# hadleyhzy34/porl

Measured on AMD Instinct MI355X. Metric: gradient-steps/sec (POR update, batch=1024), higher is better.
Workload: dtype f32; 1 GPU; POR S=60 A=2 H=1024 L=2 B=1024/GPU (global 1024), 1000000 -row replay (1000000/GPU) resident in HBM, device sampler + gather + full update per step; parallelism=dp1, global_batch=1024

## Files before the change

### include/porl_hip.h

```cpp
#ifndef PORL_HIP_H
#define PORL_HIP_H

#include <stdint.h>

#ifdef __cplusplus
extern "C" {
#endif

#define PORL_ABI_VERSION 11
#define PORL_MAX_HIDDEN 8

#define PORL_OK 0
#define PORL_ERR_INVALID (-1)
#define PORL_ERR_UNSUPPORTED (-2)
#define PORL_ERR_UNBOUND (-3)

int porl_abi_version(void);
const char* porl_last_error(void);

typedef struct porl_iql_cfg {
  int32_t obs_dim;
  int32_t pol_out_dim;
  int32_t hidden_dim;
  int32_t n_hidden;
  int32_t layer_norm;
  int32_t pol_tanh;
  int32_t weight_mode;
  int32_t max_batch;
} porl_iql_cfg;

typedef struct porl_iql porl_iql;

int porl_iql_create(const porl_iql_cfg* cfg, porl_iql** out);
void porl_iql_destroy(porl_iql* h);

int64_t porl_iql_group_floats(const porl_iql* h, int group);
int32_t porl_iql_group_tensors(const porl_iql* h, int group);
int porl_iql_tensor_info(const porl_iql* h, int group, int index, int64_t* offset, int32_t* rows,
                         int32_t* cols);

int64_t porl_iql_workspace_floats(const porl_iql* h);

typedef struct porl_iql_buffers {
  float* params_vf;
  float* params_tgt;
  float* params_pol;
  float* grads_vf;
  float* grads_pol;
  float* adam_m_vf;
  float* adam_v_vf;
  float* adam_m_pol;
  float* adam_v_pol;
  float* workspace;
  float* stats;
} porl_iql_buffers;

int porl_iql_bind(porl_iql* h, const porl_iql_buffers* bufs);

int porl_iql_load_batch(porl_iql* h, int32_t batch,
                        const float* obs, int64_t obs_rs,
                        const float* next_obs, int64_t next_rs,
                        const float* rew, int64_t rew_rs,
                        const float* term, int64_t term_rs,
                        const float* pol_target, int64_t pt_rs,
                        void* stream);

int porl_iql_load_batch_sampled(porl_iql* h, int32_t batch, const float* rows, int64_t row_stride,
                                int64_t n_rows, int32_t act_dim, int32_t target_is_action,
                                uint64_t seed, uint64_t step, int64_t* idx_out, void* stream);

#define PORL_IQL_SLOTS 3
#define PORL_IQL_MODE_TWO_SLOTS 1
#define PORL_IQL_MODE_FOLD_COMBINE 2
#define PORL_IQL_MODE_SHORT_BLOCKS 4
int porl_iql_set_mode(porl_iql* h, int32_t mode);

int porl_iql_set_stats(porl_iql* h, float* stats);

typedef struct porl_iql_hyper {
  float tau;
  float discount;
  float alpha;
  float inv_batch;
  int32_t value_step;
  int32_t policy_step;
  int32_t reserved;
  double ema_beta;
  double value_lr;
  double policy_lr;
  double adam_beta1, adam_beta2, adam_eps;
} porl_iql_hyper;

int porl_iql_value_backward(porl_iql* h, const porl_iql_hyper* hp, void* stream);
int porl_iql_value_apply(porl_iql* h, const porl_iql_hyper* hp, void* stream);
int porl_iql_policy_prefetch(porl_iql* h, void* stream);
int porl_iql_policy_forward(porl_iql* h, const porl_iql_hyper* hp, void* stream);
int porl_iql_policy_backward(porl_iql* h, const porl_iql_hyper* hp, void* stream);
int porl_iql_policy_apply(porl_iql* h, const porl_iql_hyper* hp, void* stream);
int porl_iql_step(porl_iql* h, const porl_iql_hyper* hp, void* stream);
int porl_iql_policy_only_forward(porl_iql* h, const porl_iql_hyper* hp, void* stream);
int porl_iql_policy_only_step(porl_iql* h, const porl_iql_hyper* hp, void* stream);

int porl_iql_forward_value(porl_iql* h, int which, const float* x, int64_t x_rs, int32_t batch,
                           float* v1_out, float* v2_out, void* stream);
int porl_iql_forward_policy(porl_iql* h, const float* x, int64_t x_rs, int32_t batch, float* mean_out,
                            int64_t mean_rs, void* stream);

typedef struct porl_qnet_cfg {
  int32_t state_dim;
  int32_t n_actions;
  int32_t n_hidden;
  int32_t hidden[PORL_MAX_HIDDEN];
  int32_t max_batch;
} porl_qnet_cfg;

typedef struct porl_qnet porl_qnet;

typedef struct porl_qnet_buffers {
  float* params;
  float* params_tgt;
  float* grads;
  float* adam_m;
  float* adam_v;
  float* workspace;
  float* stats;
} porl_qnet_buffers;

typedef struct porl_qnet_hyper {
  float gamma;
  float alpha;
  float inv_batch;
  int32_t step;
  double lr;
  double adam_beta1, adam_beta2, adam_eps;
} porl_qnet_hyper;

int porl_qnet_create(const porl_qnet_cfg* cfg, porl_qnet** out);
void porl_qnet_destroy(porl_qnet* h);
int64_t porl_qnet_param_floats(const porl_qnet* h);
int32_t porl_qnet_tensors(const porl_qnet* h);
int porl_qnet_tensor_info(const porl_qnet* h, int index, int64_t* offset, int32_t* rows, int32_t* cols,
                          int32_t* row_stride);
int64_t porl_qnet_workspace_floats(const porl_qnet* h);
int porl_qnet_bind(porl_qnet* h, const porl_qnet_buffers* bufs);
int porl_qnet_load_batch(porl_qnet* h, int32_t batch, const float* states, int64_t s_rs,
                         const int64_t* actions, int64_t a_rs, const float* rewards, int64_t r_rs,
                         const float* next_states, int64_t n_rs, const float* dones, int64_t d_rs,
                         void* stream);
int porl_qnet_cql_backward(porl_qnet* h, const porl_qnet_hyper* hp, void* stream);
int porl_qnet_forward_loaded(porl_qnet* h, int which_params, int which_input, int keep, float* out, int64_t out_rs,
                             void* stream);
int porl_qnet_backward(porl_qnet* h, const float* dout, int64_t dout_rs, void* stream);

int porl_qr_loss(const float* z_cur, const float* z_next_online, const float* z_next_target, int64_t ld,
                 const int64_t* actions, const float* rewards, const float* dones, int32_t batch, int32_t n_actions,
                 int32_t n_quantiles, float gamma, float kappa, float* dz_out, float* row_loss, void* stream);
int porl_iqn_quantile_huber(const float* current, const float* target, const float* taus, int32_t batch, int32_t n_current,
                            int32_t n_target, float kappa, float* dcurrent_out, float* row_loss, void* stream);
int porl_iqn_cos_embed(const float* taus, int64_t n, int32_t embedding_dim, float* out, void* stream);
int porl_iqn_hadamard(const float* feat, int64_t ldf, const float* emb, int32_t batch, int32_t n_tau, int32_t width,
                      float* out, void* stream);
int porl_iqn_hadamard_backward(const float* dout, const float* feat, int64_t ldf, const float* emb, int32_t batch,
                               int32_t n_tau, int32_t width, float* dfeat, float* demb, void* stream);
int porl_iqn_select(const float* z, const int64_t* actions, int32_t batch, int32_t n_tau, int32_t n_actions, float* out,
                    void* stream);
int porl_iqn_scatter(const float* dsel, const int64_t* actions, int32_t batch, int32_t n_tau, int32_t n_actions, float* dz,
                     void* stream);
int porl_iqn_target(const float* z_online_next, const float* z_target_next, const float* rewards, const float* dones,
                    float gamma, int32_t batch, int32_t n_tau, int32_t n_actions, float* td, int64_t* next_actions,
                    void* stream);
int porl_grad_clip(float* grads, int64_t n, float max_norm, float* norm_coef, double* workspace, void* stream);
int porl_c51_loss(const float* logits_cur, const float* logits_next_target, int64_t ld, const int64_t* actions,
                  const float* rewards, const float* dones, const float* support, int32_t batch, int32_t n_actions,
                  int32_t n_atoms, float gamma, float v_min, float v_max, float* dlogits_out, float* row_loss, void* stream);
int porl_reduce_mean(const float* x, int32_t n, float* out, void* stream);

int porl_qnet_apply(porl_qnet* h, const porl_qnet_hyper* hp, void* stream);
int porl_qnet_learn(porl_qnet* h, const porl_qnet_hyper* hp, void* stream);
int32_t porl_qnet_one_launch(const porl_qnet* h);
int porl_qnet_learn_indexed(porl_qnet* h, const float* states, int64_t s_rs, const int64_t* actions,
                            const float* rewards, const float* next_states, int64_t n_rs, const float* dones,
                            const int64_t* idx, int32_t batch, const porl_qnet_hyper* hp, void* stream);
typedef struct porl_qnet_variant {
  int32_t double_dqn;
  const float* is_weights;
  const float* uniform_weight;
  float* td_abs;
  const float* next_mask;
  int32_t td_off;
} porl_qnet_variant;
int32_t porl_qnet_can_sample(const porl_qnet* h);
int porl_qnet_learn_sampled(porl_qnet* h, const float* states, int64_t s_rs, const int64_t* actions, const float* rewards,
                            const float* next_states, int64_t n_rs, const float* dones, int64_t n_rows, uint64_t seed,
                            uint64_t draw, int32_t batch, const porl_qnet_hyper* hp, void* stream);
int porl_qnet_learn_variant(porl_qnet* h, const float* states, int64_t s_rs, const int64_t* actions,
                            const float* rewards, const float* next_states, int64_t n_rs, const float* dones,
                            const int64_t* idx, int32_t batch, const porl_qnet_hyper* hp,
                            const porl_qnet_variant* variant, void* stream);
int porl_qnet_learn_sampled_variant(porl_qnet* h, const float* states, int64_t s_rs, const int64_t* actions,
                                    const float* rewards, const float* next_states, int64_t n_rs, const float* dones,
                                    int64_t n_rows, uint64_t seed, uint64_t draw, int32_t batch, const porl_qnet_hyper* hp,
                                    const porl_qnet_variant* variant, void* stream);
int porl_qnet_bcq_mask(porl_qnet* beh, const float* next_states, int64_t n_rs, const int64_t* idx, int32_t batch,
                       float threshold, float* mask_out, void* stream);
int porl_qnet_bcq_learn(porl_qnet* h, porl_qnet* beh, const float* states, int64_t s_rs, const int64_t* actions,
                        const float* rewards, const float* next_states, int64_t n_rs, const float* dones,
                        const int64_t* idx, int32_t batch, const porl_qnet_hyper* hp, float threshold, void* stream);
int porl_qnet_bcq_learn_sampled(porl_qnet* h, porl_qnet* beh, const float* states, int64_t s_rs, const int64_t* actions,
                                const float* rewards, const float* next_states, int64_t n_rs, const float* dones,
                                int64_t n_rows, uint64_t seed, uint64_t draw, int32_t batch, const porl_qnet_hyper* hp,
                                float threshold, void* stream);
#define PORL_DIST_QR 0
#define PORL_DIST_C51 1
typedef struct porl_dist_head {
  int32_t kind;
  int32_t n_actions;
  int32_t n_sub;
  float kappa;
  float v_min, v_max;
  const float* support;
} porl_dist_head;
int porl_qnet_dist_learn(porl_qnet* h, const float* states, int64_t s_rs, const int64_t* actions, const float* rewards,
                         const float* next_states, int64_t n_rs, const float* dones, const int64_t* idx, int32_t batch,
                         const porl_qnet_hyper* hp, const porl_dist_head* head, void* stream);
int porl_qnet_sync_target(porl_qnet* h, void* stream);
int porl_qnet_forward(porl_qnet* h, int which, const float* states, int64_t s_rs, int32_t batch,
                      float* q_out, int64_t q_rs, void* stream);
// ... 216 lines not shown
```

### porl_amd/agent/_iql.py

```python
from __future__ import annotations

import math
import warnings

import torch
import torch.nn as nn

from ..engine import IqlEngine
from ..parallel import GradExchange



_PIPE_SYNC = __import__("os").environ.get("PORL_PIPE_SYNC", "signal2")
_PIPE_ONECALL = __import__("os").environ.get("PORL_PIPE_ONECALL", "auto")
_DP_POLICY_GROUP = __import__("os").environ.get("PORL_DP_POLICY_GROUP", "1") != "0"
_ONECALL_MAX_WORK = 32 << 20

class ArenaAdam:

    def __init__(self, agent, group, named_params, lr):
        self._agent, self._group = agent, group
        self._names = [n for n, _ in named_params]
        self._params = [p for _, p in named_params]
        self.step_count = 0
# ... 12 lines not shown
        table = eng.tensor_table(self._group)
        return IqlEngine.views(flat_m, table), IqlEngine.views(flat_v, table)

    def zero_grad(self, set_to_none=True):
        pass

    def step(self):
        raise RuntimeError("ArenaAdam steps inside the fused update (por_residual_update / update)")

    sharded = False

    def _gather_moments(self):
        if self.sharded:
            eng, ex = self._agent._engine, self._agent._exchange
            _, _, m, v, _ = eng.group(self._group)
            ex.all_gather_(m)
            ex.all_gather_(v)

    def _unshard(self):
        if self.sharded:
            self._gather_moments()
            self.sharded = False

    def consolidate_state(self):
        self._agent.flush()
        self._unshard()

    def state_dict(self):
        self._agent.flush()
        self._gather_moments()
        ms, vs = self._moments()
        state = {}
        if self.step_count > 0:
            for i, (m, v) in enumerate(zip(ms, vs)):
                state[i] = dict(step=torch.tensor(float(self.step_count)), exp_avg=m.clone(), exp_avg_sq=v.clone())
        groups = [{k: v for k, v in self.param_groups[0].items() if k != "params"}]
        groups[0]["params"] = list(range(len(self._params)))
        return dict(state=state, param_groups=groups)

    def load_state_dict(self, sd):
        self._agent.flush()
        ms, vs = self._moments()
        steps = set()
        with torch.no_grad():
            for i, st in sd["state"].items():
                ms[int(i)].copy_(st["exp_avg"])
                vs[int(i)].copy_(st["exp_avg_sq"])
                steps.add(int(float(st["step"])))
        if len(steps) > 1:
            raise ValueError("per-parameter Adam step counts differ; the flat sweep needs one counter")
        self.step_count = steps.pop() if steps else 0
        self.sharded = False
        g = sd["param_groups"][0]
        for k in ("lr", "betas", "eps", "initial_lr"):
            if k in g:
                self.param_groups[0][k] = g[k]


class CosineSchedule:

    def __init__(self, optimizer: ArenaAdam, T_max):
        self.optimizer, self.T_max, self.last_epoch = optimizer, T_max, 0
        self.base_lrs = [optimizer.param_groups[0]["initial_lr"]]

    def _lr(self, t):
        return self.base_lrs[0] * (1.0 + math.cos(math.pi * t / self.T_max)) / 2.0

    def step(self):
        self.last_epoch += 1
        self.optimizer.param_groups[0]["lr"] = self._lr(self.last_epoch)

    def get_last_lr(self):
        return [self.optimizer.param_groups[0]["lr"]]

    def state_dict(self):
        return dict(T_max=self.T_max, last_epoch=self.last_epoch, base_lrs=list(self.base_lrs))

    def load_state_dict(self, sd):
        self.T_max, self.last_epoch = sd["T_max"], sd["last_epoch"]
        self.base_lrs = list(sd["base_lrs"])
        self.optimizer.param_groups[0]["lr"] = self._lr(self.last_epoch)


class IqlAgentBase(nn.Module):

    _warned_nll = False
    pipeline = True
    grad_exchange = "reduce_scatter"
    dp_policy_group = _DP_POLICY_GROUP

    def _setup_engine(self, vf: nn.Module, v_target: nn.Module, policy: nn.Module, *, obs_dim, pol_out_dim,
                      hidden_dim, n_hidden, layer_norm, pol_tanh, weight_mode, device, max_batch):
        self._engine = IqlEngine(obs_dim, pol_out_dim, hidden_dim, n_hidden, layer_norm, pol_tanh, weight_mode,
                                 max_batch, device)
        self._mods = (vf, v_target, policy)
        self._adopt(copy_from_modules=True)
        self._exchange = GradExchange()
        self._gslice = {}
        self.async_losses = False

    def _adopt(self, copy_from_modules=False):
        eng = self._engine
        vf, v_target, policy = self._mods
        pairs = ((vf, eng.params_vf, IqlEngine.GROUP_VF, "vf"),
                 (v_target, eng.params_tgt, IqlEngine.GROUP_VF, "target"),
                 (policy, eng.params_pol, IqlEngine.GROUP_POL, "policy"))
        with torch.no_grad():
            for mod, flat, group, role in pairs:
                views = IqlEngine.views(flat, eng.tensor_table(group))
                params = list(mod.parameters())
                if len(params) != len(views):
                    raise RuntimeError(f"{role}: {len(params)} parameters vs {len(views)} engine tensors")
                for p, v in zip(params, views):
                    if tuple(p.shape) != tuple(v.shape):
                        raise RuntimeError(f"{role}: parameter shape {tuple(p.shape)} vs engine {tuple(v.shape)}")
                    if copy_from_modules:
                        v.copy_(p)
                    p.data = v
                mod._engine, mod._engine_role, mod._private = eng, role, False
        for p in v_target.parameters():
            p.requires_grad_(False)

    def _apply(self, fn, recurse=True):
        self.flush()
        probe = fn(torch.empty(0, dtype=torch.float32, device=self._engine.device))
        if probe.dtype != torch.float32:
            raise RuntimeError("porl_amd agents are fp32 only")
        self._engine.to(probe.device)
        self.device = probe.device
        self._adopt()
        backbone = getattr(self, "backbone", None)
        if backbone is not None:
            backbone._apply(fn)
        return self

    def _hyper(self, batch, v_opt: ArenaAdam, p_opt: ArenaAdam):
        world = self._exchange.world_size
        return self._engine.hyper(
            tau=self.tau, discount=self.discount, alpha=self.alpha, ema_beta=self.beta,
            inv_batch=1.0 / (batch * world), value_lr=v_opt.lr, policy_lr=p_opt.lr,
            value_step=v_opt.step_count, policy_step=p_opt.step_count,
            adam_beta1=v_opt.param_groups[0]["betas"][0], adam_beta2=v_opt.param_groups[0]["betas"][1],
            adam_eps=v_opt.param_groups[0]["eps"])

    def _full_update(self, obs, next_obs, rew, term, pol_target, v_opt, p_opt, sched, replay=None, batch=None):
        eng, ex = self._engine, self._exchange
        world = ex.world_size
        dp = ex.active
        pipelined = self.async_losses and self.pipeline
        if not pipelined:
            eng.join()
        eng._ensure_bound()
        eng.set_mode(((IqlEngine.MODE_TWO_SLOTS | IqlEngine.MODE_SHORT_BLOCKS) if pipelined else 0) |
                     (IqlEngine.MODE_FOLD_COMBINE if not dp else 0))
        use_sig = pipelined and _PIPE_SYNC in ("signal", "signal2") and eng.signals() is not None
        onecall = _PIPE_ONECALL is True or _PIPE_ONECALL == "1" or (
            _PIPE_ONECALL == "auto" and (batch or 0) * eng.cfg.hidden_dim ** 2 <= _ONECALL_MAX_WORK)
        if use_sig and not dp and replay is not None and onecall:
            eng._seq += 1
            seq = eng._seq
            v_opt.step_count += 1
            p_opt.step_count += 1
            hp = self._hyper(batch, v_opt, p_opt)
            vr = eng._values_read
            try:
                eng.update_pipelined(hp, replay, batch, seq,
                                     wait_policy_seq=max(0, seq - eng.SLOTS) if _PIPE_SYNC == "signal" else 0,
                                     wait_fwd_seq=vr[1] if isinstance(vr, tuple) else 0,
                                     write_policy=_PIPE_SYNC == "signal")
            except Exception:
                eng._seq -= 1
                v_opt.step_count -= 1
                p_opt.step_count -= 1
                raise
            replay.draws += 1
            eng._values_read, eng._policy_done = ("sig", seq), True
            sched.step()
            return self._losses()
        if use_sig:
            main = torch.cuda.current_stream(eng.device)
            eng._seq += 1
            seq = eng._seq
            if _PIPE_SYNC == "signal":
                eng.wait_signal(eng.SIG_POLICY, seq - eng.SLOTS, main)
        elif pipelined:
            eng.wait_slot_free()
        if replay is not None:
            B = eng.load_batch_sampled(replay.rows, batch, replay.seed, replay.draws, replay.act_dim,
                                       self._engine.cfg.weight_mode == 1)
            replay.draws += 1
        else:
            B = eng.load_batch(obs, next_obs, rew, term, pol_target)
        v_opt.step_count += 1
        p_opt.step_count += 1
        hp = self._hyper(B, v_opt, p_opt)
        if not dp and not pipelined:
            eng.step(hp)
            sched.step()
            return self._losses()
        eng.value_backward(hp)
        if dp and self._sharded():
            self._sharded_apply(IqlEngine.GROUP_VF, hp, v_opt)
        else:
            if dp:
                v_opt._unshard()
                ex.allreduce_sum_(eng.grads_vf)
            eng.wait_values_read()
            eng.value_apply(hp)
        if pipelined:
            main, side = torch.cuda.current_stream(eng.device), eng.side_stream()
            k = (v_opt.step_count % eng.SLOTS) * 3
            ev_v, ev_f, ev_p = eng.event(k), eng.event(k + 1), eng.event(k + 2)
            if use_sig:
                eng.signal(eng.SIG_VALUE, seq, main)
            else:
                ev_v.record(main)
            with torch.cuda.stream(side):
                if use_sig:
                    eng.wait_signal(eng.SIG_VALUE, seq, side)
                else:
                    side.wait_event(ev_v)
                eng.policy_forward(hp)
                if use_sig:
                    eng.signal(eng.SIG_FWD, seq, side)
                else:
                    ev_f.record(side)
                eng.policy_backward(hp)
                if dp and self._sharded():
                    self._sharded_apply(IqlEngine.GROUP_POL, hp, p_opt, self._exchange_for(IqlEngine.GROUP_POL, True))
                else:
                    if dp:
                        p_opt._unshard()
                        self._exchange_for(IqlEngine.GROUP_POL, True).allreduce_sum_(eng.grads_pol)
                    eng.policy_apply(hp)
                if _PIPE_SYNC == "signal" and use_sig:
                    eng.signal(eng.SIG_POLICY, seq, side)
                if not use_sig:
                    ev_p.record(side)
            eng._values_read, eng._policy_done = (("sig", seq) if use_sig else ev_f), (True if use_sig else ev_p)
            eng._slot_users = eng._slot_users[1:] + [None if use_sig else ev_p]
        else:
            eng.policy_backward(hp)
            if self._sharded():
                self._sharded_apply(IqlEngine.GROUP_POL, hp, p_opt)
            else:
                p_opt._unshard()
                ex.allreduce_sum_(eng.grads_pol)
                eng.policy_apply(hp)
            if not self.async_losses:
                ex.allreduce_stats_(eng.stats)
        sched.step()
        return self._losses()

    def _sharded(self):
        eng, ex = self._engine, self._exchange
        return self.grad_exchange == "reduce_scatter" and ex.can_shard(eng.grads_vf) and ex.can_shard(eng.grads_pol)

    def _exchange_for(self, group, pipelined):
        ex = self._exchange
        if group != IqlEngine.GROUP_POL or not pipelined or not ex.active or not self.dp_policy_group:
            return ex
        if getattr(self, "_exchange_pol", None) is None:
            import torch.distributed as dist
            self._exchange_pol = GradExchange(dist.new_group(), force=ex.force)
            probe = torch.zeros(1, dtype=torch.float32, device=self._engine.device)
            dist.all_reduce(probe, group=self._exchange_pol.group)
            torch.cuda.synchronize(self._engine.device)
        return self._exchange_pol

    def _sharded_apply(self, group, hp, opt, ex=None):
        from .. import engine as E
        eng = self._engine
        ex = ex or self._exchange
        p, g, m, v, tgt = eng.group(group)
        gs = self._gslice.get(group)
        if gs is None or gs.numel() != p.numel() // ex.world_size:
            gs = self._gslice[group] = torch.empty(p.numel() // ex.world_size, dtype=torch.float32, device=p.device)
        ex.reduce_scatter_sum(g, gs)
        if group == IqlEngine.GROUP_VF:
            eng.wait_values_read()
        b1, b2 = opt.param_groups[0]["betas"]
        E.adam_ema(ex.slice_of(p), gs, ex.slice_of(m), ex.slice_of(v), None, opt.lr, opt.step_count, b1, b2,
                   opt.param_groups[0]["eps"], 0.0)
        ex.all_gather_(p)
        if tgt is not None:
            E.ema(tgt, p, hp.ema_beta)
        opt.sharded = True

    def flush(self):
        self._engine.join()

    def state_dict(self, *args, **kwargs):
        self.flush()
        return super().state_dict(*args, **kwargs)

    def load_state_dict(self, *args, **kwargs):
        self.flush()
        return super().load_state_dict(*args, **kwargs)

    def _load(self, obs, next_obs, rew, term, pol_target, replay, batch):
        eng = self._engine
        if replay is None:
            return eng.load_batch(obs, next_obs, rew, term, pol_target)
        B = eng.load_batch_sampled(replay.rows, batch, replay.seed, replay.draws, replay.act_dim,
                                   eng.cfg.weight_mode == 1)
        replay.draws += 1
        return B
# ... 74 lines not shown
```

### porl_amd/csrc/gemm_f32.hpp

```cpp
#pragma once
#include <hip/hip_runtime.h>
#include <stdint.h>

#ifndef PORL_ABL
#define PORL_ABL 0
#endif

namespace porl {

enum : int { ACT_NONE = 0, ACT_RELU = 1, ACT_TANH = 2 };

enum : int {
  APRO_NONE = 0,
  APRO_AFFINE_RELU = 1,
};

struct GemmProb {
  const float* A;
  const float* B;
  float* C;
  const float* bias;
  const float* mask;
  const float* headw;
  float* headout;
  float* colsum;
  const float* a_colscale;
  const float* a_colshift;
  const float* resid;
  const float* rscale;
  float* cstat;
  int rs_rows, rs_row0;
  int a_grp, a_grp_jump, a_seg_tiles, a_seg_jump;
  int M, N, K;
  int lda, ldb, ldc, ldmask;
  int act;
  int apro;
  int splitk;
  int store_c;
  int a_vec, b_vec;
  int a_kc, b_kc;
  int c_vec;
  int tiles_m, tiles_n, block_start, kchunk;
};

constexpr int MAX_GROUP = 8;
struct GemmGroup {
  int nprob;
  int total_blocks;
  int single_buffer;
  GemmProb p[MAX_GROUP];
  int lds_pad, lds_pad_min_blocks;
};

typedef float f32x16 __attribute__((ext_vector_type(16)));

__host__ __device__ constexpr int lds_stride(int R) { return R + 4; }

struct StageSlot {
  unsigned off;
  int kpos;
  int cpos;
  int lds;
};

typedef int i32x4 __attribute__((ext_vector_type(4)));
typedef float f32x4 __attribute__((ext_vector_type(4)));
constexpr unsigned BUF_OOB = 0x80000000u;

__device__ f32x4 llvm_raw_buffer_load_v4f32(i32x4 rsrc, int voffset, int soffset, int aux) __asm("llvm.amdgcn.raw.buffer.load.v4f32");
__device__ float llvm_raw_buffer_load_f32(i32x4 rsrc, int voffset, int soffset, int aux) __asm("llvm.amdgcn.raw.buffer.load.f32");

typedef i32x4 BufRsrc;
__device__ __forceinline__ BufRsrc make_rsrc(const float* p, size_t bytes) {
  const unsigned long long a = reinterpret_cast<unsigned long long>(p);
  BufRsrc r;
  r.x = (int)(unsigned)(a & 0xFFFFFFFFull);
  r.y = (int)(unsigned)((a >> 32) & 0xFFFFull);
  r.z = (int)(bytes >= 0x7FFFFFFFull ? 0x7FFFFFFFu : (unsigned)bytes);
  r.w = 0x00020000;
  return r;
}
__device__ __forceinline__ float4 buf_ld128(BufRsrc r, unsigned voff, unsigned soff) {
  const f32x4 v = llvm_raw_buffer_load_v4f32(r, (int)voff, (int)soff, 0);
  return make_float4(v.x, v.y, v.z, v.w);
}
__device__ __forceinline__ float buf_ld32(BufRsrc r, unsigned voff, unsigned soff) {
  return llvm_raw_buffer_load_f32(r, (int)voff, (int)soff, 0);
}

template <bool V> struct BoolTag { static constexpr bool value = V; };
template <int V> struct IntTag { static constexpr int value = V; };

#ifdef PORL_STAMP
__device__ unsigned long long g_stamps[16 * 4096];
#endif

template <int BM, int BN, int BK, int WM, int WN, bool VEC, bool APRO, bool ONEBUF = false>
__global__ __launch_bounds__(64 * WM * WN) void gemm_f32_kernel(const GemmGroup g) {
  constexpr int THREADS = 64 * WM * WN;
  constexpr int WTM = BM / WM / 32;
  constexpr int WTN = BN / WN / 32;
  constexpr int SA = lds_stride(BM);
  constexpr int SB = lds_stride(BN);
  constexpr int SK = BK + 4;
  constexpr int A_TILE = (BK * SA > BM * SK) ? BK * SA : BM * SK;
  constexpr int B_TILE = (BK * SB > BN * SK) ? BK * SB : BN * SK;
  static_assert(BK % 8 == 0, "a k-group is 8 wide");
  constexpr int NLA = BM * BK / 4 / THREADS;
  constexpr int NLB = BN * BK / 4 / THREADS;
  static_assert(NLA >= 1 && NLB >= 1, "tile too small for the thread count");
  static_assert(BM * BK / 4 % THREADS == 0 && BN * BK / 4 % THREADS == 0, "staging must divide evenly");
  static_assert(BK % 4 == 0 && WTM >= 1 && WTN >= 1 && BM % (32 * WM) == 0 && BN % (32 * WN) == 0, "tile shape");

  constexpr int APRO_MAX_K = ONEBUF ? 512 : 1024;
  constexpr int NBUF = ONEBUF ? 1 : 2;
  __shared__ __attribute__((aligned(16))) float lds[NBUF * (A_TILE + B_TILE) + (APRO ? 2 * APRO_MAX_K : 0)];

  const int t = threadIdx.x;
  const int lane = t & 63;
  const int wave = t >> 6;
  const int wm = wave / WN, wn = wave % WN;
  const int li = lane & 31, kh = lane >> 5;
#ifdef PORL_STAMP
  unsigned long long rt_entry = 0, rt_loop0 = 0, rt_loop1 = 0, cy0 = 0, cy1 = 0, cy_barrier = 0, cy_store = 0, cy_load = 0, cy_group[4] = {0, 0, 0, 0};
  if (t == 0) rt_entry = __builtin_amdgcn_s_memrealtime();
#endif

  int lin;
  {
    const int nb = gridDim.x, bid = blockIdx.x;
    const int q = nb >> 3, r = nb & 7, xcd = bid & 7;
    lin = (xcd < r ? xcd * (q + 1) : r * (q + 1) + (xcd - r) * q) + (bid >> 3);
  }
  int pi = 0;
#pragma unroll
  for (int i = 1; i < MAX_GROUP; ++i)
    if (i < g.nprob && lin >= g.p[i].block_start) pi = i;
  const GemmProb& P = g.p[pi];
  const int local = lin - P.block_start;
  const int tiles = P.tiles_m * P.tiles_n;
  const int split = local / tiles;
  const int tl = local - split * tiles;
  const int tm = tl / P.tiles_n, tn = tl - tm * P.tiles_n;
  const int m0 = tm * BM, n0 = tn * BN;
  const int M = P.M, N = P.N;
  const int ks = split * P.kchunk;
  const int ke = min(P.K, ks + P.kchunk);
  const int nkt = (ke - ks + BK - 1) / BK;
  const float* __restrict__ Ag = P.A;
  const float* __restrict__ Bg = P.B;
  const bool a_kc = P.a_kc != 0, b_kc = P.b_kc != 0;
  const bool do_colsum = (!a_kc) && (P.colsum != nullptr) && (tn == 0);
  const bool full = VEC && (m0 + BM <= M) && (n0 + BN <= N) && ((ke - ks) % BK == 0);
  auto ktile = [&](int i) { return i; };

  StageSlot sa[NLA], sb[NLB];
  const int a_dk = a_kc ? 1 : 0, a_dc = 1 - a_dk;
  const int b_dk = b_kc ? 1 : 0, b_dc = 1 - b_dk;
  const size_t a_step = a_kc ? (size_t)BK : (size_t)BK * P.lda;
  const size_t b_step = b_kc ? (size_t)BK : (size_t)BK * P.ldb;
  const size_t a_rows_ext = P.a_grp > 0 ? (size_t)M + (size_t)(M / P.a_grp + 1) * (size_t)(P.a_grp_jump / P.lda + 1) +
                                              (size_t)(P.a_seg_jump / P.lda + 1)
                                        : (size_t)(a_kc ? M : P.K);
  const BufRsrc a_rsrc = make_rsrc(Ag, a_rows_ext * P.lda * sizeof(float));
  const BufRsrc b_rsrc = make_rsrc(Bg, (size_t)(b_kc ? N : P.K) * P.ldb * sizeof(float));
  const unsigned a_org = (unsigned)((a_kc ? (size_t)ks : (size_t)ks * P.lda) * sizeof(float));
  const unsigned b_org = (unsigned)((b_kc ? (size_t)ks : (size_t)ks * P.ldb) * sizeof(float));
  const int a_seg_tiles = P.a_grp > 0 ? P.a_seg_tiles : 0x7fffffff;
  const unsigned a_seg_jump = (unsigned)((size_t)P.a_seg_jump * sizeof(float));
  auto a_soff = [&](int kt) {
    return a_org + (unsigned)(kt * a_step * sizeof(float)) + (kt >= a_seg_tiles ? a_seg_jump : 0u);
  };
  auto b_soff = [&](int kt) { return b_org + (unsigned)(kt * b_step * sizeof(float)); };
#pragma unroll
  for (int i = 0; i < NLA; ++i) {
    const int f = t + THREADS * i;
    if (a_kc) {
      const int kq = f % (BK / 4), row = f / (BK / 4);
      sa[i].kpos = ks + kq * 4; sa[i].cpos = m0 + row; sa[i].lds = row * SK + kq * 4;
      const size_t grp = P.a_grp > 0 ? (size_t)((m0 + row) / P.a_grp) * P.a_grp_jump : 0;
      sa[i].off = (unsigned)(((size_t)(m0 + row) * P.lda + grp + kq * 4) * sizeof(float));
    } else {
      const int c4 = f % (BM / 4), kr = f / (BM / 4);
      sa[i].kpos = ks + kr; sa[i].cpos = m0 + c4 * 4; sa[i].lds = kr * SA + c4 * 4;
      sa[i].off = (unsigned)(((size_t)kr * P.lda + (m0 + c4 * 4)) * sizeof(float));
    }
  }
#pragma unroll
  for (int i = 0; i < NLB; ++i) {
    const int f = t + THREADS * i;
    if (b_kc) {
      const int kq = f % (BK / 4), row = f / (BK / 4);
      sb[i].kpos = ks + kq * 4; sb[i].cpos = n0 + row; sb[i].lds = row * SK + kq * 4;
      sb[i].off = (unsigned)(((size_t)(n0 + row) * P.ldb + kq * 4) * sizeof(float));
    } else {
      const int c4 = f % (BN / 4), kr = f / (BN / 4);
      sb[i].kpos = ks + kr; sb[i].cpos = n0 + c4 * 4; sb[i].lds = kr * SB + c4 * 4;
      sb[i].off = (unsigned)(((size_t)kr * P.ldb + (n0 + c4 * 4)) * sizeof(float));
    }
  }

  float* const apro_cs = lds + NBUF * (A_TILE + B_TILE);
  if constexpr (APRO) {
    for (int k = t; k < P.K; k += THREADS) { apro_cs[k] = P.a_colscale[k]; apro_cs[APRO_MAX_K + k] = P.a_colshift[k]; }
  }

  float4 ra[NLA], rb[NLB];
  float4 csum = make_float4(0.f, 0.f, 0.f, 0.f);

  f32x16 acc[WTM][WTN];
#pragma unroll
  for (int i = 0; i < WTM; ++i)
#pragma unroll
    for (int j = 0; j < WTN; ++j)
#pragma unroll
      for (int r = 0; r < 16; ++r) acc[i][j][r] = 0.f;

  const int a_off = wm * (BM / WM) + li;
  const int b_off = wn * (BN / WN) + li;

  auto main_loop = [&](auto guard_tag, auto akc_tag, auto bkc_tag, auto csum_tag) {
    constexpr bool GUARD = decltype(guard_tag)::value;
    constexpr bool AKC = decltype(akc_tag)::value;
    constexpr bool CSUM = decltype(csum_tag)::value;

    auto slot_ok = [&](const StageSlot& s, int kadv, int dk, int dc, int cmax, bool (&ok)[4]) {
      const int k = s.kpos + kadv;
      if constexpr (VEC) {
        ok[0] = ok[1] = ok[2] = ok[3] = (k < ke) && (s.cpos < cmax);
      } else {
#pragma unroll
        for (int j = 0; j < 4; ++j) ok[j] = (k + j * dk < ke) && (s.cpos + j * dc < cmax);
      }
    };
    auto load_raw = [&](const StageSlot& s, BufRsrc r, unsigned soff, const bool (&ok)[4]) -> float4 {
      float4 v;
      if constexpr (VEC) {
        v = buf_ld128(r, ok[0] ? s.off : BUF_OOB, soff);
      } else {
        v.x = buf_ld32(r, ok[0] ? s.off : BUF_OOB, soff);
        v.y = buf_ld32(r, ok[1] ? s.off + 4u : BUF_OOB, soff);
        v.z = buf_ld32(r, ok[2] ? s.off + 8u : BUF_OOB, soff);
        v.w = buf_ld32(r, ok[3] ? s.off + 12u : BUF_OOB, soff);
      }
      return v;
    };

    auto load_tile = [&](int kt) {
      const int kadv = kt * BK;
#pragma unroll
// ... 258 lines not shown
    } else {
      main_loop(guard_tag, BoolTag<false>{}, BoolTag<false>{}, BoolTag<false>{});
    }
  };
  if constexpr (VEC) {
    if (full) run(BoolTag<false>{});
    else run(BoolTag<true>{});
  } else {
    run(BoolTag<true>{});
  }
#ifdef PORL_STAMP
  if (t == 0) { rt_loop1 = __builtin_amdgcn_s_memrealtime(); cy1 = __builtin_amdgcn_s_memtime(); }
#endif

  if (do_colsum) {
    __syncthreads();
    float4* red = reinterpret_cast<float4*>(lds);
    constexpr int C4 = BM / 4;
    auto reduce_cols = [&](const float4& mine, float* out) {
      red[t] = mine;
      __syncthreads();
      if (t < C4) {
        float4 s = red[t];
        for (int u = t + C4; u < THREADS; u += C4) {
          const float4 o = red[u];
          s.x += o.x; s.y += o.y; s.z += o.z; s.w += o.w;
        }
        const int c = m0 + t * 4;
        if (c < M) out[c] = s.x;
        if (c + 1 < M) out[c + 1] = s.y;
        if (c + 2 < M) out[c + 2] = s.z;
        if (c + 3 < M) out[c + 3] = s.w;
      }
      __syncthreads();
    };
    reduce_cols(csum, P.colsum + (size_t)split * M);
  }

  const bool raw = P.splitk > 1;
  float* __restrict__ Cg = P.C + (raw ? (size_t)split * M * P.ldc : 0);
  const bool has_head = (!raw) && P.headw != nullptr;
  const float* __restrict__ maskp = raw ? nullptr : P.mask;
  const int act = raw ? ACT_NONE : P.act;
  const bool store_c = P.store_c != 0;
  constexpr int WROWS = BM / WM, WCOLS = BN / WN, CS = WCOLS + 4;
  static_assert(WM * WN * WROWS * CS <= NBUF * (A_TILE + B_TILE), "C sub-tiles must fit in the staging LDS");
  const bool fast_c = store_c && P.c_vec && (m0 + BM <= M) && (n0 + BN <= N);
  float* ctile = lds + wave * (WROWS * CS);
#pragma unroll
  for (int i = 0; i < WTM; ++i) {
    const int rbase = m0 + wm * (BM / WM) + i * 32 + 4 * kh;
#pragma unroll
    for (int j = 0; j < WTN; ++j) {
      const int col = n0 + wn * (BN / WN) + j * 32 + li;
      const bool col_ok = col < N;
      float bv = 0.f, hw = 0.f;
      if (!raw && col_ok) {
        if (P.bias) bv = P.bias[col];
        if (has_head) hw = P.headw[col];
      }
      float vals[16];
#pragma unroll
      for (int r = 0; r < 16; ++r) {
        float v = acc[i][j][r] + bv;
        if (act == ACT_RELU) v = fmaxf(v, 0.f);
        else if (act == ACT_TANH) v = tanhf(v);
        vals[r] = v;
      }
      if (maskp && !fast_c) {
#pragma unroll
        for (int r = 0; r < 16; ++r) {
          const int row = rbase + (r & 3) + 8 * (r >> 2);
          const bool ok = row < M && col_ok;
          const float mv = *(ok ? maskp + (size_t)row * P.ldmask + col : maskp);
          vals[r] = (ok && mv > 0.f) ? vals[r] : 0.f;
        }
      }
      if (!raw && P.resid && !fast_c) {
#pragma unroll
        for (int r = 0; r < 16; ++r) {
          const int row = rbase + (r & 3) + 8 * (r >> 2);
          if (row < M && col_ok) {
            const float rs = P.rscale ? P.rscale[(row + P.rs_row0) / P.rs_rows] : 1.f;
            vals[r] = __fadd_rn(P.resid[(size_t)row * P.ldc + col], __fmul_rn(vals[r], rs));
          }
        }
      }
      if (!raw && P.cstat) {
        float cs = 0.f, cq = 0.f;
#pragma unroll
        for (int r = 0; r < 16; ++r) {
          const int row = rbase + (r & 3) + 8 * (r >> 2);
          const float v = row < M ? vals[r] : 0.f;
          cs += v;
          cq = fmaf(v, v, cq);
        }
        cs += __shfl_xor(cs, 32);
        cq += __shfl_xor(cq, 32);
        const int rblk = (m0 + wm * (BM / WM)) / 32 + i;
        if (kh == 0 && col_ok && rblk * 32 < M) {
          float* o = P.cstat + (size_t)rblk * 2 * N + col;
          o[0] = cs;
          o[N] = cq;
        }
      }
      if (has_head) {
        const int part = (n0 + wn * (BN / WN) + j * 32) >> 5;
#pragma unroll
        for (int r = 0; r < 16; ++r) {
          float sh = vals[r] * hw;
          sh += __shfl_xor(sh, 16);
          sh += __shfl_xor(sh, 8);
          sh += __shfl_xor(sh, 4);
          sh += __shfl_xor(sh, 2);
          sh += __shfl_xor(sh, 1);
          const int row = rbase + (r & 3) + 8 * (r >> 2);
          if (li == 0 && row < M && part * 32 < N) P.headout[(size_t)part * M + row] = sh;
        }
      }
      if (store_c) {
        if (fast_c) {
#pragma unroll
          for (int r = 0; r < 16; ++r)
            ctile[(i * 32 + (r & 3) + 8 * (r >> 2) + 4 * kh) * CS + j * 32 + li] = vals[r];
        } else {
#pragma unroll
          for (int r = 0; r < 16; ++r) {
            const int row = rbase + (r & 3) + 8 * (r >> 2);
            if (row < M && col_ok) Cg[(size_t)row * P.ldc + col] = vals[r];
          }
        }
      }
    }
  }
  if (fast_c) {
    constexpr int C4 = WCOLS / 4;
    const int wr0 = m0 + wm * WROWS, wc0 = n0 + wn * WCOLS;
#pragma unroll 4
    for (int f = lane; f < WROWS * C4; f += 64) {
      const int r = f / C4, c = (f % C4) * 4;
      float4 v = *reinterpret_cast<const float4*>(ctile + r * CS + c);
      if (maskp) {
        const float4 mk = *reinterpret_cast<const float4*>(maskp + (size_t)(wr0 + r) * P.ldmask + wc0 + c);
        v.x = mk.x > 0.f ? v.x : 0.f; v.y = mk.y > 0.f ? v.y : 0.f;
        v.z = mk.z > 0.f ? v.z : 0.f; v.w = mk.w > 0.f ? v.w : 0.f;
      }
      if (!raw && P.resid) {
        const float rs = P.rscale ? P.rscale[(wr0 + r + P.rs_row0) / P.rs_rows] : 1.f;
        const float4 x4 = *reinterpret_cast<const float4*>(P.resid + (size_t)(wr0 + r) * P.ldc + wc0 + c);
        v.x = __fadd_rn(x4.x, __fmul_rn(v.x, rs)); v.y = __fadd_rn(x4.y, __fmul_rn(v.y, rs));
        v.z = __fadd_rn(x4.z, __fmul_rn(v.z, rs)); v.w = __fadd_rn(x4.w, __fmul_rn(v.w, rs));
      }
      *reinterpret_cast<float4*>(Cg + (size_t)(wr0 + r) * P.ldc + wc0 + c) = v;
    }
  }
#ifdef PORL_STAMP
  __syncthreads();
  if (t == 0 && blockIdx.x < 4096) {
    const unsigned hwid = __builtin_amdgcn_s_getreg((4 ) | (0 << 6) | (31 << 11));
    const unsigned xcc = __builtin_amdgcn_s_getreg((20 ) | (0 << 6) | (31 << 11));
    unsigned long long* o = g_stamps + 16 * blockIdx.x;
    o[0] = rt_entry; o[1] = rt_loop0; o[2] = rt_loop1; o[3] = __builtin_amdgcn_s_memrealtime();
    o[4] = cy1 - cy0; o[5] = ((xcc & 0xF) << 12) | ((hwid >> 8) & 0xFFF);
    o[6] = cy_group[0]; o[7] = cy_group[1]; o[8] = cy_group[2]; o[9] = cy_group[3];
  }
#endif
}

__global__ void slab_reduce_kernel(float* __restrict__ out, const float* __restrict__ slab, int nslab,
                                   long n, long stride, const float* __restrict__ bias, int ncols, int act) {
  for (long i = (long)blockIdx.x * blockDim.x + threadIdx.x; i < n; i += (long)gridDim.x * blockDim.x) {
    float s = slab[i];
    for (int k = 1; k < nslab; ++k) s += slab[(long)k * stride + i];
    if (bias) s += bias[i % ncols];
    if (act == ACT_RELU) s = fmaxf(s, 0.f);
    else if (act == ACT_TANH) s = tanhf(s);
    out[i] = s;
  }
}

enum GemmMode : int { GEMM_NT = 0, GEMM_NN = 1, GEMM_TN = 2 };
enum GemmTile : int { TILE_128x128 = 0, TILE_128x64 = 1, TILE_64x128 = 2, TILE_64x64 = 3,
                      TILE_128x96 = 4,
                      TILE_COUNT = 5 };

constexpr int GEMM_BK = 32;

struct TileCfg { int bm, bn, wm, wn; };
inline TileCfg tile_cfg(int tile) {
  switch (tile) {
    case TILE_128x128: return {128, 128, 2, 2};
    case TILE_128x64: return {128, 64, 2, 2};
    case TILE_64x128: return {64, 128, 2, 2};
    case TILE_128x96: return {128, 96, 4, 1};
    default: return {64, 64, 2, 2};
  }
}

inline void tile_dims(int tile, int& bm, int& bn) {
  const TileCfg c = tile_cfg(tile);
  bm = c.bm; bn = c.bn;
}

inline int head_parts(int N, int tile) {
  (void)tile;
  return (N + 31) / 32;
}
constexpr int HEAD_PARTS_PER_64_COLS = 2;

inline bool aligned16(const void* p) { return (reinterpret_cast<uintptr_t>(p) & 15u) == 0; }

inline int plan_group(GemmGroup& g, int tile) {
  int bm, bn;
  tile_dims(tile, bm, bn);
  int start = 0;
  for (int i = 0; i < g.nprob; ++i) {
    GemmProb& p = g.p[i];
    p.tiles_m = (p.M + bm - 1) / bm;
    p.tiles_n = (p.N + bn - 1) / bn;
    if (p.splitk < 1) p.splitk = 1;
    int kc = (p.K + p.splitk - 1) / p.splitk;
    kc = ((kc + GEMM_BK - 1) / GEMM_BK) * GEMM_BK;
    p.kchunk = kc;
    p.c_vec = aligned16(p.C) && (p.ldc % 4 == 0) && (p.splitk == 1 || ((size_t)p.M * p.ldc) % 4 == 0) &&
              (p.mask == nullptr || (aligned16(p.mask) && p.ldmask % 4 == 0));
    p.block_start = start;
    start += p.tiles_m * p.tiles_n * p.splitk;
  }
  g.total_blocks = start;
  return start;
}

template <int BM, int BN, int WM, int WN>
inline hipError_t launch_tile(const GemmGroup& g, hipStream_t s) {
  dim3 grid(g.total_blocks), block(64 * WM * WN);
  const int pad = g.total_blocks >= g.lds_pad_min_blocks ? g.lds_pad : 0;
  bool vec = true, apro = g.p[0].apro != APRO_NONE;
  for (int i = 0; i < g.nprob; ++i) {
    vec = vec && g.p[i].a_vec && g.p[i].b_vec;
    if ((g.p[i].apro != APRO_NONE) != apro) return hipErrorInvalidValue;
    if (g.p[i].splitk <= 1 && (g.p[i].mask || g.p[i].resid) && (g.p[i].cstat || g.p[i].headw)) return hipErrorInvalidValue;
  }
  if (apro) {
    if constexpr ((BM == 64 && BN == 64) || (BM == 128 && BN == 64) || (BM == 128 && BN == 96)) {
      for (int i = 0; i < g.nprob; ++i) {
        const GemmProb& p = g.p[i];
        if (!p.a_kc || !p.b_kc || p.K % GEMM_BK || p.splitk > 1 || !p.a_colscale || !p.a_colshift || !vec ||
            (reinterpret_cast<uintptr_t>(p.a_colscale) & 15u) || (reinterpret_cast<uintptr_t>(p.a_colshift) & 15u))
          return hipErrorInvalidValue;
        if (p.K > (g.single_buffer && BM == 64 && BN == 64 ? 512 : 1024)) return hipErrorInvalidValue;
      }
      if constexpr (BM == 64 && BN == 64) {
        if (g.single_buffer) {
          hipLaunchKernelGGL((gemm_f32_kernel<BM, BN, GEMM_BK, WM, WN, true, true, true>), grid, block, pad, s, g);
          return hipGetLastError();
        }
      }
      hipLaunchKernelGGL((gemm_f32_kernel<BM, BN, GEMM_BK, WM, WN, true, true>), grid, block, pad, s, g);
      return hipGetLastError();
    } else {
      return hipErrorInvalidValue;
    }
  }
  if constexpr (BM == 64 && BN == 64) {
    if (vec && g.single_buffer) {
      hipLaunchKernelGGL((gemm_f32_kernel<BM, BN, GEMM_BK, WM, WN, true, false, true>), grid, block, pad, s, g);
      return hipGetLastError();
    }
  }
  if (vec) hipLaunchKernelGGL((gemm_f32_kernel<BM, BN, GEMM_BK, WM, WN, true, false>), grid, block, pad, s, g);
  else hipLaunchKernelGGL((gemm_f32_kernel<BM, BN, GEMM_BK, WM, WN, false, false>), grid, block, pad, s, g);
  return hipGetLastError();
}

inline hipError_t launch_gemm_group(int tile, GemmGroup& g, hipStream_t s) {
  if (g.nprob < 1 || g.nprob > MAX_GROUP) return hipErrorInvalidValue;
  if (plan_group(g, tile) == 0) return hipSuccess;
  switch (tile) {
    case TILE_128x128: return launch_tile<128, 128, 2, 2>(g, s);
    case TILE_128x64: return launch_tile<128, 64, 2, 2>(g, s);
    case TILE_64x128: return launch_tile<64, 128, 2, 2>(g, s);
    case TILE_64x64: return launch_tile<64, 64, 2, 2>(g, s);
    case TILE_128x96: return launch_tile<128, 96, 4, 1>(g, s);
  }
  return hipErrorInvalidValue;
}

inline GemmProb make_prob(int mode, const float* A, int lda, const float* B, int ldb, float* C, int ldc, int M,
                          int N, int K) {
  GemmProb p{};
  p.a_kc = (mode == GEMM_NT || mode == GEMM_NN);
  p.b_kc = (mode == GEMM_NT);
  p.A = A; p.B = B; p.C = C;
  p.M = M; p.N = N; p.K = K;
  p.lda = lda; p.ldb = ldb; p.ldc = ldc;
  p.act = ACT_NONE; p.apro = APRO_NONE; p.splitk = 1; p.store_c = 1; p.rs_rows = 1;
  p.a_vec = aligned16(A) && (lda % 4 == 0) && ((p.a_kc ? K : M) % 4 == 0);
  p.b_vec = aligned16(B) && (ldb % 4 == 0) && ((p.b_kc ? K : N) % 4 == 0);
  return p;
}

}
```

### porl_amd/csrc/kernels.hpp

```cpp
#pragma once
#include <hip/hip_runtime.h>
#include <stdint.h>

namespace porl {

constexpr float LOG_STD_MIN = -5.0f;
constexpr float LOG_STD_MAX = 2.0f;
constexpr float EXP_ADV_MAX = 100.0f;

__device__ __forceinline__ float wave_sum(float v) {
#pragma unroll
  for (int o = 32; o > 0; o >>= 1) v += __shfl_xor(v, o);
  return v;
}
__device__ __forceinline__ float wave_min(float v) {
#pragma unroll
  for (int o = 32; o > 0; o >>= 1) v = fminf(v, __shfl_xor(v, o));
  return v;
}

struct PackJob {
  const float* src; float* dst;
  long src_row_stride;
  long src_col_stride;
// ... 155 lines not shown
    m += mb[0];
    if (a.tanh_mean) m = tanhf(m);
    const float z = cv ? (xv - m) * isg[0] : 0.f;
    const float zz = wave_sum(z * z);
    const float nlp = half_log2pi_D + 0.5f * zz + lsig;
    loss_acc += wb * nlp;
    min_acc = fminf(min_acc, nlp);
    if (cv) {
      float dm = -wb * z * isg[0];
      if (a.tanh_mean) dm *= (1.f - m * m);
      a.dmean[(size_t)b * a.ldd + lane] = dm;
      dls[0] += wb * (1.f - z * z);
    }
  }
  for (int b = row0 + wave; !fast && b < row1; b += 4) {
    float v0 = 0.f, v1 = 0.f;
    for (int p = lane; p < a.parts; p += 64) {
      v0 += a.hp_v[0][(size_t)p * a.B + b];
      v1 += a.hp_v[1][(size_t)p * a.B + b];
    }
    v0 = wave_sum(v0); v1 = wave_sum(v1);
    const float adv = a.weight ? 0.f : a.target_v[b] - fminf(v0 + bv0, v1 + bv1);
    const float wgt = a.weight ? a.weight[b] : fminf(expf(a.weight_mode ? a.alpha * adv : adv / a.alpha), EXP_ADV_MAX);
    const float wb = wgt * a.inv_batch;
    float zz = 0.f;
    float z[NLL_MAX_COLS_PER_LANE], mu[NLL_MAX_COLS_PER_LANE];
#pragma unroll
    for (int c = 0; c < NLL_MAX_COLS_PER_LANE; ++c) {
      const int j = lane + 64 * c;
      z[c] = 0.f; mu[c] = 0.f;
      if (c < ncl && j < a.D) {
        float m = a.mean_slab[(size_t)b * a.ldm + j];
#pragma unroll 8
        for (int s = 1; s < a.nslab; ++s) m += a.mean_slab[(size_t)s * a.slab_stride + (size_t)b * a.ldm + j];
        m += mb[c];
        if (a.tanh_mean) m = tanhf(m);
        mu[c] = m;
        z[c] = (a.x[(size_t)b * a.ldx + j] - m) * isg[c];
        zz += z[c] * z[c];
      }
    }
    zz = wave_sum(zz);
    const float nlp = half_log2pi_D + 0.5f * zz + lsig;
    loss_acc += wb * nlp;
    min_acc = fminf(min_acc, nlp);
#pragma unroll
    for (int c = 0; c < NLL_MAX_COLS_PER_LANE; ++c) {
      const int j = lane + 64 * c;
      if (c < ncl && j < a.D) {
        float dm = -wb * z[c] * isg[c];
        if (a.tanh_mean) dm *= (1.f - mu[c] * mu[c]);
        a.dmean[(size_t)b * a.ldd + j] = dm;
        dls[c] += wb * (1.f - z[c] * z[c]);
      }
    }
  }
  for (int b = row0 + wave; b < row1; b += 4)
    for (int j = a.D + lane; j < a.ldd; j += 64) a.dmean[(size_t)b * a.ldd + j] = 0.f;

#pragma unroll
  for (int c = 0; c < NLL_MAX_COLS_PER_LANE; ++c) sh_dls[wave][c * 64 + lane] = dls[c];
  if (lane == 0) { sh_loss[wave] = loss_acc; sh_min[wave] = min_acc; }
  __syncthreads();
  if (wave == 0) {
#pragma unroll
    for (int c = 0; c < NLL_MAX_COLS_PER_LANE; ++c) {
      const int j = lane + 64 * c;
      if (c < ncl && j < a.D) {
        const float ls = a.log_std[j];
        const float inside = (ls >= LOG_STD_MIN && ls <= LOG_STD_MAX) ? 1.f : 0.f;
        a.part_dls[(size_t)blockIdx.x * a.D + j] = inside *
            (sh_dls[0][c * 64 + lane] + sh_dls[1][c * 64 + lane] + sh_dls[2][c * 64 + lane] + sh_dls[3][c * 64 + lane]);
      }
    }
    if (lane == 0) {
      a.part_loss[blockIdx.x] = sh_loss[0] + sh_loss[1] + sh_loss[2] + sh_loss[3];
      a.part_min[blockIdx.x] = fminf(fminf(sh_min[0], sh_min[1]), fminf(sh_min[2], sh_min[3]));
    }
  }
}


struct ReduceJob {
  float* out; const float* slab; const float* bias;
  long n; long stride; int nslab; int ncols; int act;
  int op;
  float scale;
  long adam_off;
  int width;
};
constexpr int MAX_REDUCE_JOBS = 12;
struct ReduceArgs { int njobs; ReduceJob job[MAX_REDUCE_JOBS]; };

constexpr int REDUCE_LDS_FLOATS = 64 * 5;
__device__ __forceinline__ float reduce_chunk(const ReduceJob& j, long i0, float* sh) {
  const int W = j.width, L = 256 / W;
  const int tx = threadIdx.x % W, ty = threadIdx.x / W;
  const long i = i0 + tx;
  const float id = j.op ? INFINITY : 0.f;
  float s0 = id, s1 = id, s2 = id, s3 = id;
  if (i < j.n) {
    const float* p = j.slab + i;
    int k = ty;
    for (; k + 3 * L < j.nslab; k += 4 * L) {
      const float x0 = p[(long)k * j.stride], x1 = p[(long)(k + L) * j.stride];
      const float x2 = p[(long)(k + 2 * L) * j.stride], x3 = p[(long)(k + 3 * L) * j.stride];
      if (j.op) { s0 = fminf(s0, x0); s1 = fminf(s1, x1); s2 = fminf(s2, x2); s3 = fminf(s3, x3); }
      else { s0 += x0; s1 += x1; s2 += x2; s3 += x3; }
    }
    for (; k < j.nslab; k += L) {
      const float x = p[(long)k * j.stride];
      s0 = j.op ? fminf(s0, x) : s0 + x;
    }
  }
  const float s = j.op ? fminf(fminf(s0, s1), fminf(s2, s3)) : (s0 + s1) + (s2 + s3);
  sh[ty * (W + 1) + tx] = s;
  __syncthreads();
  if (W == 4) {
    const int w = threadIdx.x >> 6, ln = threadIdx.x & 63;
    float v = sh[ln * (W + 1) + w];
    v = j.op ? wave_min(v) : wave_sum(v);
    __syncthreads();
    if (ln == 0) sh[w] = v;
    __syncthreads();
  }
  float t = 0.f;
  if (ty == 0 && i < j.n) {
    t = sh[tx];
    if (W != 4)
      for (int q = 1; q < L; ++q) t = j.op ? fminf(t, sh[q * (W + 1) + tx]) : t + sh[q * (W + 1) + tx];
    t *= j.scale;
    if (j.bias) t += j.bias[i % j.ncols];
    if (j.act == 1) t = fmaxf(t, 0.f);
    else if (j.act == 2) t = tanhf(t);
  }
  __syncthreads();
  return t;
}

__global__ __launch_bounds__(256) void multi_reduce_kernel(const ReduceArgs a) {
  __shared__ float sh[REDUCE_LDS_FLOATS];
  const ReduceJob& j = a.job[blockIdx.y];
  const int W = j.width, tx = threadIdx.x % W, ty = threadIdx.x / W;
  for (long i0 = (long)blockIdx.x * W; i0 < j.n; i0 += (long)gridDim.x * W) {
    const float t = reduce_chunk(j, i0, sh);
    if (ty == 0 && i0 + tx < j.n) j.out[i0 + tx] = t;
  }
}

struct AdamScalars { float omb1, beta2, omb2, eps, step_size, bc2_sqrt, ema_beta, omeb; };
constexpr int ADAM_SWEEP_SLABS = 16;
constexpr int MAX_ADAM_REGIONS = 8;
struct AdamRegion { long lo, hi; const float* slab; long stride; int nslab; };
struct AdamArgs {
  float* p; float* g; float* m; float* v; float* tgt;
  long n4;
  long span4;
  int reduce_blocks;
  AdamScalars s;
  int nregions; AdamRegion region[MAX_ADAM_REGIONS];
  int nskip; long skip_lo[MAX_REDUCE_JOBS], skip_hi[MAX_REDUCE_JOBS];
  int job_block0[MAX_REDUCE_JOBS + 1];
  ReduceArgs r;
};

__device__ __forceinline__ float ema1(float t, float p, float omeb, float ema_beta) { return t * omeb + ema_beta * p; }

__device__ __forceinline__ void adam1(float& p, float g, float& m, float& v, const AdamScalars& s) {
  m = m + s.omb1 * (g - m);
  v = v * s.beta2 + s.omb2 * g * g;
  p = p - s.step_size * (m / (sqrtf(v) / s.bc2_sqrt + s.eps));
}

__global__ __launch_bounds__(256) void adam_ema_kernel(const AdamArgs a) {
  __shared__ float sh[REDUCE_LDS_FLOATS];
  const AdamScalars s = a.s;
  if ((int)blockIdx.x < a.reduce_blocks) {
    const int rb = blockIdx.x;
    int ji = 0;
#pragma unroll
    for (int q = 1; q < MAX_REDUCE_JOBS; ++q)
      if (q < a.r.njobs && rb >= a.job_block0[q]) ji = q;
    const ReduceJob& j = a.r.job[ji];
    const long i0 = (long)(rb - a.job_block0[ji]) * j.width;
    const float t = reduce_chunk(j, i0, sh);
    const int tx = threadIdx.x % j.width, ty = threadIdx.x / j.width;
    if (ty == 0 && i0 + tx < j.n) {
      j.out[i0 + tx] = t;
      if (j.adam_off >= 0) {
        const long e = j.adam_off + i0 + tx;
        float pp = a.p[e], mm = a.m[e], vv = a.v[e];
        adam1(pp, t, mm, vv, s);
        a.p[e] = pp; a.m[e] = mm; a.v[e] = vv;
        if (a.tgt) a.tgt[e] = ema1(a.tgt[e], pp, s.omeb, s.ema_beta);
      }
    }
    return;
  }
  float4* p4 = reinterpret_cast<float4*>(a.p);
  float4* g4 = reinterpret_cast<float4*>(a.g);
  float4* m4 = reinterpret_cast<float4*>(a.m);
  float4* v4 = reinterpret_cast<float4*>(a.v);
  float4* t4 = reinterpret_cast<float4*>(a.tgt);
  const long lo4 = (long)(blockIdx.x - a.reduce_blocks) * a.span4, hi4 = min(a.n4, lo4 + a.span4);
  bool special = false;
  for (int q = 0; q < a.nregions; ++q) special = special || (lo4 * 4 < a.region[q].hi && hi4 * 4 > a.region[q].lo);
  for (int q = 0; q < a.nskip; ++q) special = special || (lo4 * 4 < a.skip_hi[q] && hi4 * 4 > a.skip_lo[q]);
  for (long i = lo4 + threadIdx.x; i < hi4; i += 256) {
    float4 gg;
    bool have_g = false;
    if (special) {
      const long e = i * 4;
      bool skip = false;
      for (int q = 0; q < a.nskip; ++q) skip = skip || (e >= a.skip_lo[q] && e < a.skip_hi[q]);
      if (skip) continue;
      for (int q = 0; q < a.nregions; ++q) {
        const AdamRegion& R = a.region[q];
        if (e >= R.lo && e < R.hi) {
          float4 part[8];
#pragma unroll
          for (int u = 0; u < 8; ++u) part[u] = make_float4(0.f, 0.f, 0.f, 0.f);
          const float* base = R.slab + (e - R.lo);
#pragma unroll
          for (int k = 0; k < ADAM_SWEEP_SLABS; ++k)
            if (k < R.nslab) {
              const float4 x = *reinterpret_cast<const float4*>(base + (long)k * R.stride);
              part[k & 7].x += x.x; part[k & 7].y += x.y; part[k & 7].z += x.z; part[k & 7].w += x.w;
            }
          gg = part[0];
#pragma unroll
          for (int u = 1; u < 8; ++u) { gg.x += part[u].x; gg.y += part[u].y; gg.z += part[u].z; gg.w += part[u].w; }
          g4[i] = gg;
          have_g = true;
        }
      }
    }
    if (!have_g) gg = g4[i];
    float4 pp = p4[i];
    float4 mm = m4[i], vv = v4[i];
    adam1(pp.x, gg.x, mm.x, vv.x, s); adam1(pp.y, gg.y, mm.y, vv.y, s);
    adam1(pp.z, gg.z, mm.z, vv.z, s); adam1(pp.w, gg.w, mm.w, vv.w, s);
    p4[i] = pp; m4[i] = mm; v4[i] = vv;
    if (a.tgt) {
      float4 tt = t4[i];
      tt.x = ema1(tt.x, pp.x, s.omeb, s.ema_beta); tt.y = ema1(tt.y, pp.y, s.omeb, s.ema_beta);
      tt.z = ema1(tt.z, pp.z, s.omeb, s.ema_beta); tt.w = ema1(tt.w, pp.w, s.omeb, s.ema_beta);
      t4[i] = tt;
    }
  }
}

__global__ __launch_bounds__(256) void ema_kernel(float* __restrict__ tgt, const float* __restrict__ src, long n4,
                                                   float omeb, float ema_beta) {
  float4* t4 = reinterpret_cast<float4*>(tgt);
  const float4* p4 = reinterpret_cast<const float4*>(src);
  const long i = (long)blockIdx.x * 256 + threadIdx.x;
  if (i >= n4) return;
  float4 tt = t4[i];
  const float4 pp = p4[i];
  tt.x = ema1(tt.x, pp.x, omeb, ema_beta); tt.y = ema1(tt.y, pp.y, omeb, ema_beta);
  tt.z = ema1(tt.z, pp.z, omeb, ema_beta); tt.w = ema1(tt.w, pp.w, omeb, ema_beta);
  t4[i] = tt;
}

constexpr int SMALL_FWD_MAX_B = 8;
struct SmallFwdArgs {
  const float* W[2]; const float* bias[2];
  const float* X[2]; long ldx[2];
  float* Y[2]; long ldy[2];
  int N, K, B, act;
};

__global__ __launch_bounds__(256) void small_fwd_kernel(const SmallFwdArgs a) {
  extern __shared__ float xs[];
  const int net = blockIdx.y;
  const float* __restrict__ X = a.X[net];
  for (int i = threadIdx.x; i < a.B * a.K; i += 256) {
    const int b = i / a.K, k = i - b * a.K;
    xs[i] = X[(long)b * a.ldx[net] + k];
  }
  __syncthreads();
  const int wave = threadIdx.x >> 6, lane = threadIdx.x & 63;
  const float* __restrict__ W = a.W[net];
  const bool vec = (a.K & 3) == 0 && ((reinterpret_cast<uintptr_t>(W) & 15) == 0);
  for (int n = blockIdx.x * 4 + wave; n < a.N; n += gridDim.x * 4) {
    const float* __restrict__ w = W + (size_t)n * a.K;
    float acc[SMALL_FWD_MAX_B];
#pragma unroll
    for (int b = 0; b < SMALL_FWD_MAX_B; ++b) acc[b] = 0.f;
    if (vec) {
      for (int k = lane * 4; k < a.K; k += 256) {
        const float4 wv = *reinterpret_cast<const float4*>(w + k);
#pragma unroll
        for (int b = 0; b < SMALL_FWD_MAX_B; ++b)
          if (b < a.B) {
            const float4 xv = *reinterpret_cast<const float4*>(xs + b * a.K + k);
            acc[b] = fmaf(wv.x, xv.x, fmaf(wv.y, xv.y, fmaf(wv.z, xv.z, fmaf(wv.w, xv.w, acc[b]))));
          }
      }
    } else {
      for (int k = lane; k < a.K; k += 64) {
        const float wv = w[k];
#pragma unroll
        for (int b = 0; b < SMALL_FWD_MAX_B; ++b)
          if (b < a.B) acc[b] = fmaf(wv, xs[b * a.K + k], acc[b]);
      }
    }
    const float bv = a.bias[net] ? a.bias[net][n] : 0.f;
#pragma unroll
    for (int b = 0; b < SMALL_FWD_MAX_B; ++b)
      if (b < a.B) {
        float v = wave_sum(acc[b]) + bv;
        if (a.act == 1) v = fmaxf(v, 0.f);
        else if (a.act == 2) v = tanhf(v);
        if (lane == 0) a.Y[net][(long)b * a.ldy[net] + n] = v;
      }
  }
}

__global__ void head_finish_kernel(const float* __restrict__ hp0, const float* __restrict__ hp1,
                                   const float* __restrict__ b0, const float* __restrict__ b1, int parts, int B,
                                   float* __restrict__ out0, float* __restrict__ out1) {
  const int b = blockIdx.x * blockDim.x + threadIdx.x;
  if (b >= B) return;
  float v0 = 0.f, v1 = 0.f;
  for (int p = 0; p < parts; ++p) { v0 += hp0[(size_t)p * B + b]; v1 += hp1[(size_t)p * B + b]; }
  out0[b] = v0 + b0[0];
  out1[b] = v1 + b1[0];
}

__global__ void mean_finish_kernel(const float* __restrict__ slab, int nslab, long stride, int B, int D, int ldm,
                                   const float* __restrict__ bias, int tanh_mean, float* __restrict__ out,
                                   long out_rs) {
  const long n = (long)B * D;
  for (long i = (long)blockIdx.x * blockDim.x + threadIdx.x; i < n; i += (long)gridDim.x * blockDim.x) {
    const long b = i / D;
    const int j = (int)(i - b * D);
    float m = slab[b * ldm + j];
    for (int s = 1; s < nslab; ++s) m += slab[(long)s * stride + b * ldm + j];
    m += bias[j];
    if (tanh_mean) m = tanhf(m);
    out[b * out_rs + j] = m;
  }
}

__global__ __launch_bounds__(256) void gather_rows_kernel(const float* __restrict__ rows, long row_stride,
                                                           const int64_t* __restrict__ idx, int n, int width,
                                                           float* __restrict__ out, long out_stride) {
  const int wave = (blockIdx.x * blockDim.x + threadIdx.x) >> 6, lane = threadIdx.x & 63;
  const int nwaves = (gridDim.x * blockDim.x) >> 6;
  const bool vec = (width & 3) == 0 && (row_stride & 3) == 0 && (out_stride & 3) == 0 &&
                   ((reinterpret_cast<uintptr_t>(rows) | reinterpret_cast<uintptr_t>(out)) & 15) == 0;
  for (int i = wave; i < n; i += nwaves) {
    const float* src = rows + idx[i] * row_stride;
    float* dst = out + (long)i * out_stride;
    if (vec) {
      for (int c = lane * 4; c < width; c += 256)
        *reinterpret_cast<float4*>(dst + c) = *reinterpret_cast<const float4*>(src + c);
    } else {
      for (int c = lane; c < width; c += 64) dst[c] = src[c];
    }
  }
}

__device__ __forceinline__ uint32_t mix32(uint32_t x) {
  x ^= x >> 16; x *= 0x7feb352du; x ^= x >> 15; x *= 0x846ca68bu; x ^= x >> 16;
  return x;
}

__device__ __forceinline__ int64_t feistel_index(int64_t n, int64_t i, uint64_t seed, uint64_t step, int hb) {
  const uint32_t mask = (1u << hb) - 1u;
  uint32_t keys[4];
#pragma unroll
  for (int r = 0; r < 4; ++r)
    keys[r] = mix32((uint32_t)(seed >> (r & 1 ? 32 : 0)) ^ mix32((uint32_t)step * 4u + r) ^ (uint32_t)(step >> 30));
  uint64_t x = (uint64_t)i;
  do {
    uint32_t L = (uint32_t)(x >> hb) & mask, R = (uint32_t)x & mask;
#pragma unroll
    for (int r = 0; r < 4; ++r) {
      const uint32_t f = mix32(R ^ keys[r]) & mask;
      const uint32_t t = L ^ f;
      L = R; R = t;
    }
    x = ((uint64_t)L << hb) | R;
  } while ((int64_t)x >= n);
  return (int64_t)x;
}

struct SampledBatchArgs {
  const float* rows; long row_stride; int64_t n_rows;
  int batch, S, A, D, Sp, Dp, hb, target_is_action;
  uint64_t seed, step;
  float* xs; float* xn; float* xt; float* rew; float* term;
  int64_t* idx_out;
};

__global__ __launch_bounds__(256) void sampled_batch_kernel(const SampledBatchArgs a) {
  const int i = blockIdx.x * 4 + (threadIdx.x >> 6), lane = threadIdx.x & 63;
  if (i >= a.batch) return;
  const int64_t r = feistel_index(a.n_rows, i, a.seed, a.step, a.hb);
  const float* __restrict__ src = a.rows + r * a.row_stride;
  const int S = a.S;
  for (int c = lane; c < a.Sp; c += 64) {
    a.xs[(size_t)i * a.Sp + c] = c < S ? src[c] : 0.f;
    a.xn[(size_t)i * a.Sp + c] = c < S ? src[S + 1 + c] : 0.f;
  }
  const int toff = a.target_is_action ? 2 * S + 2 : S + 1;
  for (int c = lane; c < a.Dp; c += 64) a.xt[(size_t)i * a.Dp + c] = c < a.D ? src[toff + c] : 0.f;
  if (lane == 0) {
    a.rew[i] = src[S];
    a.term[i] = src[2 * S + 1];
    if (a.idx_out) a.idx_out[i] = r;
  }
// ... 415 lines not shown
```

### porl_amd/csrc/porl_api.hip

```cpp
#include <hip/hip_runtime.h>

#include <algorithm>
#include <cmath>
#include <cstdio>
#include <cstring>
#include <string>
#include <vector>

#include "../../include/porl_hip.h"
#include "gemm_f32.hpp"
#include "gemm_bf16.hpp"
#include "kernels.hpp"
#include "l0_fwd.hpp"
#include "skinny.hpp"
#include "iqn.hpp"
#include "qnet_fused.hpp"
#include "per_tree.hpp"
#include "dist_losses.hpp"
#include "online.hpp"
#include "per_online.hpp"
#include "bcq_mask.hpp"

using namespace porl;

namespace {

thread_local std::string g_err;

#define PORL_FAIL(code, ...)                         \
  do {                                               \
    char _b[512];                                    \
    snprintf(_b, sizeof _b, __VA_ARGS__);            \
    g_err = _b;                                      \
    return (code);                                   \
  } while (0)

#define PORL_HIP(expr)                                                        \
  do {                                                                        \
    hipError_t _e = (expr);                                                   \
    if (_e != hipSuccess) {                                                   \
      g_err = std::string(#expr) + ": " + hipGetErrorString(_e);              \
      return (int)_e;                                                         \
    }                                                                         \
  } while (0)

#define PORL_TRY(expr)          \
  do {                          \
    int _r = (expr);            \
    if (_r != 0) return _r;     \
  } while (0)

struct DevGuard {
  int prev = -1;
  bool switched = false;
  explicit DevGuard(int dev) {
    if (dev >= 0 && hipGetDevice(&prev) == hipSuccess && prev != dev) switched = hipSetDevice(dev) == hipSuccess;
  }
  ~DevGuard() { if (switched) (void)hipSetDevice(prev); }
  DevGuard(const DevGuard&) = delete;
  DevGuard& operator=(const DevGuard&) = delete;
};
int device_of(const void* p) {
  hipPointerAttribute_t a;
  if (!p || hipPointerGetAttributes(&a, p) != hipSuccess) { (void)hipGetLastError(); return -1; }
  return a.type == hipMemoryTypeDevice ? a.device : -1;
}

struct ProfRec { int label; hipEvent_t e0, e1; double flops, bytes; };
struct ProfState {
  bool on = false;
  std::vector<std::string> labels;
  std::vector<ProfRec> recs;
  std::vector<hipEvent_t> pool;
  size_t pool_used = 0;
  hipEvent_t get() {
    if (pool_used == pool.size()) { hipEvent_t e; (void)hipEventCreate(&e); pool.push_back(e); }
    return pool[pool_used++];
  }
  int label_id(const std::string& s) {
    for (size_t i = 0; i < labels.size(); ++i) if (labels[i] == s) return (int)i;
    labels.push_back(s);
    return (int)labels.size() - 1;
  }
} g_prof;

const char* g_phase = "";

struct ProfScope {
  bool active; ProfRec r; hipStream_t s;
  ProfScope(const std::string& label, hipStream_t st, double flops, double bytes) : active(g_prof.on), s(st) {
    if (!active) return;
    r.label = g_prof.label_id(std::string(g_phase) + label); r.flops = flops; r.bytes = bytes;
    r.e0 = g_prof.get(); r.e1 = g_prof.get();
    (void)hipEventRecord(r.e0, s);
  }
  ~ProfScope() {
    if (!active) return;
    (void)hipEventRecord(r.e1, s);
    g_prof.recs.push_back(r);
  }
};

const float* g_dbg_a_scale = nullptr; const float* g_dbg_a_shift = nullptr; const float* g_dbg_resid = nullptr;
float* g_dbg_cstat = nullptr;
unsigned long long* g_qnet_stamps = nullptr;

constexpr int NUM_CU = 256;
constexpr int SK_MAX = 16;
constexpr int NLL_ROWS_PER_BLOCK = 4;
constexpr int LN_ROWS_PER_BLOCK = 8;
constexpr int HEAD_ROWS_PER_BLOCK = HEAD_ROWS;

struct Tune {
  int tile_map[4] = {TILE_64x128, TILE_64x64, TILE_64x128, TILE_64x64};
  int tile_map_short[4] = {TILE_64x64, TILE_64x64, TILE_64x128, TILE_64x64};
  int vbwd_tile_short = -1;
  int l0_kernel = 1;
  int l0_tile = -1;
  int skinny = 7;
  int skinny_pipelined = -1, skinny_pipelined_max_h = 768;
  int dw0_slabs = 16;
  int iql_fold = 1;
  int gemm_lds_pad = 0, gemm_lds_pad_min_blocks = 0;
  int iql_pad_value = 18432, iql_pad_policy = 0, iql_pad_min_blocks = 4 * NUM_CU, iql_pad_min_k = 0;
  int enc_tile_n96 = 0;
  int enc_gemm_sb = 1;
  int enc_patch_rows = 0;
  int enc_s2d = 0;
  int enc_bf16_operands_only = 0;
  int enc_pconv_mfma = 0;
  int enc_bn_sweep = 0;
  int enc_dense_patch = 0;
  int qnet_fused = 1;
  int qnet_rows16 = 1;
  int qnet_wgrad_share = 11;
  int qnet_two_groups = 1;
} g_tune;

enum TuneClamp { TC_ANY, TC_BOOL, TC_NONNEG, TC_1_16, TC_MASK };
struct TuneKey { const char* key; int Tune::*field; TuneClamp clamp; };
#define TK(key, clamp) {#key, &Tune::key, clamp}
const TuneKey k_tune_keys[] = {
    TK(gemm_lds_pad, TC_NONNEG), TK(gemm_lds_pad_min_blocks, TC_NONNEG), TK(iql_pad_value, TC_NONNEG), TK(iql_pad_policy, TC_NONNEG),
    TK(iql_pad_min_blocks, TC_NONNEG), TK(iql_pad_min_k, TC_NONNEG), TK(qnet_fused, TC_BOOL), TK(qnet_two_groups, TC_BOOL),
    TK(qnet_wgrad_share, TC_1_16), TK(qnet_rows16, TC_BOOL), TK(enc_dense_patch, TC_BOOL), TK(enc_s2d, TC_BOOL), TK(enc_patch_rows, TC_NONNEG),
    TK(enc_gemm_sb, TC_ANY), TK(enc_tile_n96, TC_BOOL), TK(enc_bn_sweep, TC_BOOL), TK(enc_pconv_mfma, TC_BOOL), TK(enc_bf16_operands_only, TC_BOOL),
    TK(iql_fold, TC_BOOL), TK(skinny, TC_MASK), TK(skinny_pipelined, TC_MASK), TK(skinny_pipelined_max_h, TC_ANY), TK(dw0_slabs, TC_1_16),
    TK(l0_tile, TC_ANY), TK(l0_kernel, TC_BOOL), TK(vbwd_tile_short, TC_ANY),
};

int tune_apply(Tune& t, const char* key, int value) {
  if (!key) PORL_FAIL(PORL_ERR_INVALID, "null key");
  for (const TuneKey& k : k_tune_keys) {
    if (strcmp(key, k.key)) continue;
    const TuneClamp c = k.clamp;
    t.*k.field = c == TC_BOOL ? value != 0 : c == TC_NONNEG ? std::max(0, value) : c == TC_1_16 ? std::max(1, std::min(value, 16))
               : c == TC_MASK && value == 1 ? 7 : value;
    return PORL_OK;
  }
  const bool sh = !strncmp(key, "tile_map_short", 14);
  const char* i = key + (sh ? 14 : 8);
  if (!strncmp(key, "tile_map", 8) && *i >= '0' && *i <= '3' && !i[1] && value >= 0 && value < TILE_COUNT) {
    (sh ? t.tile_map_short : t.tile_map)[*i - '0'] = value;
    return PORL_OK;
  }
  PORL_FAIL(PORL_ERR_INVALID, "unknown tuning key '%s'", key);
}

inline int64_t ru4(int64_t x) { return (x + 3) & ~int64_t(3); }
inline int cdiv(int a, int b) { return (a + b - 1) / b; }

struct TensorInfo { int64_t off; int rows, cols; };

struct MlpLayout {
  int n_lin = 0;
  int dims[PORL_MAX_HIDDEN + 2] = {0};
  int64_t w[PORL_MAX_HIDDEN + 1] = {0}, b[PORL_MAX_HIDDEN + 1] = {0};
  int64_t lnw[PORL_MAX_HIDDEN] = {0}, lnb[PORL_MAX_HIDDEN] = {0};
  bool ln = false;
};

int64_t add_tensor(std::vector<TensorInfo>& v, int64_t& cur, int rows, int cols) {
  const int64_t off = cur;
  v.push_back({off, rows, cols});
  cur += ru4((int64_t)(rows ? rows : 1) * cols);
  return off;
}

void layout_mlp(MlpLayout& m, std::vector<TensorInfo>& v, int64_t& cur, int in, int hid, int L, int out, bool ln) {
  m.n_lin = L + 1;
  m.ln = ln;
  m.dims[0] = in;
  for (int l = 0; l < L; ++l) m.dims[l + 1] = hid;
  m.dims[L + 1] = out;
  for (int l = 0; l <= L; ++l) {
    m.w[l] = add_tensor(v, cur, m.dims[l + 1], m.dims[l]);
    m.b[l] = add_tensor(v, cur, 0, m.dims[l + 1]);
    if (ln && l < L) {
      m.lnw[l] = add_tensor(v, cur, 0, hid);
      m.lnb[l] = add_tensor(v, cur, 0, hid);
    }
  }
}

struct Workspace {
  int64_t xs_slot[PORL_IQL_SLOTS], xt_slot[PORL_IQL_SLOTS], target_v_slot[PORL_IQL_SLOTS];
  int64_t xn, rew, term;
  int64_t act_v[2][PORL_MAX_HIDDEN], act_t[2][2], act_p[PORL_MAX_HIDDEN];
  int64_t dz_v[2][2], dz_p[2];
  int64_t hp_t[2], hp_v[2];
  int64_t act_q[2][2], hp_q[2];
  int64_t dv[2], dmu;
  int64_t slab_mean, slab_a, slab_b, slab_pa;
  int64_t part_loss, part_min, part_dls;
  int64_t xhat_v[2][PORL_MAX_HIDDEN], rstd_v[2][PORL_MAX_HIDDEN];
  int64_t ln_dg[2], ln_db[2], ln_dh[2];
  int64_t head_part[2], head_loss, head_db[2];
  int64_t pol_w;
  int64_t total;
};

}

struct porl_iql {
  porl_iql_cfg cfg;
  MlpLayout v[2], pol;
  int64_t logstd_off = 0, n_vf = 0, n_pol = 0;
  std::vector<TensorInfo> t_vf, t_pol;
  porl_iql_buffers buf{};
  bool bound = false;
  int device = -1;
  int mode = 0;
  int slot = 0;
  ReduceArgs fin_v{}, fin_p{};
  bool fin_v_pending = false, fin_p_pending = false;
  int batch = 0;
  bool have_pol_target = false;
  bool pol_prefetched = false;
  bool pol_fwd_done = false;
  int pol_nslab = 1;
  int Sp = 0, Dp = 0, Hp = 0, parts_max = 0;
  Workspace ws{};
  Tune tune = g_tune;
};

namespace {

int pick_tile(const GemmGroup& g, const Tune& t, bool short_blocks = false) {
  int minM = 1 << 30, minN = 1 << 30, maxK = 0;
  for (int i = 0; i < g.nprob; ++i) {
    minM = std::min(minM, g.p[i].M); minN = std::min(minN, g.p[i].N); maxK = std::max(maxK, g.p[i].K);
  }
  if (maxK <= 128) return TILE_64x64;
  auto blocks = [&](int tile) {
    int bm, bn, n = 0;
    tile_dims(tile, bm, bn);
    for (int i = 0; i < g.nprob; ++i) n += cdiv(g.p[i].M, bm) * cdiv(g.p[i].N, bn) * std::max(1, g.p[i].splitk);
    return n;
  };
  int cand[3], nc = 0;
  if (minN <= 64 && minM <= 64) { cand[nc++] = TILE_64x64; }
  else if (minN <= 64) { cand[nc++] = TILE_128x64; cand[nc++] = TILE_64x64; }
  else if (minM <= 64) { cand[nc++] = TILE_64x128; cand[nc++] = TILE_64x64; }
  else { cand[nc++] = TILE_128x128; cand[nc++] = TILE_128x64; cand[nc++] = TILE_64x64; }
  const int* map = short_blocks ? t.tile_map_short : t.tile_map;
  for (int i = 0; i < nc; ++i)
    if (blocks(cand[i]) >= NUM_CU) return map[cand[i]];
  return map[cand[nc - 1]];
}

int pick_splitk(int M, int N, int K, int nprob, int bm, int bn) {
  const int tiles = nprob * cdiv(M, bm) * cdiv(N, bn);
  int sk = cdiv(NUM_CU, tiles);
  sk = std::min(sk, std::max(1, K / 64));
  return std::max(1, std::min(sk, SK_MAX));
}

int launch_group(GemmGroup& g, int tile, const Tune& t, hipStream_t s, int iql_pad = -1) {
  const bool iql = iql_pad >= 0 && !t.gemm_lds_pad && g.nprob > 0 && g.p[0].K >= t.iql_pad_min_k;
  g.lds_pad = iql ? iql_pad : t.gemm_lds_pad;
  g.lds_pad_min_blocks = iql ? t.iql_pad_min_blocks : t.gemm_lds_pad_min_blocks;
  double flops = 0.0, bytes = 0.0;
  std::string label;
  if (g_prof.on) {
    bool vec = true, apro = false;
    for (int i = 0; i < g.nprob; ++i) {
      const GemmProb& p = g.p[i];
      flops += 2.0 * p.M * p.N * p.K;
      bytes += 4.0 * ((double)p.M * p.K + (double)p.N * p.K + (p.store_c ? (double)p.M * p.N : 0.0));
      vec = vec && p.a_vec && p.b_vec;
      apro = apro || p.apro != APRO_NONE;
    }
    int bm, bn;
    tile_dims(tile, bm, bn);
    const TileCfg tc = tile_cfg(tile);
    label = "gemm_f32_kernel<" + std::to_string(bm) + "," + std::to_string(bn) + "," + std::to_string(GEMM_BK) + "," +
            std::to_string(tc.wm) + "," + std::to_string(tc.wn) + "," + (vec ? "true" : "false") + "," +
            (apro ? "true" : "false") + (g.single_buffer && vec && tile == TILE_64x64 ? ",true>" : ">");
  }
  ProfScope ps(label, s, flops, bytes);
  hipError_t e = launch_gemm_group(tile, g, s);
  if (e != hipSuccess) {
    g_err = std::string("gemm launch: ") + hipGetErrorString(e);
    return (int)e;
  }
  return 0;
}

int launch_group_bf16(GemmGroup& g, int tile, hipStream_t s) {
  double flops = 0.0, bytes = 0.0;
  std::string label;
  if (g_prof.on) {
    for (int i = 0; i < g.nprob; ++i) {
      const GemmProb& p = g.p[i];
      flops += 2.0 * p.M * p.N * p.K;
      bytes += 4.0 * ((double)p.M * p.K + (double)p.N * p.K + (double)p.M * p.N * (p.resid ? 2.0 : 1.0));
    }
    int bm, bn;
    tile_dims(tile, bm, bn);
    label = "gemm_bf16_kernel<" + std::to_string(bm) + "," + std::to_string(bn) + "," +
            (g.p[0].apro != APRO_NONE ? "true" : "false") + ">";
  }
  ProfScope ps(label, s, flops, bytes);
  hipError_t e = launch_gemm_bf16_group(tile, g, s);
  if (e != hipSuccess) {
    g_err = std::string("bf16 gemm launch: ") + hipGetErrorString(e);
    return (int)e;
  }
  return 0;
}

int launch_reduce(ReduceArgs& r, hipStream_t s) {
  if (r.njobs == 0) return 0;
  long maxn = 0;
  for (int i = 0; i < r.njobs; ++i) maxn = std::max(maxn, r.job[i].n);
  dim3 grid((unsigned)std::min<long>((maxn + 31) / 32, 2048), r.njobs);
  ProfScope ps("multi_reduce_kernel", s, 0.0, 0.0);
  hipLaunchKernelGGL(multi_reduce_kernel, grid, dim3(256), 0, s, r);
  PORL_HIP(hipGetLastError());
  return 0;
}

void add_reduce(ReduceArgs& r, float* out, const float* slab, long n, long stride, int nslab, int op = 0,
                float scale = 1.f) {
  ReduceJob& j = r.job[r.njobs++];
  j.out = out; j.slab = slab; j.bias = nullptr; j.n = n; j.stride = stride; j.nslab = nslab; j.ncols = 1; j.act = 0;
  j.op = op; j.scale = scale; j.adam_off = -1;
  j.width = nslab > 64 ? 4 : 32;
}

int check_ready(const porl_iql* h, bool need_batch) {
  if (!h) PORL_FAIL(PORL_ERR_INVALID, "null engine");
  if (!h->bound) PORL_FAIL(PORL_ERR_UNBOUND, "porl_iql_bind() has not been called");
  if (need_batch && h->batch <= 0) PORL_FAIL(PORL_ERR_INVALID, "no minibatch loaded (porl_iql_load_batch)");
  return 0;
}

bool short_blocks(const porl_iql* h) { return (h->mode & PORL_IQL_MODE_SHORT_BLOCKS) != 0; }
int skinny_mask(const porl_iql* h) {
  const Tune& t = h->tune;
  if (!short_blocks(h)) return t.skinny;
  return t.skinny_pipelined >= 0 ? t.skinny_pipelined : h->cfg.hidden_dim <= t.skinny_pipelined_max_h ? t.skinny : 0;
}
int iql_tile(const porl_iql* h, const GemmGroup& g) { return pick_tile(g, h->tune, short_blocks(h)); }

int iql_launch(const porl_iql* h, GemmGroup& g, int tile, bool policy, hipStream_t s) {
  const Tune& t = h->tune;
  return launch_group(g, tile, t, s, !short_blocks(h) ? -1 : policy ? t.iql_pad_policy : t.iql_pad_value);
}

constexpr int MAX_FWD_NETS = 5;
struct FwdNet {
  const float* in; int ldin;
  const float* W; const float* b;
  float* out;
  const float* headw; float* headout;
  const float* ln_g = nullptr; const float* ln_b = nullptr;
  float* xhat = nullptr; float* rstd = nullptr;
};

int fwd_hidden_layer(porl_iql* h, const FwdNet* nets, int nnets, int B, int K, bool last, int* parts_out, bool policy,
                     hipStream_t s) {
  const int H = h->cfg.hidden_dim;
  if (h->tune.l0_kernel && K <= L0_KP && nnets <= L0_MAX_NETS) {
    L0Args a{};
    a.nnets = nnets; a.B = B; a.H = H; a.K = K; a.ldw = K; a.ldo = h->Hp;
    bool plain = true;
    for (int n = 0; n < nnets; ++n) {
      plain = plain && !nets[n].ln_g && nets[n].out && !(last && nets[n].headw);
      a.net[n] = L0Net{nets[n].in, nets[n].W, nets[n].b, nets[n].out, nets[n].ldin};
    }
    if (plain && l0_fwd_supported(a)) {
      if (parts_out) *parts_out = head_parts(H, 0);
      ProfScope ps("l0_fwd_kernel", s, 2.0 * nnets * B * (double)H * K, 4.0 * nnets * ((double)B * K + (double)H * K + (double)B * H));
      PORL_HIP(launch_l0_fwd(a, s));
      return 0;
    }
  }
  GemmGroup g{};
  g.nprob = nnets;
  bool any_ln = false;
  for (int n = 0; n < nnets; ++n) {
    const bool ln = nets[n].ln_g != nullptr;
    any_ln = any_ln || ln;
    GemmProb p = make_prob(GEMM_NT, nets[n].in, nets[n].ldin, nets[n].W, K, nets[n].out, h->Hp, B, H, K);
    p.bias = nets[n].b;
    p.act = ln ? ACT_NONE : ACT_RELU;
    p.store_c = nets[n].out != nullptr;
    if (ln && !nets[n].out) PORL_FAIL(PORL_ERR_INVALID, "LayerNorm needs a pre-activation buffer");
    if (!ln && last && nets[n].headw) { p.headw = nets[n].headw; p.headout = nets[n].headout; }
    g.p[n] = p;
  }
  const int tile = (K <= 128 && h->tune.l0_tile >= 0) ? h->tune.l0_tile : iql_tile(h, g);
  if (parts_out) *parts_out = any_ln ? 1 : head_parts(H, tile);
  PORL_TRY(iql_launch(h, g, tile, policy, s));
  if (any_ln) {
    LnFwdArgs a{};
    for (int n = 0; n < nnets; ++n) {
      if (!nets[n].ln_g) continue;
      const int k = a.nnets++;
      a.Z[k] = nets[n].out; a.xhat[k] = nets[n].xhat; a.rstd[k] = nets[n].rstd;
      a.gamma[k] = nets[n].ln_g; a.beta[k] = nets[n].ln_b;
      a.headw[k] = last ? nets[n].headw : nullptr; a.headb[k] = nullptr; a.headout[k] = nets[n].headout;
    }
    a.B = B; a.H = H; a.ld = h->Hp; a.rows_per_block = LN_ROWS_PER_BLOCK;
    hipLaunchKernelGGL(ln_relu_fwd_kernel, dim3(cdiv(B, LN_ROWS_PER_BLOCK), a.nnets), dim3(256), 0, s, a);
    PORL_HIP(hipGetLastError());
  }
  return 0;
}

}

extern "C" {

int porl_abi_version(void) { return PORL_ABI_VERSION; }
const char* porl_last_error(void) { return g_err.c_str(); }

int porl_iql_create(const porl_iql_cfg* c, porl_iql** out) {
  if (!c || !out) PORL_FAIL(PORL_ERR_INVALID, "null argument");
  if (c->obs_dim < 1 || c->pol_out_dim < 1 || c->hidden_dim < 1 || c->max_batch < 1)
    PORL_FAIL(PORL_ERR_INVALID, "dimensions must be positive");
  if (c->n_hidden < 1 || c->n_hidden > PORL_MAX_HIDDEN) PORL_FAIL(PORL_ERR_INVALID, "n_hidden must be in [1,%d]", PORL_MAX_HIDDEN);
  if (c->pol_out_dim > 64 * NLL_MAX_COLS_PER_LANE) PORL_FAIL(PORL_ERR_UNSUPPORTED, "pol_out_dim > %d", 64 * NLL_MAX_COLS_PER_LANE);
  if (c->layer_norm && c->hidden_dim > 256 * LN_MAX_COLS)
    PORL_FAIL(PORL_ERR_UNSUPPORTED, "layer_norm with hidden_dim > %d", 256 * LN_MAX_COLS);
  porl_iql* h = new porl_iql();
  h->cfg = *c;
  const int S = c->obs_dim, D = c->pol_out_dim, H = c->hidden_dim, L = c->n_hidden, B = c->max_batch;
  int64_t cur = 0;
  layout_mlp(h->v[0], h->t_vf, cur, S, H, L, 1, c->layer_norm != 0);
  layout_mlp(h->v[1], h->t_vf, cur, S, H, L, 1, c->layer_norm != 0);
  h->n_vf = cur;
  cur = 0;
  h->logstd_off = add_tensor(h->t_pol, cur, 0, D);
  layout_mlp(h->pol, h->t_pol, cur, S, H, L, D, false);
  h->n_pol = cur;

  h->Sp = (int)ru4(S); h->Dp = (int)ru4(D); h->Hp = (int)ru4(H);
  h->parts_max = 0;
  for (int tile = 0; tile < TILE_COUNT; ++tile) h->parts_max = std::max(h->parts_max, head_parts(H, tile));
  Workspace& w = h->ws;
  int64_t o = 0;
  auto take = [&](int64_t n) { int64_t r = o; o += ru4(n); return r; };
  const int64_t BH = (int64_t)B * h->Hp;
  for (int k = 0; k < PORL_IQL_SLOTS; ++k) {
    w.xs_slot[k] = take((int64_t)B * h->Sp); w.xt_slot[k] = take((int64_t)B * h->Dp); w.target_v_slot[k] = take(B);
  }
  w.xn = take((int64_t)B * h->Sp);
  w.rew = take(B); w.term = take(B);
  for (int i = 0; i < 2; ++i) {
    for (int l = 0; l < L; ++l) w.act_v[i][l] = take(BH);
    w.act_t[i][0] = take(BH); w.act_t[i][1] = take(BH);
    w.act_q[i][0] = take(BH); w.act_q[i][1] = take(BH);
    w.hp_q[i] = take((int64_t)h->parts_max * B);
    w.dz_v[i][0] = take(BH); w.dz_v[i][1] = take(BH);
    w.hp_t[i] = take((int64_t)h->parts_max * B); w.hp_v[i] = take((int64_t)h->parts_max * B);
    w.dv[i] = take(B);
  }
  for (int l = 0; l < L; ++l) w.act_p[l] = take(BH);
  w.dz_p[0] = take(BH); w.dz_p[1] = take(BH);
  w.dmu = take((int64_t)B * h->Dp);
  w.slab_mean = take((int64_t)SK_MAX * B * h->Dp);
  w.slab_a = take((int64_t)SK_MAX * 2 * ((int64_t)H * S + 2 * H + 8));
  w.slab_b = take((int64_t)SK_MAX * ((int64_t)D * H + D + 8));
  w.slab_pa = take((int64_t)SK_MAX * ((int64_t)H * S + 2 * H + 8));
  const int nblk = cdiv(B, NLL_ROWS_PER_BLOCK);
  w.part_loss = take(nblk); w.part_min = take(nblk); w.part_dls = take((int64_t)nblk * D);
  for (int i = 0; i < 2; ++i) { w.head_part[i] = take((int64_t)cdiv(B, HEAD_ROWS_PER_BLOCK) * H); w.head_db[i] = take(cdiv(B, HEAD_ROWS_PER_BLOCK)); }
  w.head_loss = take(cdiv(B, HEAD_ROWS_PER_BLOCK));
  if (c->layer_norm) {
    const int nln = cdiv(B, LN_ROWS_PER_BLOCK);
    for (int i = 0; i < 2; ++i) {
      for (int l = 0; l < L; ++l) { w.xhat_v[i][l] = take(BH); w.rstd_v[i][l] = take(B); }
      w.ln_dg[i] = take((int64_t)nln * H); w.ln_db[i] = take((int64_t)nln * H); w.ln_dh[i] = take((int64_t)nln * H);
    }
  }
  w.pol_w = take(B);
  w.total = o;
  *out = h;
  return PORL_OK;
}

void porl_iql_destroy(porl_iql* h) { delete h; }

int64_t porl_iql_group_floats(const porl_iql* h, int group) { return !h ? 0 : (group == 0 ? h->n_vf : h->n_pol); }
int32_t porl_iql_group_tensors(const porl_iql* h, int group) {
  return !h ? 0 : (int32_t)(group == 0 ? h->t_vf.size() : h->t_pol.size());
}
int porl_iql_tensor_info(const porl_iql* h, int group, int index, int64_t* offset, int32_t* rows, int32_t* cols) {
  if (!h || group < 0 || group > 1) PORL_FAIL(PORL_ERR_INVALID, "bad group");
  const auto& v = group == 0 ? h->t_vf : h->t_pol;
  if (index < 0 || index >= (int)v.size()) PORL_FAIL(PORL_ERR_INVALID, "tensor index out of range");
  if (offset) *offset = v[index].off;
  if (rows) *rows = v[index].rows;
  if (cols) *cols = v[index].cols;
  return PORL_OK;
}
int64_t porl_iql_workspace_floats(const porl_iql* h) { return h ? h->ws.total : 0; }

int porl_iql_bind(porl_iql* h, const porl_iql_buffers* b) {
  if (!h || !b) PORL_FAIL(PORL_ERR_INVALID, "null argument");
  const void* ptrs[] = {b->params_vf, b->params_tgt, b->params_pol, b->grads_vf, b->grads_pol, b->adam_m_vf,
                        b->adam_v_vf, b->adam_m_pol, b->adam_v_pol, b->workspace, b->stats};
  for (const void* p : ptrs) {
    if (!p) PORL_FAIL(PORL_ERR_INVALID, "null buffer");
    if (!aligned16(p)) PORL_FAIL(PORL_ERR_INVALID, "buffers must be 16-byte aligned");
  }
  h->buf = *b;
  h->bound = true;
  h->device = device_of(b->workspace);
  h->batch = 0;
  return PORL_OK;
}

int porl_iql_load_batch(porl_iql* h, int32_t batch, const float* obs, int64_t obs_rs, const float* next_obs,
                        int64_t next_rs, const float* rew, int64_t rew_rs, const float* term, int64_t term_rs,
                        const float* pol_target, int64_t pt_rs, void* stream) {
  PORL_TRY(check_ready(h, false)); DevGuard _dg(h->device);
  if (batch < 1 || batch > h->cfg.max_batch) PORL_FAIL(PORL_ERR_INVALID, "batch %d outside [1,%d]", batch, h->cfg.max_batch);
  if (!obs || !next_obs || !rew || !term) PORL_FAIL(PORL_ERR_INVALID, "null batch tensor");
  float* W = h->buf.workspace;
  if (h->mode & PORL_IQL_MODE_TWO_SLOTS) h->slot = (h->slot + 1) % PORL_IQL_SLOTS;
  PackArgs a{};
  a.rows = batch;
  auto job = [&](const float* src, int64_t rs, float* dst, int cols, int ld) {
    PackJob& j = a.job[a.njobs++];
    j.src = src; j.dst = dst; j.src_row_stride = rs; j.src_col_stride = 1; j.cols = cols; j.ld = ld;
  };
  job(obs, obs_rs, W + h->ws.xs_slot[h->slot], h->cfg.obs_dim, h->Sp);
  job(next_obs, next_rs, W + h->ws.xn, h->cfg.obs_dim, h->Sp);
  job(rew, rew_rs, W + h->ws.rew, 1, 1);
  job(term, term_rs, W + h->ws.term, 1, 1);
  if (pol_target) job(pol_target, pt_rs, W + h->ws.xt_slot[h->slot], h->cfg.pol_out_dim, h->Dp);
  h->have_pol_target = pol_target != nullptr;
  h->pol_prefetched = false;
  h->pol_fwd_done = false;
  const long n = (long)batch * std::max(h->Sp, h->Dp);
  dim3 grid((unsigned)std::min<long>((n + 255) / 256, 1024), a.njobs);
  hipLaunchKernelGGL(pack_kernel, grid, dim3(256), 0, (hipStream_t)stream, a);
  PORL_HIP(hipGetLastError());
  h->batch = batch;
  return PORL_OK;
}

static int value_backward_ln(porl_iql* h, const porl_iql_hyper* hp, hipStream_t s, ReduceArgs* defer) {
  (void)hp;
  const int B = h->batch, S = h->cfg.obs_dim, H = h->cfg.hidden_dim, L = h->cfg.n_hidden, Hp = h->Hp;
  float* W = h->buf.workspace;
  const Workspace& ws = h->ws;
  const float* Pv = h->buf.params_vf;
  float* Gv = h->buf.grads_vf;
  const int nln = cdiv(B, LN_ROWS_PER_BLOCK);
  for (int l = L - 1; l >= 0; --l) {
    const bool top = l == L - 1;
    const int Kin = l == 0 ? S : H;
    {
      LnBwdArgs a{};
      a.nnets = 2;
      for (int i = 0; i < 2; ++i) {
        a.dH[i] = top ? nullptr : W + ws.dz_v[i][0];
        a.dv[i] = W + ws.dv[i]; a.headw[i] = Pv + h->v[i].w[L];
        a.Hact[i] = W + ws.act_v[i][l]; a.xhat[i] = W + ws.xhat_v[i][l]; a.rstd[i] = W + ws.rstd_v[i][l];
        a.gamma[i] = Pv + h->v[i].lnw[l];
        a.dZ[i] = W + ws.dz_v[i][1];
        a.part_dgamma[i] = W + ws.ln_dg[i]; a.part_dbeta[i] = W + ws.ln_db[i]; a.part_dhead[i] = W + ws.ln_dh[i];
      }
      a.B = B; a.H = H; a.ld = Hp; a.rows_per_block = LN_ROWS_PER_BLOCK;
      hipLaunchKernelGGL(ln_relu_bwd_kernel, dim3(nln, 2), dim3(256), 0, s, a);
      PORL_HIP(hipGetLastError());
      ReduceArgs r{};
      for (int i = 0; i < 2; ++i) {
        add_reduce(r, Gv + h->v[i].lnw[l], W + ws.ln_dg[i], H, H, nln);
        add_reduce(r, Gv + h->v[i].lnb[l], W + ws.ln_db[i], H, H, nln);
        if (top) add_reduce(r, Gv + h->v[i].w[L], W + ws.ln_dh[i], H, H, nln);
      }
      PORL_TRY(launch_reduce(r, s));
    }
    ReduceArgs red{};
    GemmGroup g{};
    for (int i = 0; i < 2; ++i) {
      const float* dz = W + ws.dz_v[i][1];
      const float* in = l == 0 ? W + ws.xs_slot[h->slot] : W + ws.act_v[i][l - 1];
      const int ldin = l == 0 ? h->Sp : Hp;
      GemmProb p = make_prob(GEMM_TN, dz, Hp, in, ldin, Gv + h->v[i].w[l], Kin, H, Kin, B);
      p.colsum = Gv + h->v[i].b[l];
      g.p[g.nprob++] = p;
      if (l > 0)
        g.p[g.nprob++] = make_prob(GEMM_NN, dz, Hp, Pv + h->v[i].w[l], Kin, W + ws.dz_v[i][0], Hp, B, Kin, H);
    }
    const int tile = iql_tile(h, g);
    if (l == 0) {
      int bm, bn;
      tile_dims(tile, bm, bn);
      const int sk = pick_splitk(H, Kin, B, 2, bm, bn);
      if (sk > 1) {
        const int64_t per = (int64_t)H * Kin, perc = H;
        for (int i = 0; i < 2; ++i) {
          float* slabW = W + ws.slab_a + (int64_t)i * SK_MAX * (per + 2 * perc + 8);
          float* slabC = slabW + (int64_t)SK_MAX * per;
          g.p[i].splitk = sk; g.p[i].C = slabW; g.p[i].colsum = slabC;
          add_reduce(red, Gv + h->v[i].w[0], slabW, per, per, sk);
          add_reduce(red, Gv + h->v[i].b[0], slabC, perc, perc, sk);
        }
      }
    }
    PORL_TRY(iql_launch(h, g, tile, false, s));
    if (l == 0 && defer) *defer = red;
    else PORL_TRY(launch_reduce(red, s));
  }
  return PORL_OK;
}

static int feistel_half_bits(int64_t n_rows) {
  int bits = 1;
  while ((int64_t(1) << bits) < n_rows) ++bits;
  return std::max(1, (bits + 1) / 2);
}

int porl_iql_load_batch_sampled(porl_iql* h, int32_t batch, const float* rows, int64_t row_stride, int64_t n_rows,
                                int32_t act_dim, int32_t target_is_action, uint64_t seed, uint64_t step,
                                int64_t* idx_out, void* stream) {
  PORL_TRY(check_ready(h, false)); DevGuard _dg(h->device);
  if (batch < 1 || batch > h->cfg.max_batch) PORL_FAIL(PORL_ERR_INVALID, "batch %d outside [1,%d]", batch, h->cfg.max_batch);
  if (!rows || n_rows < batch || n_rows > (int64_t(1) << 40)) PORL_FAIL(PORL_ERR_INVALID, "need batch <= n_rows");
  const int S = h->cfg.obs_dim, D = h->cfg.pol_out_dim;
  if (row_stride < 2 * (int64_t)S + 2 + act_dim) PORL_FAIL(PORL_ERR_INVALID, "row stride shorter than 2*S+2+A");
  if (target_is_action ? D != act_dim : D != S) PORL_FAIL(PORL_ERR_INVALID, "policy target width mismatch");
  float* W = h->buf.workspace;
  if (h->mode & PORL_IQL_MODE_TWO_SLOTS) h->slot = (h->slot + 1) % PORL_IQL_SLOTS;
  SampledBatchArgs a{};
  a.rows = rows; a.row_stride = (long)row_stride; a.n_rows = n_rows;
  a.batch = batch; a.S = S; a.A = act_dim; a.D = D; a.Sp = h->Sp; a.Dp = h->Dp;
  a.hb = feistel_half_bits(n_rows); a.target_is_action = target_is_action;
  a.seed = seed; a.step = step;
  a.xs = W + h->ws.xs_slot[h->slot]; a.xn = W + h->ws.xn; a.xt = W + h->ws.xt_slot[h->slot]; a.rew = W + h->ws.rew; a.term = W + h->ws.term;
  a.idx_out = idx_out;
  {
    g_phase = "V1.";
    ProfScope ps("sampled_batch_kernel", (hipStream_t)stream, 0.0, 8.0 * batch * (2 * S + 2 + act_dim));
    hipLaunchKernelGGL(sampled_batch_kernel, dim3(cdiv(batch, 4)), dim3(256), 0, (hipStream_t)stream, a);
    g_phase = "";
  }
  PORL_HIP(hipGetLastError());
  h->batch = batch;
  h->have_pol_target = true;
  h->pol_prefetched = false;
  h->pol_fwd_done = false;
  return PORL_OK;
}

int porl_iql_set_mode(porl_iql* h, int32_t mode) {
  if (!h) PORL_FAIL(PORL_ERR_INVALID, "null engine");
  if (mode & ~(PORL_IQL_MODE_TWO_SLOTS | PORL_IQL_MODE_FOLD_COMBINE | PORL_IQL_MODE_SHORT_BLOCKS)) PORL_FAIL(PORL_ERR_INVALID, "unknown mode bits");
  if (h->fin_v_pending || h->fin_p_pending) PORL_FAIL(PORL_ERR_INVALID, "a backward pass is waiting for its apply call");
  h->mode = mode;
  return PORL_OK;
}

int porl_iql_set_stats(porl_iql* h, float* stats) {
  PORL_TRY(check_ready(h, false)); DevGuard _dg(h->device);
  if (!stats) PORL_FAIL(PORL_ERR_INVALID, "null stats");
  h->buf.stats = stats;
  return PORL_OK;
}


struct Dw0Net { const float* dz; float* gw; float* gb; float* slabW; float* slabC; };
static bool dw0_skinny(const porl_iql* h, const Dw0Net* nets, int nnets, const float* X, int ldx, int B, int H, int S, int ldz,
                       ReduceArgs& red, const char* phase, hipStream_t s, int* rc) {
  *rc = 0;
  if (!(skinny_mask(h) & 1) || S > SKN_T || nnets > SKN_MAX_NETS || H % 4 || !skn_ok4(X, ldx) || ldz % 4) return false;
  for (int i = 0; i < nnets; ++i) if (!skn_ok4(nets[i].dz, ldz)) return false;
  WgradSkinnyArgs a{};
  a.nnets = nnets; a.B = B; a.H = H; a.S = S; a.ldz = ldz; a.ldx = ldx; a.ldo = S;
  a.tiles_n = cdiv(H, SKN_T);
  skn_split(cdiv(B, SKN_T), h->tune.dw0_slabs, a.nslab, a.rtiles);
  a.slabW_stride = (long)H * S; a.slabC_stride = H;
  for (int i = 0; i < nnets; ++i) {
    a.net[i] = WgradSkinnyNet{nets[i].dz, X, nets[i].slabW, nets[i].slabC};
    add_reduce(red, nets[i].gw, nets[i].slabW, (long)H * S, (long)H * S, a.nslab);
    add_reduce(red, nets[i].gb, nets[i].slabC, H, H, a.nslab);
  }
  g_phase = phase;
  {
    ProfScope ps("wgrad_skinny_kernel", s, 2.0 * nnets * B * (double)H * S,
                 4.0 * nnets * ((double)B * H + (double)B * S + (double)a.nslab * H * (S + 1)));
    hipLaunchKernelGGL(wgrad_skinny_kernel, dim3(nnets * a.nslab * a.tiles_n), dim3(256), 0, s, a);
  }
  g_phase = "";
  const hipError_t e = hipGetLastError();
  if (e != hipSuccess) { g_err = std::string("wgrad_skinny_kernel: ") + hipGetErrorString(e); *rc = (int)e; }
  return true;
}

static int value_backward_impl(porl_iql* h, const porl_iql_hyper* hp, hipStream_t s, ReduceArgs* defer) {
  const int B = h->batch, S = h->cfg.obs_dim, H = h->cfg.hidden_dim, L = h->cfg.n_hidden, Hp = h->Hp;
  float* W = h->buf.workspace;
  const Workspace& ws = h->ws;
  const float* Pv = h->buf.params_vf;
  const float* Pt = h->buf.params_tgt;
  float* Gv = h->buf.grads_vf;
  int parts = 0;
  const bool LN = h->cfg.layer_norm != 0;

  for (int l = 0; l < L; ++l) {
    FwdNet nets[4];
    const int K = l == 0 ? S : H;
    for (int n = 0; n < 4; ++n) {
      const bool tgt = n < 2;
      const int i = n & 1;
      const float* P = tgt ? Pt : Pv;
      FwdNet& f = nets[n];
      if (l == 0) { f.in = W + (tgt ? ws.xn : ws.xs_slot[h->slot]); f.ldin = h->Sp; }
      else { f.in = W + (tgt ? ws.act_t[i][(l - 1) & 1] : ws.act_v[i][l - 1]); f.ldin = Hp; }
      f.W = P + h->v[i].w[l]; f.b = P + h->v[i].b[l];
      const bool last = l == L - 1;
      f.out = tgt ? ((last && !LN) ? nullptr : W + ws.act_t[i][l & 1]) : W + ws.act_v[i][l];
      f.headw = P + h->v[i].w[L];
      f.headout = W + (tgt ? ws.hp_t[i] : ws.hp_v[i]);
      if (LN) {
        f.ln_g = P + h->v[i].lnw[l]; f.ln_b = P + h->v[i].lnb[l];
        if (!tgt) { f.xhat = W + ws.xhat_v[i][l]; f.rstd = W + ws.rstd_v[i][l]; }
      }
    }
    g_phase = l == 0 ? "V2.L0fwd:" : "V3.fwd:";
    PORL_TRY(fwd_hidden_layer(h, nets, 4, B, K, l == L - 1, &parts, false, s));
  }
  g_phase = "V4.head:";

  if (LN) {
    ValueLossArgs a{};
    for (int i = 0; i < 2; ++i) {
      a.hp_t[i] = W + ws.hp_t[i]; a.hp_v[i] = W + ws.hp_v[i];
      a.b_t[i] = Pt + h->v[i].b[L]; a.b_v[i] = Pv + h->v[i].b[L];
      a.dv[i] = W + ws.dv[i];
      a.db_out[i] = Gv + h->v[i].b[L];
    }
    a.rew = W + ws.rew; a.term = W + ws.term; a.target_v = W + ws.target_v_slot[h->slot]; a.stats = h->buf.stats;
    a.B = B; a.parts = parts; a.tau = hp->tau; a.discount = hp->discount; a.inv_batch = hp->inv_batch;
    hipLaunchKernelGGL(value_loss_kernel, dim3(1), dim3(1024), 0, s, a);
    PORL_HIP(hipGetLastError());
  }

  ReduceArgs red{};
  if (LN) return value_backward_ln(h, hp, s, defer);
  {
    const int nhb = cdiv(B, HEAD_ROWS_PER_BLOCK);
    HeadBwdArgs a{};
    for (int i = 0; i < 2; ++i) {
      a.Hact[i] = W + ws.act_v[i][L - 1]; a.w[i] = Pv + h->v[i].w[L];
      a.dZ[i] = W + ws.dz_v[i][(L - 1) & 1]; a.part_dw[i] = W + ws.head_part[i];
      a.hp_t[i] = W + ws.hp_t[i]; a.hp_v[i] = W + ws.hp_v[i];
      a.b_t[i] = Pt + h->v[i].b[L]; a.b_v[i] = Pv + h->v[i].b[L];
      a.dv[i] = W + ws.dv[i]; a.part_db[i] = W + ws.head_db[i];
      add_reduce(red, Gv + h->v[i].w[L], W + ws.head_part[i], H, H, nhb);
      add_reduce(red, Gv + h->v[i].b[L], W + ws.head_db[i], 1, 1, nhb);
    }
    a.rew = W + ws.rew; a.term = W + ws.term; a.target_v = W + ws.target_v_slot[h->slot]; a.part_loss = W + ws.head_loss;
    add_reduce(red, h->buf.stats, W + ws.head_loss, 1, 1, nhb, 0, hp->inv_batch);
    a.B = B; a.H = H; a.ld = Hp; a.parts = parts;
    a.tau = hp->tau; a.discount = hp->discount; a.inv_batch = hp->inv_batch;
    ProfScope ps("relu_head_bwd_kernel", s, 0.0, 16.0 * B * H);
    hipLaunchKernelGGL(relu_head_bwd_kernel, dim3(nhb, 2), dim3(256), 0, s, a);
    PORL_HIP(hipGetLastError());
  }
  for (int l = L - 1; l >= 0; --l) {
    const int Kin = l == 0 ? S : H;
    if (l == 0) {
      Dw0Net dn[2];
      const int64_t per = (int64_t)H * S, perc = H;
      for (int i = 0; i < 2; ++i) {
        float* slabW = W + ws.slab_a + (int64_t)i * SK_MAX * (per + 2 * perc + 8);
        dn[i] = Dw0Net{W + ws.dz_v[i][0], Gv + h->v[i].w[0], Gv + h->v[i].b[0], slabW, slabW + (int64_t)SK_MAX * per};
      }
      int rc = 0;
      if (dw0_skinny(h, dn, 2, W + ws.xs_slot[h->slot], h->Sp, B, H, S, Hp, red, "V6.dW0:", s, &rc)) {
        if (rc) return rc;
        break;
      }
    }
    GemmGroup g{};
    for (int i = 0; i < 2; ++i) {
      const float* dz = W + ws.dz_v[i][l & 1];
      const float* in = l == 0 ? W + ws.xs_slot[h->slot] : W + ws.act_v[i][l - 1];
      const int ldin = l == 0 ? h->Sp : Hp;
      GemmProb p = make_prob(GEMM_TN, dz, Hp, in, ldin, Gv + h->v[i].w[l], Kin, H, Kin, B);
      p.colsum = Gv + h->v[i].b[l];
      g.p[g.nprob++] = p;
      if (l > 0) {
        GemmProb q = make_prob(GEMM_NN, dz, Hp, Pv + h->v[i].w[l], Kin, W + ws.dz_v[i][(l - 1) & 1], Hp, B, Kin, H);
        q.mask = W + ws.act_v[i][l - 1]; q.ldmask = Hp;
        g.p[g.nprob++] = q;
      }
    }
    int tile = iql_tile(h, g);
    if (l > 0 && short_blocks(h) && h->tune.vbwd_tile_short >= 0) tile = h->tune.vbwd_tile_short;
    if (l == 0) {
      int bm, bn;
      tile_dims(tile, bm, bn);
      const int sk = pick_splitk(H, Kin, B, 2, bm, bn);
      if (sk > 1) {
        const int64_t per = (int64_t)H * Kin, perc = H;
        for (int i = 0; i < 2; ++i) {
          float* slabW = W + ws.slab_a + (int64_t)i * SK_MAX * (per + 2 * perc + 8);
          float* slabC = slabW + (int64_t)SK_MAX * per;
          g.p[i].splitk = sk; g.p[i].C = slabW; g.p[i].colsum = slabC;
          add_reduce(red, Gv + h->v[i].w[0], slabW, per, per, sk);
          add_reduce(red, Gv + h->v[i].b[0], slabC, perc, perc, sk);
        }
      }
    }
    g_phase = l == 0 ? "V6.dW0:" : "V5.bwd:";
    PORL_TRY(iql_launch(h, g, tile, false, s));
  }
  g_phase = "V7.combine:";
  if (defer) *defer = red;
  else PORL_TRY(launch_reduce(red, s));
  g_phase = "";
  return PORL_OK;
}

int porl_iql_value_backward(porl_iql* h, const porl_iql_hyper* hp, void* stream) {
  PORL_TRY(check_ready(h, true)); DevGuard _dg(h->device);
  if (!hp) PORL_FAIL(PORL_ERR_INVALID, "null hyper-parameters");
  const bool fold = (h->mode & PORL_IQL_MODE_FOLD_COMBINE) != 0;
  h->fin_v = ReduceArgs{};
  PORL_TRY(value_backward_impl(h, hp, (hipStream_t)stream, fold ? &h->fin_v : nullptr));
  h->fin_v_pending = fold;
  return PORL_OK;
}

static int adam_launch(float* p, float* g, float* m, float* v, float* tgt, int64_t n, double lr, int step,
                       double b1, double b2, double eps, double ema_beta, hipStream_t s, const ReduceArgs* fin = nullptr) {
  if (n < 0 || n % 4) PORL_FAIL(PORL_ERR_INVALID, "adam range must be a non-negative multiple of 4 floats");
  if (step < 1) PORL_FAIL(PORL_ERR_INVALID, "adam step must be >= 1");
  if (n == 0 && !(fin && fin->njobs)) return PORL_OK;
  AdamArgs a{};
  a.p = p; a.g = g; a.m = m; a.v = v; a.tgt = tgt;
  const double bc1 = 1.0 - std::pow(b1, (double)step);
  const double bc2 = 1.0 - std::pow(b2, (double)step);
  a.s.step_size = (float)(lr / bc1);
  a.s.bc2_sqrt = (float)std::sqrt(bc2);
  a.s.omb1 = (float)(1.0 - b1); a.s.beta2 = (float)b2; a.s.omb2 = (float)(1.0 - b2);
  a.s.eps = (float)eps; a.s.ema_beta = (float)ema_beta; a.s.omeb = (float)(1.0 - ema_beta);
  a.n4 = n / 4;
  const int sweep_blocks = (int)std::min<long>((a.n4 + 255) / 256, 1 << 20);
  a.span4 = sweep_blocks ? ((a.n4 + sweep_blocks - 1) / sweep_blocks + 255) / 256 * 256 : 256;
  int reduce_blocks = 0;
  double extra_bytes = 0.0;
  if (fin) {
    for (int q = 0; q < fin->njobs; ++q) {
      ReduceJob j = fin->job[q];
      const bool inside = j.out >= g && j.out + j.n <= g + n;
      const long off = inside ? (long)(j.out - g) : -1;
      extra_bytes += 4.0 * (double)j.n * j.nslab;
      const bool plain = j.op == 0 && j.scale == 1.f && !j.bias && j.act == 0;
      if (inside && plain && j.nslab <= ADAM_SWEEP_SLABS && off % 4 == 0 && j.n % 4 == 0 && j.stride % 4 == 0 &&
          aligned16(j.slab) && a.nregions < MAX_ADAM_REGIONS) {
        AdamRegion& R = a.region[a.nregions++];
        R.lo = off; R.hi = off + j.n; R.slab = j.slab; R.stride = j.stride; R.nslab = j.nslab;
        continue;
      }
      if (inside) {
        if (off % 4) PORL_FAIL(PORL_ERR_INVALID, "gradient tensors start on 16-byte boundaries");
        j.adam_off = off;
        a.skip_lo[a.nskip] = off; a.skip_hi[a.nskip] = ru4(off + j.n); ++a.nskip;
      } else {
        j.adam_off = -1;
      }
      a.job_block0[a.r.njobs] = reduce_blocks;
      a.r.job[a.r.njobs++] = j;
      reduce_blocks += (int)((j.n + j.width - 1) / j.width);
    }
    a.job_block0[a.r.njobs] = reduce_blocks;
  }
  ProfScope ps("adam_ema_kernel", s, 0.0, (double)n * (tgt ? 36.0 : 28.0) + extra_bytes);
  a.reduce_blocks = reduce_blocks;
  hipLaunchKernelGGL(adam_ema_kernel, dim3(sweep_blocks + reduce_blocks), dim3(256), 0, s, a);
  PORL_HIP(hipGetLastError());
  return PORL_OK;
}

int porl_iql_value_apply(porl_iql* h, const porl_iql_hyper* hp, void* stream) {
  PORL_TRY(check_ready(h, false)); DevGuard _dg(h->device);
  if (!hp) PORL_FAIL(PORL_ERR_INVALID, "null hyper-parameters");
  g_phase = "V8.";
  const int rc = adam_launch(h->buf.params_vf, h->buf.grads_vf, h->buf.adam_m_vf, h->buf.adam_v_vf, h->buf.params_tgt,
                             h->n_vf, hp->value_lr, hp->value_step, hp->adam_beta1, hp->adam_beta2, hp->adam_eps,
                             hp->ema_beta, (hipStream_t)stream, h->fin_v_pending ? &h->fin_v : nullptr);
  g_phase = "";
  h->fin_v_pending = false;
  return rc;
}

int porl_iql_policy_apply(porl_iql* h, const porl_iql_hyper* hp, void* stream) {
  PORL_TRY(check_ready(h, false)); DevGuard _dg(h->device);
  if (!hp) PORL_FAIL(PORL_ERR_INVALID, "null hyper-parameters");
  g_phase = "P9.";
  const int rc = adam_launch(h->buf.params_pol, h->buf.grads_pol, h->buf.adam_m_pol, h->buf.adam_v_pol, nullptr, h->n_pol,
                             hp->policy_lr, hp->policy_step, hp->adam_beta1, hp->adam_beta2, hp->adam_eps, 0.0,
                             (hipStream_t)stream, h->fin_p_pending ? &h->fin_p : nullptr);
  g_phase = "";
  h->fin_p_pending = false;
  return rc;
}

static int policy_mean_slabs(porl_iql* h, int B, int* nslab, bool policy, hipStream_t s) {
  const int H = h->cfg.hidden_dim, D = h->cfg.pol_out_dim, L = h->cfg.n_hidden;
  float* W = h->buf.workspace;
  if ((skinny_mask(h) & 2) && D <= SKN_T && H % 4 == 0 && skn_ok4(W + h->ws.act_p[L - 1], h->Hp) &&
      skn_ok4(h->buf.params_pol + h->pol.w[L], H) && h->Dp % 4 == 0) {
    MeanSkinnyArgs a{};
    a.A = W + h->ws.act_p[L - 1]; a.W = h->buf.params_pol + h->pol.w[L]; a.slab = W + h->ws.slab_mean;
    a.B = B; a.H = H; a.D = D; a.lda = h->Hp; a.ldw = H; a.ldo = h->Dp;
    a.tiles_m = cdiv(B, SKN_T);
    skn_split(cdiv(H, SKN_T), a.tiles_m >= 16 ? SK_MAX / 2 : SK_MAX, a.nslab, a.ktiles);
    a.slab_stride = (long)B * h->Dp;
    *nslab = a.nslab;
    ProfScope ps("mean_skinny_kernel", s, 2.0 * B * (double)H * D, 4.0 * ((double)B * H + (double)D * H + (double)a.nslab * B * h->Dp));
    hipLaunchKernelGGL(mean_skinny_kernel, dim3(a.tiles_m * a.nslab), dim3(256), 0, s, a);
    PORL_HIP(hipGetLastError());
    return 0;
  }
  GemmGroup g{};
  g.nprob = 1;
  g.p[0] = make_prob(GEMM_NT, W + h->ws.act_p[L - 1], h->Hp, h->buf.params_pol + h->pol.w[L], H, W + h->ws.slab_mean,
                     h->Dp, B, D, H);
  const int tile = iql_tile(h, g);
  int bm, bn;
  tile_dims(tile, bm, bn);
  const int sk = pick_splitk(B, D, H, 1, bm, bn);
  g.p[0].splitk = sk;
  *nslab = sk;
  if (sk == 1) { g.p[0].bias = nullptr; g.p[0].act = ACT_NONE; }
  return iql_launch(h, g, tile, policy, s);
}

int porl_iql_policy_prefetch(porl_iql* h, void* stream) {
  PORL_TRY(check_ready(h, true)); DevGuard _dg(h->device);
  if (!h->have_pol_target) PORL_FAIL(PORL_ERR_INVALID, "policy step needs pol_target in porl_iql_load_batch");
  hipStream_t s = (hipStream_t)stream;
  const int B = h->batch, S = h->cfg.obs_dim, H = h->cfg.hidden_dim, L = h->cfg.n_hidden;
  float* W = h->buf.workspace;
  const Workspace& ws = h->ws;
  const float* Pp = h->buf.params_pol;
  int parts = 0;
  for (int l = 0; l < L; ++l) {
    FwdNet f{};
    if (l == 0) { f.in = W + ws.xs_slot[h->slot]; f.ldin = h->Sp; }
    else { f.in = W + ws.act_p[l - 1]; f.ldin = h->Hp; }
    f.W = Pp + h->pol.w[l]; f.b = Pp + h->pol.b[l];
    f.out = W + ws.act_p[l]; f.headw = nullptr; f.headout = nullptr;
    PORL_TRY(fwd_hidden_layer(h, &f, 1, B, l == 0 ? S : H, l == L - 1, &parts, false, s));
  }
  PORL_TRY(policy_mean_slabs(h, B, &h->pol_nslab, false, s));
  h->pol_prefetched = true;
  return PORL_OK;
}

static int policy_backward_impl(porl_iql* h, const porl_iql_hyper* hp, hipStream_t s, ReduceArgs* defer, int part = 3,
                                bool only_policy = false) {
  if (!h->have_pol_target) PORL_FAIL(PORL_ERR_INVALID, "policy step needs pol_target in porl_iql_load_batch");
  const int B = h->batch, S = h->cfg.obs_dim, H = h->cfg.hidden_dim, L = h->cfg.n_hidden, D = h->cfg.pol_out_dim;
  const int Hp = h->Hp, Dp = h->Dp;
  float* W = h->buf.workspace;
  const Workspace& ws = h->ws;
  const float* Pv = h->buf.params_vf;
  const float* Pp = h->buf.params_pol;
  float* Gp = h->buf.grads_pol;
  int parts = 0;
  const bool LN = h->cfg.layer_norm != 0;

  const int nblk = cdiv(B, NLL_ROWS_PER_BLOCK);
  if (part == 2 && !h->pol_fwd_done) PORL_FAIL(PORL_ERR_INVALID, "porl_iql_policy_forward has not run for this batch");
  if ((part & 1) && !h->pol_fwd_done) {
  const bool pre = h->pol_prefetched;
  const bool pre_weight = only_policy;
  h->pol_prefetched = false;
  if (only_policy) {
    const float* Pt = h->buf.params_tgt;
    for (int l = 0; l < L; ++l) {
      FwdNet nets[MAX_FWD_NETS];
      const int K = l == 0 ? S : H;
      const bool last = l == L - 1;
      for (int n = 0; n < 4; ++n) {
        const bool tgt = n < 2;
        const int i = n & 1;
        const float* P = tgt ? Pt : Pv;
        const int64_t* act = tgt ? ws.act_t[i] : ws.act_q[i];
        FwdNet& f = nets[n];
        if (l == 0) { f.in = W + (tgt ? ws.xn : ws.xs_slot[h->slot]); f.ldin = h->Sp; }
        else { f.in = W + act[(l - 1) & 1]; f.ldin = Hp; }
        f.W = P + h->v[i].w[l]; f.b = P + h->v[i].b[l];
        f.out = (last && !LN) ? nullptr : W + act[l & 1];
        f.headw = P + h->v[i].w[L]; f.headout = W + (tgt ? ws.hp_t[i] : ws.hp_q[i]);
        if (LN) { f.ln_g = P + h->v[i].lnw[l]; f.ln_b = P + h->v[i].lnb[l]; }
      }
      int first = 4;
      if (!pre) {
        FwdNet& f = nets[4];
        if (l == 0) { f.in = W + ws.xs_slot[h->slot]; f.ldin = h->Sp; }
        else { f.in = W + ws.act_p[l - 1]; f.ldin = Hp; }
        f.W = Pp + h->pol.w[l]; f.b = Pp + h->pol.b[l];
        f.out = W + ws.act_p[l]; f.headw = nullptr; f.headout = nullptr;
        first = 5;
      }
      g_phase = l == 0 ? "O1.L0fwd:" : "O2.fwd:";
      PORL_TRY(fwd_hidden_layer(h, nets, first, B, K, last, &parts, true, s));
    }
    g_phase = "O3.head:";
    PolicyWeightArgs a{};
    for (int i = 0; i < 2; ++i) {
      a.hp_t[i] = W + ws.hp_t[i]; a.hp_v[i] = W + ws.hp_q[i];
      a.b_t[i] = Pt + h->v[i].b[L]; a.b_v[i] = Pv + h->v[i].b[L];
    }
    a.rew = W + ws.rew; a.term = W + ws.term; a.target_v = W + ws.target_v_slot[h->slot]; a.weight = W + ws.pol_w;
    a.B = B; a.parts = parts; a.weight_mode = h->cfg.weight_mode; a.discount = hp->discount; a.alpha = hp->alpha;
    {
      ProfScope ps("policy_weight_kernel", s, 0.0, 4.0 * B * (4.0 * parts + 4.0));
      hipLaunchKernelGGL(policy_weight_kernel, dim3(cdiv(B, PW_ROWS_PER_BLOCK)), dim3(256), 0, s, a);
    }
    PORL_HIP(hipGetLastError());
  }
  for (int l = 0; l < L && !only_policy; ++l) {
    FwdNet nets[3];
    const int K = l == 0 ? S : H;
    const bool last = l == L - 1;
    for (int i = 0; i < 2; ++i) {
      FwdNet& f = nets[i];
      if (l == 0) { f.in = W + ws.xs_slot[h->slot]; f.ldin = h->Sp; }
      else { f.in = W + ws.act_q[i][(l - 1) & 1]; f.ldin = Hp; }
      f.W = Pv + h->v[i].w[l]; f.b = Pv + h->v[i].b[l];
      f.out = (last && !LN) ? nullptr : W + ws.act_q[i][l & 1];
      f.headw = Pv + h->v[i].w[L]; f.headout = W + ws.hp_q[i];
      if (LN) { f.ln_g = Pv + h->v[i].lnw[l]; f.ln_b = Pv + h->v[i].lnb[l]; }
    }
    FwdNet& f = nets[2];
    if (l == 0) { f.in = W + ws.xs_slot[h->slot]; f.ldin = h->Sp; }
    else { f.in = W + ws.act_p[l - 1]; f.ldin = Hp; }
    f.W = Pp + h->pol.w[l]; f.b = Pp + h->pol.b[l];
    f.out = W + ws.act_p[l]; f.headw = nullptr; f.headout = nullptr;
    g_phase = l == 0 ? "P1.L0fwd:" : "P2.fwd:";
    PORL_TRY(fwd_hidden_layer(h, nets, pre ? 2 : 3, B, K, last, &parts, true, s));
  }
  int nslab = h->pol_nslab;
  g_phase = only_policy ? "O4.mean:" : "P3.mean:";
  if (!pre) PORL_TRY(policy_mean_slabs(h, B, &nslab, true, s));
  g_phase = only_policy ? "O5." : "P4.";

  {
    PolicyNllArgs a{};
    for (int i = 0; i < 2; ++i) { a.hp_v[i] = W + ws.hp_q[i]; a.b_v[i] = Pv + h->v[i].b[L]; }
    a.parts = pre_weight ? 0 : parts; a.target_v = W + ws.target_v_slot[h->slot];
    a.weight = pre_weight ? W + ws.pol_w : nullptr;
    a.mean_slab = W + ws.slab_mean; a.nslab = nslab; a.slab_stride = (long)B * Dp;
    a.mean_bias = Pp + h->pol.b[L]; a.log_std = Pp + h->logstd_off;
    a.x = W + ws.xt_slot[h->slot]; a.ldx = Dp; a.dmean = W + ws.dmu; a.ldd = Dp;
    a.part_loss = W + ws.part_loss; a.part_min = W + ws.part_min; a.part_dls = W + ws.part_dls;
    a.B = B; a.D = D; a.ldm = Dp; a.tanh_mean = h->cfg.pol_tanh; a.weight_mode = h->cfg.weight_mode;
    a.alpha = hp->alpha; a.inv_batch = hp->inv_batch; a.rows_per_block = NLL_ROWS_PER_BLOCK;
    ProfScope ps("policy_nll_kernel", s, 0.0, 4.0 * B * (nslab + 2.0) * Dp);
    hipLaunchKernelGGL(policy_nll_kernel, dim3(nblk), dim3(256), 0, s, a);
    PORL_HIP(hipGetLastError());
  }
  g_phase = "";
  h->pol_fwd_done = true;
  }
  if (!(part & 2)) return PORL_OK;
  h->pol_fwd_done = false;

  ReduceArgs red{};
  add_reduce(red, Gp + h->logstd_off, W + ws.part_dls, D, D, nblk);
  add_reduce(red, h->buf.stats + 1, W + ws.part_loss, 1, 1, nblk);
  add_reduce(red, h->buf.stats + 2, W + ws.part_min, 1, 1, nblk,  1);
  if ((skinny_mask(h) & 4) && D <= SKN_T && H % 4 == 0 && Dp % 4 == 0 && Hp % 4 == 0 && skn_ok4(Pp + h->pol.w[L], H)) {
    OutBwdArgs a{};
    a.dmu = W + ws.dmu; a.W = Pp + h->pol.w[L]; a.A = W + ws.act_p[L - 1];
    a.dZ = W + ws.dz_p[(L - 1) & 1];
    a.slabW = W + ws.slab_b; a.slabC = a.slabW + (int64_t)SK_MAX * D * H;
    a.B = B; a.H = H; a.D = D; a.lddmu = Dp; a.ldw = H; a.lda = Hp; a.lddz = Hp;
    a.tiles_n = cdiv(H, SKN_T);
    skn_split(cdiv(B, SKN_T), SK_MAX, a.nslab, a.rtiles);
    a.slabW_stride = (long)D * H; a.slabC_stride = D;
    add_reduce(red, Gp + h->pol.w[L], a.slabW, (long)D * H, (long)D * H, a.nslab);
    add_reduce(red, Gp + h->pol.b[L], a.slabC, D, D, a.nslab);
    g_phase = "P5.outbwd:";
    {
      ProfScope ps("out_bwd_kernel", s, 4.0 * B * (double)H * D, 4.0 * (2.0 * B * H + (double)B * D + (double)D * H + (double)a.nslab * D * H));
      hipLaunchKernelGGL(out_bwd_kernel, dim3(a.nslab * a.tiles_n), dim3(256), 0, s, a);
    }
    g_phase = "";
    PORL_HIP(hipGetLastError());
  } else {
    GemmGroup g{};
    g.nprob = 2;
    g.p[0] = make_prob(GEMM_TN, W + ws.dmu, Dp, W + ws.act_p[L - 1], Hp, Gp + h->pol.w[L], H, D, H, B);
    g.p[0].colsum = Gp + h->pol.b[L];
    g.p[1] = make_prob(GEMM_NN, W + ws.dmu, Dp, Pp + h->pol.w[L], H, W + ws.dz_p[(L - 1) & 1], Hp, B, H, D);
    g.p[1].mask = W + ws.act_p[L - 1]; g.p[1].ldmask = Hp;
    const int tile = D <= 64 ? TILE_64x128 : iql_tile(h, g);
    int bm, bn;
    tile_dims(tile, bm, bn);
    const int sk = pick_splitk(D, H, B, 1, bm, bn);
    if (sk > 1) {
      float* slabW = W + ws.slab_b;
      float* slabC = slabW + (int64_t)SK_MAX * D * H;
      g.p[0].splitk = sk; g.p[0].C = slabW; g.p[0].colsum = slabC;
      add_reduce(red, Gp + h->pol.w[L], slabW, (long)D * H, (long)D * H, sk);
      add_reduce(red, Gp + h->pol.b[L], slabC, D, D, sk);
    }
    g_phase = "P5.outbwd:";
    PORL_TRY(iql_launch(h, g, tile, true, s));
  }
  for (int l = L - 1; l >= 0; --l) {
    const int Kin = l == 0 ? S : H;
    if (l == 0) {
      const int64_t per = (int64_t)H * S;
      float* slabW = W + ws.slab_pa;
      Dw0Net dn{W + ws.dz_p[0], Gp + h->pol.w[0], Gp + h->pol.b[0], slabW, slabW + (int64_t)SK_MAX * per};
      int rc = 0;
      if (dw0_skinny(h, &dn, 1, W + ws.xs_slot[h->slot], h->Sp, B, H, S, Hp, red, "P7.dW0:", s, &rc)) {
        if (rc) return rc;
        break;
      }
    }
    const float* dz = W + ws.dz_p[l & 1];
    const float* in = l == 0 ? W + ws.xs_slot[h->slot] : W + ws.act_p[l - 1];
    const int ldin = l == 0 ? h->Sp : Hp;
    GemmGroup g{};
    g.p[g.nprob] = make_prob(GEMM_TN, dz, Hp, in, ldin, Gp + h->pol.w[l], Kin, H, Kin, B);
    g.p[g.nprob++].colsum = Gp + h->pol.b[l];
    if (l > 0) {
      GemmProb q = make_prob(GEMM_NN, dz, Hp, Pp + h->pol.w[l], Kin, W + ws.dz_p[(l - 1) & 1], Hp, B, Kin, H);
      q.mask = W + ws.act_p[l - 1]; q.ldmask = Hp;
      g.p[g.nprob++] = q;
    }
    const int tile = iql_tile(h, g);
    if (l == 0) {
      int bm, bn;
      tile_dims(tile, bm, bn);
      const int sk = pick_splitk(H, Kin, B, 1, bm, bn);
      if (sk > 1) {
        const int64_t per = (int64_t)H * Kin;
        float* slabW = W + ws.slab_pa;
        float* slabC = slabW + (int64_t)SK_MAX * per;
        g.p[0].splitk = sk; g.p[0].C = slabW; g.p[0].colsum = slabC;
        add_reduce(red, Gp + h->pol.w[0], slabW, per, per, sk);
        add_reduce(red, Gp + h->pol.b[0], slabC, H, H, sk);
      }
    }
    g_phase = l == 0 ? "P7.dW0:" : "P6.bwd:";
    PORL_TRY(iql_launch(h, g, tile, true, s));
  }
  g_phase = "P8.combine:";
  if (defer) *defer = red;
  else PORL_TRY(launch_reduce(red, s));
  g_phase = "";
  return PORL_OK;
}

int porl_iql_policy_forward(porl_iql* h, const porl_iql_hyper* hp, void* stream) {
  PORL_TRY(check_ready(h, true)); DevGuard _dg(h->device);
  if (!hp) PORL_FAIL(PORL_ERR_INVALID, "null hyper-parameters");
  return policy_backward_impl(h, hp, (hipStream_t)stream, nullptr, 1);
}

int porl_iql_policy_backward(porl_iql* h, const porl_iql_hyper* hp, void* stream) {
  PORL_TRY(check_ready(h, true)); DevGuard _dg(h->device);
  if (!hp) PORL_FAIL(PORL_ERR_INVALID, "null hyper-parameters");
  const bool fold = (h->mode & PORL_IQL_MODE_FOLD_COMBINE) != 0;
  h->fin_p = ReduceArgs{};
  PORL_TRY(policy_backward_impl(h, hp, (hipStream_t)stream, fold ? &h->fin_p : nullptr));
  h->fin_p_pending = fold;
  return PORL_OK;
}

int porl_iql_step(porl_iql* h, const porl_iql_hyper* hp, void* stream) {
  PORL_TRY(check_ready(h, true)); DevGuard _dg(h->device);
  if (!hp) PORL_FAIL(PORL_ERR_INVALID, "null hyper-parameters");
  hipStream_t s = (hipStream_t)stream;
  ReduceArgs fin{};
  PORL_TRY(value_backward_impl(h, hp, s, h->tune.iql_fold ? &fin : nullptr));
  g_phase = "V8.";
  PORL_TRY(adam_launch(h->buf.params_vf, h->buf.grads_vf, h->buf.adam_m_vf, h->buf.adam_v_vf, h->buf.params_tgt, h->n_vf,
                       hp->value_lr, hp->value_step, hp->adam_beta1, hp->adam_beta2, hp->adam_eps, hp->ema_beta, s, &fin));
  fin = ReduceArgs{};
  PORL_TRY(policy_backward_impl(h, hp, s, h->tune.iql_fold ? &fin : nullptr));
  g_phase = "P9.";
  PORL_TRY(adam_launch(h->buf.params_pol, h->buf.grads_pol, h->buf.adam_m_pol, h->buf.adam_v_pol, nullptr, h->n_pol,
                       hp->policy_lr, hp->policy_step, hp->adam_beta1, hp->adam_beta2, hp->adam_eps, 0.0, s, &fin));
  g_phase = "";
  return PORL_OK;
}

int porl_iql_policy_only_forward(porl_iql* h, const porl_iql_hyper* hp, void* stream) {
  PORL_TRY(check_ready(h, true)); DevGuard _dg(h->device);
  if (!hp) PORL_FAIL(PORL_ERR_INVALID, "null hyper-parameters");
  h->pol_fwd_done = false;
  return policy_backward_impl(h, hp, (hipStream_t)stream, nullptr, 1, true);
}

int porl_iql_policy_only_step(porl_iql* h, const porl_iql_hyper* hp, void* stream) {
  PORL_TRY(check_ready(h, true)); DevGuard _dg(h->device);
  if (!hp) PORL_FAIL(PORL_ERR_INVALID, "null hyper-parameters");
  if (!h->have_pol_target) PORL_FAIL(PORL_ERR_INVALID, "policy step needs pol_target in porl_iql_load_batch");
  hipStream_t s = (hipStream_t)stream;
  h->pol_fwd_done = false;
  ReduceArgs fin{};
  PORL_TRY(policy_backward_impl(h, hp, s, h->tune.iql_fold ? &fin : nullptr, 3, true));
  g_phase = "O9.";
  PORL_TRY(adam_launch(h->buf.params_pol, h->buf.grads_pol, h->buf.adam_m_pol, h->buf.adam_v_pol, nullptr, h->n_pol,
                       hp->policy_lr, hp->policy_step, hp->adam_beta1, hp->adam_beta2, hp->adam_eps, 0.0, s, &fin));
  g_phase = "";
  return PORL_OK;
}

static int pack_x(porl_iql* h, const float* x, int64_t x_rs, int batch, int64_t dst_off, hipStream_t s) {
  if (!x) PORL_FAIL(PORL_ERR_INVALID, "null input");
  if (batch < 1 || batch > h->cfg.max_batch) PORL_FAIL(PORL_ERR_INVALID, "batch %d outside [1,%d]", batch, h->cfg.max_batch);
  PackArgs a{};
  a.rows = batch; a.njobs = 1;
  a.job[0].src = x; a.job[0].dst = h->buf.workspace + dst_off; a.job[0].src_row_stride = x_rs;
  a.job[0].src_col_stride = 1; a.job[0].cols = h->cfg.obs_dim; a.job[0].ld = h->Sp;
  const long n = (long)batch * h->Sp;
  hipLaunchKernelGGL(pack_kernel, dim3((unsigned)std::min<long>((n + 255) / 256, 1024), 1), dim3(256), 0, s, a);
  PORL_HIP(hipGetLastError());
  return PORL_OK;
}

static int small_fwd(int nnets, const float* const* Wt, const float* const* bias, const float* const* X, const long* ldx,
                     float* const* Y, const long* ldy, int N, int K, int B, int act, hipStream_t s) {
  SmallFwdArgs a{};
  for (int i = 0; i < nnets; ++i) { a.W[i] = Wt[i]; a.bias[i] = bias[i]; a.X[i] = X[i]; a.ldx[i] = ldx[i]; a.Y[i] = Y[i]; a.ldy[i] = ldy[i]; }
  a.N = N; a.K = K; a.B = B; a.act = act;
  const size_t lds = sizeof(float) * (size_t)B * K;
  if (lds > 64 * 1024) PORL_FAIL(PORL_ERR_UNSUPPORTED, "small-batch path: B*K too large");
  ProfScope ps("small_fwd_kernel", s, 2.0 * nnets * B * N * K, 4.0 * nnets * ((double)N * K + B * (N + K)));
  hipLaunchKernelGGL(small_fwd_kernel, dim3(std::min(cdiv(N, 4), 1024), nnets), dim3(256), lds, s, a);
  PORL_HIP(hipGetLastError());
  return PORL_OK;
}

int porl_iql_forward_value(porl_iql* h, int which, const float* x, int64_t x_rs, int32_t batch, float* v1_out,
                           float* v2_out, void* stream) {
  PORL_TRY(check_ready(h, false)); DevGuard _dg(h->device);
  if (!v1_out || !v2_out) PORL_FAIL(PORL_ERR_INVALID, "null output");
  hipStream_t s = (hipStream_t)stream;
  if (batch >= 1 && batch <= SMALL_FWD_MAX_B && !h->cfg.layer_norm && x) {
    const int S = h->cfg.obs_dim, H = h->cfg.hidden_dim, L = h->cfg.n_hidden;
    float* W = h->buf.workspace;
    const float* P = which ? h->buf.params_tgt : h->buf.params_vf;
    const float* in[2] = {x, x};
    long ldin[2] = {(long)x_rs, (long)x_rs};
    for (int l = 0; l <= L; ++l) {
      const float* Wt[2] = {P + h->v[0].w[l], P + h->v[1].w[l]};
      const float* bs[2] = {P + h->v[0].b[l], P + h->v[1].b[l]};
      float* out[2];
      long ldo[2];
      for (int i = 0; i < 2; ++i) {
        out[i] = l == L ? (i ? v2_out : v1_out) : W + h->ws.act_t[i][l & 1];
        ldo[i] = l == L ? 1 : h->Hp;
      }
      PORL_TRY(small_fwd(2, Wt, bs, in, ldin, out, ldo, l == L ? 1 : H, l == 0 ? S : H, batch, l == L ? ACT_NONE : ACT_RELU, s));
      for (int i = 0; i < 2; ++i) { in[i] = out[i]; ldin[i] = ldo[i]; }
    }
    return PORL_OK;
  }
  PORL_TRY(pack_x(h, x, x_rs, batch, h->ws.xn, s));
  h->batch = 0;
  const int S = h->cfg.obs_dim, H = h->cfg.hidden_dim, L = h->cfg.n_hidden;
  float* W = h->buf.workspace;
  const float* P = which ? h->buf.params_tgt : h->buf.params_vf;
  int parts = 0;
  for (int l = 0; l < L; ++l) {
    FwdNet nets[2];
    for (int i = 0; i < 2; ++i) {
      FwdNet& f = nets[i];
      if (l == 0) { f.in = W + h->ws.xn; f.ldin = h->Sp; }
      else { f.in = W + h->ws.act_t[i][(l - 1) & 1]; f.ldin = h->Hp; }
      f.W = P + h->v[i].w[l]; f.b = P + h->v[i].b[l];
      const bool LN = h->cfg.layer_norm != 0;
      f.out = (l == L - 1 && !LN) ? nullptr : W + h->ws.act_t[i][l & 1];
      f.headw = P + h->v[i].w[L]; f.headout = W + h->ws.hp_t[i];
      if (LN) { f.ln_g = P + h->v[i].lnw[l]; f.ln_b = P + h->v[i].lnb[l]; }
    }
    PORL_TRY(fwd_hidden_layer(h, nets, 2, batch, l == 0 ? S : H, l == L - 1, &parts, false, s));
  }
  hipLaunchKernelGGL(head_finish_kernel, dim3(cdiv(batch, 256)), dim3(256), 0, s, W + h->ws.hp_t[0], W + h->ws.hp_t[1],
                     P + h->v[0].b[L], P + h->v[1].b[L], parts, batch, v1_out, v2_out);
  PORL_HIP(hipGetLastError());
  return PORL_OK;
}

int porl_iql_forward_policy(porl_iql* h, const float* x, int64_t x_rs, int32_t batch, float* mean_out,
                            int64_t mean_rs, void* stream) {
  PORL_TRY(check_ready(h, false)); DevGuard _dg(h->device);
  if (!mean_out) PORL_FAIL(PORL_ERR_INVALID, "null output");
  hipStream_t s = (hipStream_t)stream;
  if (batch >= 1 && batch <= SMALL_FWD_MAX_B && x) {
    const int S = h->cfg.obs_dim, H = h->cfg.hidden_dim, L = h->cfg.n_hidden, D = h->cfg.pol_out_dim;
    float* W = h->buf.workspace;
    const float* P = h->buf.params_pol;
    const float* in[1] = {x};
    long ldin[1] = {(long)x_rs};
    for (int l = 0; l <= L; ++l) {
      const float* Wt[1] = {P + h->pol.w[l]};
      const float* bs[1] = {P + h->pol.b[l]};
      float* out[1] = {l == L ? mean_out : W + h->ws.act_t[0][l & 1]};
      long ldo[1] = {l == L ? (long)mean_rs : (long)h->Hp};
      const int act = l < L ? ACT_RELU : (h->cfg.pol_tanh ? ACT_TANH : ACT_NONE);
      PORL_TRY(small_fwd(1, Wt, bs, in, ldin, out, ldo, l == L ? D : H, l == 0 ? S : H, batch, act, s));
      in[0] = out[0]; ldin[0] = ldo[0];
    }
    return PORL_OK;
  }
  PORL_TRY(pack_x(h, x, x_rs, batch, h->ws.xn, s));
  h->batch = 0;
  const int S = h->cfg.obs_dim, H = h->cfg.hidden_dim, L = h->cfg.n_hidden, D = h->cfg.pol_out_dim;
  float* W = h->buf.workspace;
  const float* P = h->buf.params_pol;
  for (int l = 0; l < L; ++l) {
    FwdNet f{};
    if (l == 0) { f.in = W + h->ws.xn; f.ldin = h->Sp; }
    else { f.in = W + h->ws.act_p[l - 1]; f.ldin = h->Hp; }
    f.W = P + h->pol.w[l]; f.b = P + h->pol.b[l]; f.out = W + h->ws.act_p[l];
    PORL_TRY(fwd_hidden_layer(h, &f, 1, batch, l == 0 ? S : H, false, nullptr, false, s));
  }
  int nslab = 1;
  PORL_TRY(policy_mean_slabs(h, batch, &nslab, false, s));
  const long n = (long)batch * D;
  hipLaunchKernelGGL(mean_finish_kernel, dim3((unsigned)std::min<long>((n + 255) / 256, 1024)), dim3(256), 0, s,
                     W + h->ws.slab_mean, nslab, (long)batch * h->Dp, batch, D, h->Dp, P + h->pol.b[L],
                     h->cfg.pol_tanh, mean_out, (long)mean_rs);
  PORL_HIP(hipGetLastError());
  return PORL_OK;
}

int porl_gemm_f32(int mode, int tile, int32_t M, int32_t N, int32_t K, const float* A, int32_t lda, const float* B,
                  int32_t ldb, float* C, int32_t ldc, const float* bias, int act, const float* mask, int32_t ldmask,
                  int splitk, float* slab, void* stream) {
  if (mode < 0 || mode > 2) PORL_FAIL(PORL_ERR_INVALID, "mode must be 0..2");
  if (M < 1 || N < 1 || K < 0 || !A || !B || !C) PORL_FAIL(PORL_ERR_INVALID, "bad GEMM arguments");
  if (splitk > 1 && !slab) PORL_FAIL(PORL_ERR_INVALID, "splitk > 1 needs a slab buffer");
  if (splitk > 1 && ldc != N) PORL_FAIL(PORL_ERR_INVALID, "splitk > 1 needs a dense C (ldc == N)");
  DevGuard _dg(device_of(C));
  hipStream_t s = (hipStream_t)stream;
  GemmGroup g{};
  g.nprob = 1;
  g.p[0] = make_prob(mode, A, lda, B, ldb, C, ldc, M, N, K);
  if (tile < 0) tile = pick_tile(g, g_tune);
  if (tile >= TILE_COUNT) PORL_FAIL(PORL_ERR_INVALID, "tile must be -1..%d", TILE_COUNT - 1);
  if (splitk > 1) {
    g.p[0].splitk = splitk; g.p[0].C = slab;
    PORL_TRY(launch_group(g, tile, g_tune, s));
    if (mask) PORL_FAIL(PORL_ERR_UNSUPPORTED, "mask with splitk");
    const long n = (long)M * ldc;
    hipLaunchKernelGGL(slab_reduce_kernel, dim3((unsigned)std::min<long>((n + 255) / 256, 1024)), dim3(256), 0, s, C, slab,
                       splitk, n, n, bias, ldc, act);
// ... 141 lines not shown
  hipLaunchKernelGGL(sample_indices_kernel, dim3(cdiv(batch, 256)), dim3(256), 0, (hipStream_t)stream, n_rows, batch,
                     seed, step, hb, base, (int64_t)0, out);
  PORL_HIP(hipGetLastError());
  return PORL_OK;
}

int porl_epoch_indices(int64_t n_rows, int64_t first, int32_t count, uint64_t seed, uint64_t epoch, int64_t base,
                       int64_t* out, void* stream) {
  if (n_rows < 1 || count < 1 || first < 0 || first + count > n_rows || !out)
    PORL_FAIL(PORL_ERR_INVALID, "need 0 <= first, 1 <= count, first + count <= n_rows");
  if (n_rows > (int64_t(1) << 40)) PORL_FAIL(PORL_ERR_INVALID, "n_rows too large");
  const int hb = feistel_half_bits(n_rows);
  DevGuard _dg(device_of(out));
  hipLaunchKernelGGL(sample_indices_kernel, dim3(cdiv(count, 256)), dim3(256), 0, (hipStream_t)stream, n_rows, count,
                     seed, epoch, hb, base, first, out);
  PORL_HIP(hipGetLastError());
  return PORL_OK;
}

int porl_per_update(double* tree, int64_t capacity, const int64_t* tree_idx, const double* td_error, int32_t n, double eps,
                    double alpha, int32_t* stamp, void* stream) {
  if (!tree || !tree_idx || !td_error || !stamp || capacity < 1 || n < 0) PORL_FAIL(PORL_ERR_INVALID, "bad arguments");
  if (n == 0) return PORL_OK;
  DevGuard _dg(device_of(tree));
  hipStream_t s = (hipStream_t)stream;
  hipLaunchKernelGGL(per_stamp_kernel, dim3(cdiv(n, 256)), dim3(256), 0, s, tree_idx, n, capacity, stamp);
  hipLaunchKernelGGL(per_set_leaves_kernel, dim3(cdiv(n, 256)), dim3(256), 0, s, tree, tree_idx, td_error, n, capacity, eps,
                     alpha, stamp);
  int levels = 0;
  for (int64_t v = 2 * capacity - 1; v > 1; v >>= 1) ++levels;
  hipLaunchKernelGGL(per_propagate_kernel, dim3(1), dim3(1024), 0, s, tree, tree_idx, n, levels);
  PORL_HIP(hipGetLastError());
  return PORL_OK;
}

int porl_per_sample(const double* tree, int64_t capacity, const double* u, int32_t batch, int64_t n_entries, double beta,
                    int64_t* out_idx, double* out_prio, float* out_w, void* stream) {
  if (!tree || !u || !out_idx || !out_prio || !out_w || capacity < 1 || batch < 1 || n_entries < 1)
    PORL_FAIL(PORL_ERR_INVALID, "bad arguments");
  DevGuard _dg(device_of(tree));
  PerSampleArgs a{tree, capacity, u, batch, n_entries, beta, out_idx, out_prio, out_w};
  hipLaunchKernelGGL(per_sample_kernel, dim3(1), dim3(256), 0, (hipStream_t)stream, a);
  PORL_HIP(hipGetLastError());
  return PORL_OK;
}

static int per_levels(int64_t capacity) {
  int levels = 0;
  for (int64_t v = 2 * capacity - 1; v > 1; v >>= 1) ++levels;
  return levels;
}

int porl_per_record(double* tree, int64_t capacity, int64_t slot, double td_error, double eps, double alpha,
                    const float* state, const float* next_state, int32_t state_dim, int64_t action, float reward,
                    float done, const porl_qnet_mirror* store, void* stream) {
  if (!tree || !state || !next_state || !store || !store->states || !store->next_states || !store->actions ||
      !store->rewards || !store->dones)
    PORL_FAIL(PORL_ERR_INVALID, "null argument");
  if (capacity < 1 || store->capacity != capacity)
    PORL_FAIL(PORL_ERR_INVALID, "capacity %lld < 1 or the store holds %lld rows", (long long)capacity, (long long)store->capacity);
  if (state_dim < 1) PORL_FAIL(PORL_ERR_INVALID, "state_dim %d < 1", state_dim);
  if (state_dim > ONL_MAX_RECORD_S)
    PORL_FAIL(PORL_ERR_UNSUPPORTED, "state_dim %d > %d: too wide for the kernel arguments", state_dim, ONL_MAX_RECORD_S);
  if (slot < 0 || slot >= capacity) PORL_FAIL(PORL_ERR_INVALID, "slot %lld outside [0,%lld)", (long long)slot, (long long)capacity);
  DevGuard _dg(device_of(tree));
  PerRecordArgs a;
  a.states = store->states; a.next_states = store->next_states; a.actions = store->actions; a.rewards = store->rewards;
  a.dones = store->dones; a.tree = tree; a.capacity = capacity; a.slot = slot; a.action = action;
  a.td_error = td_error; a.eps = eps; a.alpha = alpha; a.reward = reward; a.done = done; a.S = state_dim;
  memcpy(a.x, state, sizeof(float) * state_dim);
  memcpy(a.x + state_dim, next_state, sizeof(float) * state_dim);
  hipLaunchKernelGGL(per_record_kernel, dim3(1), dim3(state_dim > 64 ? 256 : 64), 0, (hipStream_t)stream, a);
  PORL_HIP(hipGetLastError());
  return PORL_OK;
}

int porl_per_sample_slots(const double* tree, int64_t capacity, const double* u, int32_t batch, int64_t n_entries,
                          double beta, int64_t* out_idx, int64_t* out_slots, float* out_w, float* out_wmean,
                          double* scratch, void* stream) {
  if (!tree || !u || !out_idx || !out_slots || !out_w || !out_wmean || !scratch) PORL_FAIL(PORL_ERR_INVALID, "null argument");
  if (capacity < 1 || batch < 1 || n_entries < 1 || n_entries > capacity)
    PORL_FAIL(PORL_ERR_INVALID, "need capacity >= 1, batch >= 1, 1 <= n_entries <= capacity");
  DevGuard _dg(device_of(tree));
  PerSampleSlotsArgs a{tree, capacity, u, batch, n_entries, beta, out_idx, out_slots, out_w, out_wmean, scratch};
  hipLaunchKernelGGL(per_sample_slots_kernel, dim3(1), dim3(256), 0, (hipStream_t)stream, a);
  PORL_HIP(hipGetLastError());
  return PORL_OK;
}

int porl_per_update_f32(double* tree, int64_t capacity, const int64_t* tree_idx, const float* td_abs, int32_t n, double eps,
                        double alpha, int32_t* stamp, void* stream) {
  if (!tree || !tree_idx || !td_abs || !stamp) PORL_FAIL(PORL_ERR_INVALID, "null argument");
  if (capacity < 1 || n < 1) PORL_FAIL(PORL_ERR_INVALID, "need capacity >= 1 and n >= 1");
  DevGuard _dg(device_of(tree));
  const int threads = n >= 1024 ? 1024 : (n + 63) / 64 * 64;
  hipLaunchKernelGGL(per_update_f32_kernel, dim3(1), dim3(threads), 0, (hipStream_t)stream, tree, tree_idx, td_abs, n, capacity,
                     eps, alpha, stamp, per_levels(capacity));
  PORL_HIP(hipGetLastError());
  return PORL_OK;
}

int porl_tune_set(const char* key, int value) { return tune_apply(g_tune, key, value); }

int porl_iql_tune_set(porl_iql* h, const char* key, int value) {
  if (!h) PORL_FAIL(PORL_ERR_INVALID, "null engine");
  return tune_apply(h->tune, key, value);
}

int porl_signal_create(void** out) {
  if (!out) PORL_FAIL(PORL_ERR_INVALID, "null argument");
  int dev = 0, can = 0;
  PORL_HIP(hipGetDevice(&dev));
  PORL_HIP(hipDeviceGetAttribute(&can, hipDeviceAttributeCanUseStreamWaitValue, dev));
  if (!can) PORL_FAIL(PORL_ERR_UNSUPPORTED, "stream wait-value operations are not supported on this device");
  void* p = nullptr;
  PORL_HIP(hipExtMallocWithFlags(&p, 8, hipMallocSignalMemory));
  PORL_HIP(hipMemset(p, 0, 8));
  *out = p;
  return PORL_OK;
}
int porl_signal_destroy(void* sig) {
  if (sig) PORL_HIP(hipFree(sig));
  return PORL_OK;
}
int porl_signal_write(void* sig, uint64_t value, void* stream) {
  if (!sig) PORL_FAIL(PORL_ERR_INVALID, "null signal");
  PORL_HIP(hipStreamWriteValue64((hipStream_t)stream, sig, value, 0));
  return PORL_OK;
}
int porl_signal_wait_ge(void* sig, uint64_t value, void* stream) {
  if (!sig) PORL_FAIL(PORL_ERR_INVALID, "null signal");
  PORL_HIP(hipStreamWaitValue64((hipStream_t)stream, sig, value, hipStreamWaitValueGte, 0xFFFFFFFFFFFFFFFFull));
  return PORL_OK;
}

int porl_iql_update_pipelined(porl_iql* h, const porl_iql_hyper* hp, int32_t batch, const float* rows, int64_t row_stride,
                              int64_t n_rows, int32_t act_dim, int32_t target_is_action, uint64_t seed, uint64_t step,
                              void* sig_value, void* sig_fwd, void* sig_policy, uint64_t seq, uint64_t wait_policy_seq,
                              uint64_t wait_fwd_seq, int32_t write_policy, void* main_stream, void* side_stream) {
  PORL_TRY(check_ready(h, false)); DevGuard _dg(h->device);
  if (!hp) PORL_FAIL(PORL_ERR_INVALID, "null hyper-parameters");
  if (!sig_value || !sig_fwd || !sig_policy || seq < 1) PORL_FAIL(PORL_ERR_INVALID, "three signal counters and seq >= 1 are required");
  if (main_stream == side_stream) PORL_FAIL(PORL_ERR_INVALID, "the two phases need two streams");
  if (!(h->mode & PORL_IQL_MODE_TWO_SLOTS) || !(h->mode & PORL_IQL_MODE_FOLD_COMBINE))
    PORL_FAIL(PORL_ERR_INVALID, "pipelined updates need PORL_IQL_MODE_TWO_SLOTS | PORL_IQL_MODE_FOLD_COMBINE");
  if (batch < 1 || batch > h->cfg.max_batch) PORL_FAIL(PORL_ERR_INVALID, "batch %d outside [1,%d]", batch, h->cfg.max_batch);
  if (!rows || n_rows < batch || n_rows > (int64_t(1) << 40) || act_dim < 0 ||
      row_stride < 2 * (int64_t)h->cfg.obs_dim + 2 + act_dim)
    PORL_FAIL(PORL_ERR_INVALID, "bad replay rows (need batch <= n_rows <= 2^40, row stride >= 2*S+2+A)");
  if (target_is_action ? h->cfg.pol_out_dim != act_dim : h->cfg.pol_out_dim != h->cfg.obs_dim)
    PORL_FAIL(PORL_ERR_INVALID, "policy target width mismatch");
  if (wait_policy_seq) PORL_TRY(porl_signal_wait_ge(sig_policy, wait_policy_seq, main_stream));
  PORL_TRY(porl_iql_load_batch_sampled(h, batch, rows, row_stride, n_rows, act_dim, target_is_action, seed, step, nullptr, main_stream));
  PORL_TRY(porl_iql_value_backward(h, hp, main_stream));
  if (wait_fwd_seq) PORL_TRY(porl_signal_wait_ge(sig_fwd, wait_fwd_seq, main_stream));
  PORL_TRY(porl_iql_value_apply(h, hp, main_stream));
  PORL_TRY(porl_signal_write(sig_value, seq, main_stream));
  PORL_TRY(porl_signal_wait_ge(sig_value, seq, side_stream));
  PORL_TRY(porl_iql_policy_forward(h, hp, side_stream));
  PORL_TRY(porl_signal_write(sig_fwd, seq, side_stream));
  PORL_TRY(porl_iql_policy_backward(h, hp, side_stream));
  PORL_TRY(porl_iql_policy_apply(h, hp, side_stream));
  if (write_policy) PORL_TRY(porl_signal_write(sig_policy, seq, side_stream));
  return PORL_OK;
}

int porl_tune_set_ptr(const char* key, void* ptr) {
  if (!key) PORL_FAIL(PORL_ERR_INVALID, "null key");
  if (!strcmp(key, "qnet_stamps")) { g_qnet_stamps = (unsigned long long*)ptr; return PORL_OK; }
  if (!strcmp(key, "gemm_a_scale")) { g_dbg_a_scale = (const float*)ptr; return PORL_OK; }
  if (!strcmp(key, "gemm_a_shift")) { g_dbg_a_shift = (const float*)ptr; return PORL_OK; }
  if (!strcmp(key, "gemm_resid")) { g_dbg_resid = (const float*)ptr; return PORL_OK; }
  if (!strcmp(key, "gemm_cstat")) { g_dbg_cstat = (float*)ptr; return PORL_OK; }
  PORL_FAIL(PORL_ERR_INVALID, "unknown tuning key '%s'", key);
}

int porl_state2costmap(float* state, int64_t state_rs, int32_t batch, int32_t n_ang, int32_t n_dist, float* out,
                        void* stream) {
  if (!state || !out || batch < 1 || n_ang < 4 || n_dist < 4) PORL_FAIL(PORL_ERR_INVALID, "bad costmap arguments");
  if (batch > 65535) PORL_FAIL(PORL_ERR_INVALID, "batch > 65535");
  DevGuard _dg(device_of(out));
  hipStream_t s = (hipStream_t)stream;
  const double pi = 3.14159265358979323846;
  const float dist_inc = (float)((4.0 + 1e-4) / n_dist);
  const float ang_inc = (float)((2.0 * pi + 1e-4) / n_ang);
  const float deg_min = (float)(-pi + (2.0 * pi + 2e-4) / n_ang), deg_max = (float)(pi - (2.0 * pi + 2e-4) / n_ang);
  const float dist_max = (float)(4.0 - 4.0 / n_dist);
  hipLaunchKernelGGL(costmap_kernel, dim3(n_ang, batch), dim3(std::min(256, n_dist)), 0, s, state, (long)state_rs, n_ang,
                     n_dist, dist_inc, ang_inc, deg_min, deg_max, dist_max, out);
  PORL_HIP(hipGetLastError());
  const long n = (long)batch * (n_ang + 2);
  hipLaunchKernelGGL(clamp_gt8_kernel, dim3((unsigned)std::min<long>((n + 255) / 256, 1024)), dim3(256), 0, s, state,
                     (long)state_rs, n_ang + 2, batch);
  PORL_HIP(hipGetLastError());
  return PORL_OK;
}

int porl_prof_enable(int on) {
  g_prof.on = on != 0;
  g_prof.recs.clear();
  g_prof.pool_used = 0;
  return PORL_OK;
}

int porl_prof_read(porl_prof_entry* out, int max_entries) {
  if (!out || max_entries < 1) PORL_FAIL(PORL_ERR_INVALID, "bad profile buffer");
  PORL_HIP(hipDeviceSynchronize());
  const int nl = std::min<int>((int)g_prof.labels.size(), max_entries);
  for (int i = 0; i < nl; ++i) {
    memset(&out[i], 0, sizeof(out[i]));
    strncpy(out[i].name, g_prof.labels[i].c_str(), sizeof(out[i].name) - 1);
  }
  for (const ProfRec& r : g_prof.recs) {
    if (r.label >= nl) continue;
    float ms = 0.f;
    PORL_HIP(hipEventElapsedTime(&ms, r.e0, r.e1));
    out[r.label].launches += 1;
    out[r.label].total_ms += ms;
    out[r.label].flops += r.flops;
    out[r.label].bytes += r.bytes;
  }
  return nl;
}

}

struct porl_qnet {
  porl_qnet_cfg cfg;
  MlpLayout net;
  int64_t n_params = 0;
  std::vector<TensorInfo> tensors;
  porl_qnet_buffers buf{};
  bool bound = false;
  int device = -1;
  int batch = 0;
  int Sp = 0, Ap = 0, ld[PORL_MAX_HIDDEN + 2] = {0};
  int wld[PORL_MAX_HIDDEN + 1] = {0};
  struct {
    int64_t xs, xn, rew, done, actions;
    int64_t act[PORL_MAX_HIDDEN + 1], tmp[2], dz[2], slab, part_td, part_pen, fslab, total;
    int64_t tmp2[2], row_loss;
    int64_t mask;
  } ws;
  bool fused_ok = false;
  QnetFusedArgs fargs{};
  int fused_lds_bytes = 0;
  int fused2_lds_w2 = 0, fused2_lds_bytes = 0;
  QnetFusedArgs fargs16{};
  int fused16_lds_w2 = 0, fused16_lds_bytes = 0;
  int64_t fslab_stride = 0;
  bool fslab_clean = false;
  bool slab_clean = false;
  Tune tune = g_tune;
  const void* act_out_host = nullptr;
  int32_t* act_out_dev = nullptr;
};


extern "C" {

int porl_qnet_create(const porl_qnet_cfg* c, porl_qnet** out) {
  if (!c || !out) PORL_FAIL(PORL_ERR_INVALID, "null argument");
  if (c->state_dim < 1 || c->n_actions < 1 || c->max_batch < 1) PORL_FAIL(PORL_ERR_INVALID, "dimensions must be positive");
  if (c->n_hidden < 1 || c->n_hidden > PORL_MAX_HIDDEN) PORL_FAIL(PORL_ERR_INVALID, "n_hidden must be in [1,%d]", PORL_MAX_HIDDEN);
  if (c->n_actions > 4096) PORL_FAIL(PORL_ERR_UNSUPPORTED, "more than 4096 outputs");
  porl_qnet* h = new porl_qnet();
  h->cfg = *c;
  const int L = c->n_hidden, B = c->max_batch;
  MlpLayout& m = h->net;
  m.n_lin = L + 1;
  m.dims[0] = c->state_dim;
  for (int l = 0; l < L; ++l) {
    if (c->hidden[l] < 1) { delete h; PORL_FAIL(PORL_ERR_INVALID, "hidden size must be positive"); }
    m.dims[l + 1] = c->hidden[l];
  }
  m.dims[L + 1] = c->n_actions;
  int64_t cur = 0;
  for (int l = 0; l <= L; ++l) {
    const int rows = (m.dims[l + 1] + 31) & ~31;
    h->wld[l] = ((m.dims[l] + 15) & ~15) + 4;
    m.w[l] = cur;
    h->tensors.push_back({cur, m.dims[l + 1], m.dims[l]});
    cur += (int64_t)rows * h->wld[l];
    m.b[l] = cur;
    h->tensors.push_back({cur, 0, m.dims[l + 1]});
    cur += rows;
  }
  h->n_params = cur;
  h->Sp = (int)ru4(c->state_dim);
  h->Ap = (int)ru4(c->n_actions);
  int maxld = h->Ap;
  for (int l = 0; l <= L; ++l) { h->ld[l] = (int)ru4(m.dims[l + 1]); maxld = std::max(maxld, h->ld[l]); }
  int64_t o = 0;
  auto take = [&](int64_t n) { int64_t r = o; o += ru4(n); return r; };
  h->ws.xs = take((int64_t)B * h->Sp); h->ws.xn = take((int64_t)B * h->Sp);
  h->ws.rew = take(B); h->ws.done = take(B); h->ws.actions = take(2 * (int64_t)B);
  for (int l = 0; l <= L; ++l) h->ws.act[l] = take((int64_t)B * h->ld[l]);
  h->ws.tmp[0] = take((int64_t)B * maxld); h->ws.tmp[1] = take((int64_t)B * maxld);
  h->ws.dz[0] = take((int64_t)B * maxld); h->ws.dz[1] = take((int64_t)B * maxld);
  h->ws.slab = take((int64_t)SK_MAX * (cur + 64));
  const int nblk = cdiv(B, 16);
  h->ws.part_td = take(nblk); h->ws.part_pen = take(nblk);
  {
    bool ok = (L + 1 <= QF_MAX_LIN);
    int maxw = 0, wmax = 0;
    for (int l = 0; l <= L + 1 && ok; ++l) { ok = m.dims[l] <= QF_MAX_W; maxw = std::max(maxw, (m.dims[l] + 31) & ~31); }
    QnetFusedArgs& fa = h->fargs;
    int off = 0;
    if (ok) {
      fa.n_lin = L + 1;
      for (int l = 0; l <= L + 1; ++l) {
        fa.dims[l] = m.dims[l];
        fa.lds_act[l] = off;
        off += QF_ROWS * (((m.dims[l] + 31) & ~31) + 4);
// ... 926 lines not shown
```

### porl_amd/engine.py

```python
from __future__ import annotations

import ctypes as C
import math

import numpy as np
import torch

from . import _native as N


def _norm_device(device):
    device = torch.device(device)
    if device.type == "cuda" and device.index is None:
        device = torch.device("cuda", torch.cuda.current_device())
    return device


class IqlEngine:
    GROUP_VF, GROUP_POL = 0, 1
    MODE_TWO_SLOTS, MODE_FOLD_COMBINE, MODE_SHORT_BLOCKS = 1, 2, 4
    SLOTS = 3

    def __init__(self, obs_dim, pol_out_dim, hidden_dim, n_hidden, layer_norm=False, pol_tanh=False,
                 weight_mode=0, max_batch=1024, device="cpu"):
        self.device = _norm_device(device)
        self.cfg = N.IqlCfg(int(obs_dim), int(pol_out_dim), int(hidden_dim), int(n_hidden),
                            int(bool(layer_norm)), int(bool(pol_tanh)), int(weight_mode), int(max_batch))
        self._lib = N.lib()
        h = C.c_void_p()
        N.check(self._lib.porl_iql_create(C.byref(self.cfg), C.byref(h)), "porl_iql_create")
        self._h = h
        self.n_vf = int(self._lib.porl_iql_group_floats(h, 0))
        self.n_pol = int(self._lib.porl_iql_group_floats(h, 1))
        self._bound = False
        self._mode = 0
        self._side = None
        self._policy_done = None
        self._values_read = None
        self._slot_users = [None] * self.SLOTS
        self._events = []
        self._alloc()

    def side_stream(self):
        if self._side is None:
            import os
            self._side = torch.cuda.Stream(device=self.device, priority=int(os.environ.get("PORL_SIDE_PRIORITY", "0")))
        return self._side

    def event(self, i):
        while len(self._events) <= i:
            self._events.append(torch.cuda.Event(enable_timing=False, blocking=False))
        return self._events[i]

    SIG_VALUE, SIG_FWD, SIG_POLICY = 0, 1, 2

    def signals(self):
        if getattr(self, "_signals", None) is None:
            sig = []
            with torch.cuda.device(self.device):
                for _ in range(3):
                    p = C.c_void_p()
                    if self._lib.porl_signal_create(C.byref(p)) != 0:
                        sig = False
                        break
                    sig.append(p)
            self._signals = sig
            self._seq = 0
        return self._signals or None

    def signal(self, which, value, stream):
        N.check(self._lib.porl_signal_write(self.signals()[which], int(value), C.c_void_p(stream.cuda_stream)), "porl_signal_write")

    def wait_signal(self, which, value, stream):
        if value > 0:
            N.check(self._lib.porl_signal_wait_ge(self.signals()[which], int(value), C.c_void_p(stream.cuda_stream)),
                    "porl_signal_wait_ge")

    def join(self):
        ev, self._policy_done, self._values_read = self._policy_done, None, None
        self._slot_users = [None] * self.SLOTS
        if ev is True:
            ev = self.event(3 * self.SLOTS)
            ev.record(self.side_stream())
        if ev is not None:
            torch.cuda.current_stream(self.device).wait_event(ev)

    def wait_slot_free(self):
        ev = self._slot_users[0]
        if ev is not None:
            torch.cuda.current_stream(self.device).wait_event(ev)

    def wait_values_read(self):
        ev, self._values_read = self._values_read, None
        if isinstance(ev, tuple):
            self.wait_signal(self.SIG_FWD, ev[1], torch.cuda.current_stream(self.device))
        elif ev is not None:
            torch.cuda.current_stream(self.device).wait_event(ev)

    def set_mode(self, mode):
        if mode != self._mode:
            N.check(self._lib.porl_iql_set_mode(self._h, int(mode)), "porl_iql_set_mode")
            self._mode = mode

    def tune_set(self, key, value):
        N.check(self._lib.porl_iql_tune_set(self._h, key.encode(), int(value)), "porl_iql_tune_set")

    SLICE_QUANTUM = 4 * 840

    def _alloc(self):
        dev = self.device
        q = self.SLICE_QUANTUM
        z = lambda n: torch.zeros((n + q - 1) // q * q, dtype=torch.float32, device=dev)
        self.params_vf, self.params_tgt, self.params_pol = z(self.n_vf), z(self.n_vf), z(self.n_pol)
        self.grads_vf, self.grads_pol = z(self.n_vf), z(self.n_pol)
        self.adam_m_vf, self.adam_v_vf = z(self.n_vf), z(self.n_vf)
        self.adam_m_pol, self.adam_v_pol = z(self.n_pol), z(self.n_pol)
        self.stats = z(8)
        self.workspace = None
        self._bound = False

    def _ensure_bound(self):
        if self.device.type != "cuda":
            raise N.NativeError("porl_amd computes on a HIP device only (device='cuda'); there is no CPU path")
        if self._bound:
            return
        nws = int(self._lib.porl_iql_workspace_floats(self._h))
        self.workspace = torch.empty(nws, dtype=torch.float32, device=self.device)
        b = N.IqlBuffers(*[C.c_void_p(t.data_ptr()) for t in (
            self.params_vf, self.params_tgt, self.params_pol, self.grads_vf, self.grads_pol,
            self.adam_m_vf, self.adam_v_vf, self.adam_m_pol, self.adam_v_pol, self.workspace, self.stats)])
        N.check(self._lib.porl_iql_bind(self._h, C.byref(b)), "porl_iql_bind")
        self._bound = True
        self._mode = 0
        N.check(self._lib.porl_iql_set_mode(self._h, 0), "porl_iql_set_mode")

    def to(self, device):
        device = _norm_device(device)
        if device == self.device:
            return self
        if self.device.type == "cuda":
            self.join()
            torch.cuda.synchronize(self.device)
            self._free_signals()
        self._side, self._events = None, []
        self._policy_done = self._values_read = None
        for name in ("params_vf", "params_tgt", "params_pol", "grads_vf", "grads_pol", "adam_m_vf",
                     "adam_v_vf", "adam_m_pol", "adam_v_pol", "stats"):
            setattr(self, name, getattr(self, name).to(device))
        self.device = device
        self.workspace = None
        self._bound = False
        return self

    def tensor_table(self, group):
        n = int(self._lib.porl_iql_group_tensors(self._h, group))
        out = []
        off, r, c = C.c_int64(), C.c_int32(), C.c_int32()
        for i in range(n):
            N.check(self._lib.porl_iql_tensor_info(self._h, group, i, C.byref(off), C.byref(r), C.byref(c)))
            out.append((off.value, (c.value,) if r.value == 0 else (r.value, c.value)))
        return out

    @staticmethod
    def views(flat, table):
        return [flat[o:o + math.prod(shape)].view(shape) for o, shape in table]

    @staticmethod
    def _mat(t, cols, what):
        if t.dtype != torch.float32:
            raise RuntimeError(f"{what}: expected float32, got {t.dtype}")
        if t.dim() != 2 or t.shape[1] != cols:
            raise RuntimeError(f"{what}: expected shape (B, {cols}), got {tuple(t.shape)}")
        if t.stride(1) != 1:
# ... 309 lines not shown
```

Measured before the change: 3072 gradient-steps/sec.

## Fuse Adam and EMA update into hidden-layer weight-gradient GEMM epilogue

Adds an optional FUSE variant of the f32 GEMM kernel. For hidden-layer weight-gradient problems it applies Adam, and the target-network EMA where present, in the epilogue. Updated parameters go to a new staging buffer, and the later Adam sweep only copies those ranges back instead of re-reading grads, m and v. The aim is to avoid a separate full pass over the largest H×H parameter blocks. In exchange it adds a new GEMM instantiation, extra workspace and stricter eligibility checks. It also rewrites the Adam and EMA arithmetic into explicit fma/rounded forms, which may change numerics slightly. The fused path is gated by new tuning flags that default to 0, so it may not run by default.

```diff
diff --git a/include/porl_hip.h b/include/porl_hip.h
--- a/include/porl_hip.h
+++ b/include/porl_hip.h
@@ -73,6 +73,7 @@
 #define PORL_IQL_MODE_TWO_SLOTS 1
 #define PORL_IQL_MODE_FOLD_COMBINE 2
 #define PORL_IQL_MODE_SHORT_BLOCKS 4
+#define PORL_IQL_MODE_FUSED_ADAM 8
 int porl_iql_set_mode(porl_iql* h, int32_t mode);
 
 int porl_iql_set_stats(porl_iql* h, float* stats);
diff --git a/porl_amd/agent/_iql.py b/porl_amd/agent/_iql.py
--- a/porl_amd/agent/_iql.py
+++ b/porl_amd/agent/_iql.py
@@ -188,7 +188,7 @@
             eng.join()
         eng._ensure_bound()
         eng.set_mode(((IqlEngine.MODE_TWO_SLOTS | IqlEngine.MODE_SHORT_BLOCKS) if pipelined else 0) |
-                     (IqlEngine.MODE_FOLD_COMBINE if not dp else 0))
+                     ((IqlEngine.MODE_FOLD_COMBINE | IqlEngine.MODE_FUSED_ADAM) if not dp else 0))
         use_sig = pipelined and _PIPE_SYNC in ("signal", "signal2") and eng.signals() is not None
         onecall = _PIPE_ONECALL is True or _PIPE_ONECALL == "1" or (
             _PIPE_ONECALL == "auto" and (batch or 0) * eng.cfg.hidden_dim ** 2 <= _ONECALL_MAX_WORK)
diff --git a/porl_amd/csrc/gemm_f32.hpp b/porl_amd/csrc/gemm_f32.hpp
--- a/porl_amd/csrc/gemm_f32.hpp
+++ b/porl_amd/csrc/gemm_f32.hpp
@@ -1,6 +1,7 @@
 #pragma once
 #include <hip/hip_runtime.h>
 #include <stdint.h>
+#include "kernels.hpp"
 
 #ifndef PORL_ABL
 #define PORL_ABL 0
@@ -30,6 +31,7 @@
   const float* rscale;
   float* cstat;
   int rs_rows, rs_row0;
+  const float* ad_p; float* ad_p_next; float* ad_m; float* ad_v; float* ad_tgt;
   int a_grp, a_grp_jump, a_seg_tiles, a_seg_jump;
   int M, N, K;
   int lda, ldb, ldc, ldmask;
@@ -50,6 +52,7 @@
   int single_buffer;
   GemmProb p[MAX_GROUP];
   int lds_pad, lds_pad_min_blocks;
+  AdamScalars ad;
 };
 
 typedef float f32x16 __attribute__((ext_vector_type(16)));
@@ -95,7 +98,7 @@
 __device__ unsigned long long g_stamps[16 * 4096];
 #endif
 
-template <int BM, int BN, int BK, int WM, int WN, bool VEC, bool APRO, bool ONEBUF = false>
+template <int BM, int BN, int BK, int WM, int WN, bool VEC, bool APRO, bool ONEBUF = false, bool FUSE = false>
 __global__ __launch_bounds__(64 * WM * WN) void gemm_f32_kernel(const GemmGroup g) {
   constexpr int THREADS = 64 * WM * WN;
   constexpr int WTM = BM / WM / 32;
@@ -660,6 +663,24 @@
         v.z = __fadd_rn(x4.z, __fmul_rn(v.z, rs)); v.w = __fadd_rn(x4.w, __fmul_rn(v.w, rs));
       }
       *reinterpret_cast<float4*>(Cg + (size_t)(wr0 + r) * P.ldc + wc0 + c) = v;
+      if constexpr (FUSE) {
+        if (P.ad_p) {
+          const size_t e = (size_t)(wr0 + r) * P.ldc + wc0 + c;
+          float4 pp = *reinterpret_cast<const float4*>(P.ad_p + e);
+          float4 mm = *reinterpret_cast<const float4*>(P.ad_m + e), vv = *reinterpret_cast<const float4*>(P.ad_v + e);
+          adam1(pp.x, v.x, mm.x, vv.x, g.ad); adam1(pp.y, v.y, mm.y, vv.y, g.ad);
+          adam1(pp.z, v.z, mm.z, vv.z, g.ad); adam1(pp.w, v.w, mm.w, vv.w, g.ad);
+          *reinterpret_cast<float4*>(P.ad_p_next + e) = pp;
+          *reinterpret_cast<float4*>(P.ad_m + e) = mm;
+          *reinterpret_cast<float4*>(P.ad_v + e) = vv;
+          if (P.ad_tgt) {
+            float4 tt = *reinterpret_cast<const float4*>(P.ad_tgt + e);
+            tt.x = ema1(tt.x, pp.x, g.ad.omeb, g.ad.ema_beta); tt.y = ema1(tt.y, pp.y, g.ad.omeb, g.ad.ema_beta);
+            tt.z = ema1(tt.z, pp.z, g.ad.omeb, g.ad.ema_beta); tt.w = ema1(tt.w, pp.w, g.ad.omeb, g.ad.ema_beta);
+            *reinterpret_cast<float4*>(P.ad_tgt + e) = tt;
+          }
+        }
+      }
     }
   }
 #ifdef PORL_STAMP
@@ -743,11 +764,29 @@
 inline hipError_t launch_tile(const GemmGroup& g, hipStream_t s) {
   dim3 grid(g.total_blocks), block(64 * WM * WN);
   const int pad = g.total_blocks >= g.lds_pad_min_blocks ? g.lds_pad : 0;
-  bool vec = true, apro = g.p[0].apro != APRO_NONE;
+  bool vec = true, apro = g.p[0].apro != APRO_NONE, fuse = false;
   for (int i = 0; i < g.nprob; ++i) {
     vec = vec && g.p[i].a_vec && g.p[i].b_vec;
+    fuse = fuse || g.p[i].ad_p != nullptr;
     if ((g.p[i].apro != APRO_NONE) != apro) return hipErrorInvalidValue;
     if (g.p[i].splitk <= 1 && (g.p[i].mask || g.p[i].resid) && (g.p[i].cstat || g.p[i].headw)) return hipErrorInvalidValue;
+  }
+  if (fuse) {
+    if (apro || !vec || g.single_buffer) return hipErrorInvalidValue;
+    for (int i = 0; i < g.nprob; ++i) {
+      const GemmProb& p = g.p[i];
+      if (!p.ad_p) continue;
+      if (p.mask || p.resid || p.headw || p.cstat || p.splitk > 1 || p.act != ACT_NONE || p.bias || !p.store_c || !p.c_vec ||
+          p.M % BM || p.N % BN || !p.ad_p_next || !p.ad_m || !p.ad_v || p.ad_p_next == p.ad_p ||
+          !aligned16(p.ad_p) || !aligned16(p.ad_p_next) || !aligned16(p.ad_m) || !aligned16(p.ad_v) || !aligned16(p.ad_tgt))
+        return hipErrorInvalidValue;
+    }
+    if constexpr (BM == 128 && BN == 96) {
+      return hipErrorInvalidValue;
+    } else {
+      hipLaunchKernelGGL((gemm_f32_kernel<BM, BN, GEMM_BK, WM, WN, true, false, false, true>), grid, block, pad, s, g);
+      return hipGetLastError();
+    }
   }
   if (apro) {
     if constexpr ((BM == 64 && BN == 64) || (BM == 128 && BN == 64) || (BM == 128 && BN == 96)) {
diff --git a/porl_amd/csrc/kernels.hpp b/porl_amd/csrc/kernels.hpp
--- a/porl_amd/csrc/kernels.hpp
+++ b/porl_amd/csrc/kernels.hpp
@@ -331,6 +331,8 @@
 constexpr int ADAM_SWEEP_SLABS = 16;
 constexpr int MAX_ADAM_REGIONS = 8;
 struct AdamRegion { long lo, hi; const float* slab; long stride; int nslab; };
+constexpr int MAX_ADAM_COPIES = 2 * 7;
+struct AdamCopy { long lo, hi; const float* src; };
 struct AdamArgs {
   float* p; float* g; float* m; float* v; float* tgt;
   long n4;
@@ -340,15 +342,21 @@
   int nregions; AdamRegion region[MAX_ADAM_REGIONS];
   int nskip; long skip_lo[MAX_REDUCE_JOBS], skip_hi[MAX_REDUCE_JOBS];
   int job_block0[MAX_REDUCE_JOBS + 1];
+  int ncopy; AdamCopy copy[MAX_ADAM_COPIES];
   ReduceArgs r;
 };
 
-__device__ __forceinline__ float ema1(float t, float p, float omeb, float ema_beta) { return t * omeb + ema_beta * p; }
+enum : int { EMA_SWEEP = 0, EMA_REDUCE = 1, EMA_STANDALONE = 2 };
+__device__ __forceinline__ float ema1(float t, float p, float omeb, float ema_beta, int form = EMA_SWEEP) {
+  if (form == EMA_REDUCE) return __fadd_rn(__fmul_rn(t, omeb), __fmul_rn(ema_beta, p));
+  if (form == EMA_STANDALONE) return __fmaf_rn(omeb, t, __fmul_rn(ema_beta, p));
+  return __fmaf_rn(ema_beta, p, __fmul_rn(t, omeb));
+}
 
 __device__ __forceinline__ void adam1(float& p, float g, float& m, float& v, const AdamScalars& s) {
-  m = m + s.omb1 * (g - m);
-  v = v * s.beta2 + s.omb2 * g * g;
-  p = p - s.step_size * (m / (sqrtf(v) / s.bc2_sqrt + s.eps));
+  m = __fmaf_rn(s.omb1, g - m, m);
+  v = __fmaf_rn(g, __fmul_rn(s.omb2, g), __fmul_rn(v, s.beta2));
+  p = __fmaf_rn(-s.step_size, m / (sqrtf(v) / s.bc2_sqrt + s.eps), p);
 }
 
 __global__ __launch_bounds__(256) void adam_ema_kernel(const AdamArgs a) {
@@ -371,7 +379,7 @@
         float pp = a.p[e], mm = a.m[e], vv = a.v[e];
         adam1(pp, t, mm, vv, s);
         a.p[e] = pp; a.m[e] = mm; a.v[e] = vv;
-        if (a.tgt) a.tgt[e] = ema1(a.tgt[e], pp, s.omeb, s.ema_beta);
+        if (a.tgt) a.tgt[e] = ema1(a.tgt[e], pp, s.omeb, s.ema_beta, EMA_REDUCE);
       }
     }
     return;
@@ -385,12 +393,26 @@
   bool special = false;
   for (int q = 0; q < a.nregions; ++q) special = special || (lo4 * 4 < a.region[q].hi && hi4 * 4 > a.region[q].lo);
   for (int q = 0; q < a.nskip; ++q) special = special || (lo4 * 4 < a.skip_hi[q] && hi4 * 4 > a.skip_lo[q]);
+  for (int q = 0; q < a.ncopy; ++q) {
+    const AdamCopy& C = a.copy[q];
+    if (lo4 * 4 >= C.lo && hi4 * 4 <= C.hi) {
+      const float4* s4 = reinterpret_cast<const float4*>(C.src);
+      for (long i = lo4 + threadIdx.x; i < hi4; i += 256) p4[i] = s4[i - C.lo / 4];
+      return;
+    }
+    special = special || (lo4 * 4 < C.hi && hi4 * 4 > C.lo);
+  }
   for (long i = lo4 + threadIdx.x; i < hi4; i += 256) {
     float4 gg;
     bool have_g = false;
     if (special) {
       const long e = i * 4;
       bool skip = false;
+      for (int q = 0; q < a.ncopy; ++q)
+        if (e >= a.copy[q].lo && e < a.copy[q].hi) {
+          p4[i] = *reinterpret_cast<const float4*>(a.copy[q].src + (e - a.copy[q].lo));
+          skip = true;
+        }
       for (int q = 0; q < a.nskip; ++q) skip = skip || (e >= a.skip_lo[q] && e < a.skip_hi[q]);
       if (skip) continue;
       for (int q = 0; q < a.nregions; ++q) {
@@ -437,8 +459,8 @@
   if (i >= n4) return;
   float4 tt = t4[i];
   const float4 pp = p4[i];
-  tt.x = ema1(tt.x, pp.x, omeb, ema_beta); tt.y = ema1(tt.y, pp.y, omeb, ema_beta);
-  tt.z = ema1(tt.z, pp.z, omeb, ema_beta); tt.w = ema1(tt.w, pp.w, omeb, ema_beta);
+  tt.x = ema1(tt.x, pp.x, omeb, ema_beta, EMA_STANDALONE); tt.y = ema1(tt.y, pp.y, omeb, ema_beta, EMA_STANDALONE);
+  tt.z = ema1(tt.z, pp.z, omeb, ema_beta, EMA_STANDALONE); tt.w = ema1(tt.w, pp.w, omeb, ema_beta, EMA_STANDALONE);
   t4[i] = tt;
 }
 
diff --git a/porl_amd/csrc/porl_api.hip b/porl_amd/csrc/porl_api.hip
--- a/porl_amd/csrc/porl_api.hip
+++ b/porl_amd/csrc/porl_api.hip
@@ -120,6 +120,7 @@
   int skinny = 7;
   int skinny_pipelined = -1, skinny_pipelined_max_h = 768;
   int dw0_slabs = 16;
+  int fused_adam = 0, fused_adam_pipelined = 0;
   int iql_fold = 1;
   int gemm_lds_pad = 0, gemm_lds_pad_min_blocks = 0;
   int iql_pad_value = 18432, iql_pad_policy = 0, iql_pad_min_blocks = 4 * NUM_CU, iql_pad_min_k = 0;
@@ -145,7 +146,7 @@
     TK(iql_pad_min_blocks, TC_NONNEG), TK(iql_pad_min_k, TC_NONNEG), TK(qnet_fused, TC_BOOL), TK(qnet_two_groups, TC_BOOL),
     TK(qnet_wgrad_share, TC_1_16), TK(qnet_rows16, TC_BOOL), TK(enc_dense_patch, TC_BOOL), TK(enc_s2d, TC_BOOL), TK(enc_patch_rows, TC_NONNEG),
     TK(enc_gemm_sb, TC_ANY), TK(enc_tile_n96, TC_BOOL), TK(enc_bn_sweep, TC_BOOL), TK(enc_pconv_mfma, TC_BOOL), TK(enc_bf16_operands_only, TC_BOOL),
-    TK(iql_fold, TC_BOOL), TK(skinny, TC_MASK), TK(skinny_pipelined, TC_MASK), TK(skinny_pipelined_max_h, TC_ANY), TK(dw0_slabs, TC_1_16),
+    TK(iql_fold, TC_BOOL), TK(fused_adam, TC_BOOL), TK(fused_adam_pipelined, TC_BOOL), TK(skinny, TC_MASK), TK(skinny_pipelined, TC_MASK), TK(skinny_pipelined_max_h, TC_ANY), TK(dw0_slabs, TC_1_16),
     TK(l0_tile, TC_ANY), TK(l0_kernel, TC_BOOL), TK(vbwd_tile_short, TC_ANY),
 };
 
@@ -216,8 +217,16 @@
   int64_t xhat_v[2][PORL_MAX_HIDDEN], rstd_v[2][PORL_MAX_HIDDEN];
   int64_t ln_dg[2], ln_db[2], ln_dh[2];
   int64_t head_part[2], head_loss, head_db[2];
+  int64_t w1n_v[2][PORL_MAX_HIDDEN], w1n_p[PORL_MAX_HIDDEN];
   int64_t pol_w;
   int64_t total;
+};
+
+struct FusedAdam {
+  bool pending = false;
+  int n = 0;
+  AdamCopy copy[MAX_ADAM_COPIES];
+  AdamScalars s{};
 };
 
 }
@@ -234,6 +243,7 @@
   int slot = 0;
   ReduceArgs fin_v{}, fin_p{};
   bool fin_v_pending = false, fin_p_pending = false;
+  FusedAdam fz_v, fz_p;
   int batch = 0;
   bool have_pol_target = false;
   bool pol_prefetched = false;
@@ -283,20 +293,22 @@
   double flops = 0.0, bytes = 0.0;
   std::string label;
   if (g_prof.on) {
-    bool vec = true, apro = false;
+    bool vec = true, apro = false, fuse = false;
     for (int i = 0; i < g.nprob; ++i) {
       const GemmProb& p = g.p[i];
       flops += 2.0 * p.M * p.N * p.K;
       bytes += 4.0 * ((double)p.M * p.K + (double)p.N * p.K + (p.store_c ? (double)p.M * p.N : 0.0));
+      if (p.ad_p) bytes += 4.0 * (double)p.M * p.N * (p.ad_tgt ? 8.0 : 6.0);
       vec = vec && p.a_vec && p.b_vec;
       apro = apro || p.apro != APRO_NONE;
+      fuse = fuse || p.ad_p != nullptr;
     }
     int bm, bn;
     tile_dims(tile, bm, bn);
     const TileCfg tc = tile_cfg(tile);
     label = "gemm_f32_kernel<" + std::to_string(bm) + "," + std::to_string(bn) + "," + std::to_string(GEMM_BK) + "," +
             std::to_string(tc.wm) + "," + std::to_string(tc.wn) + "," + (vec ? "true" : "false") + "," +
-            (apro ? "true" : "false") + (g.single_buffer && vec && tile == TILE_64x64 ? ",true>" : ">");
+            (apro ? "true" : "false") + (fuse ? ",false,true>" : g.single_buffer && vec && tile == TILE_64x64 ? ",true>" : ">");
   }
   ProfScope ps(label, s, flops, bytes);
   hipError_t e = launch_gemm_group(tile, g, s);
@@ -367,6 +379,37 @@
 int iql_launch(const porl_iql* h, GemmGroup& g, int tile, bool policy, hipStream_t s) {
   const Tune& t = h->tune;
   return launch_group(g, tile, t, s, !short_blocks(h) ? -1 : policy ? t.iql_pad_policy : t.iql_pad_value);
+}
+
+AdamScalars adam_scalars(double lr, int step, double b1, double b2, double eps, double ema_beta) {
+  AdamScalars s{};
+  const double bc1 = 1.0 - std::pow(b1, (double)step);
+  const double bc2 = 1.0 - std::pow(b2, (double)step);
+  s.step_size = (float)(lr / bc1);
+  s.bc2_sqrt = (float)std::sqrt(bc2);
+  s.omb1 = (float)(1.0 - b1); s.beta2 = (float)b2; s.omb2 = (float)(1.0 - b2);
+  s.eps = (float)eps; s.ema_beta = (float)ema_beta; s.omeb = (float)(1.0 - ema_beta);
+  return s;
+}
+
+struct FuseCand { int prob; int64_t off; float* stage; };
+void fuse_adam(GemmGroup& g, int tile, FusedAdam* fz, const FuseCand* cand, int ncand, const float* p, float* m, float* v,
+               float* tgt) {
+  if (!fz || tile == TILE_128x96 || g.single_buffer) return;
+  int bm, bn;
+  tile_dims(tile, bm, bn);
+  for (int i = 0; i < g.nprob; ++i)
+    if (!g.p[i].a_vec || !g.p[i].b_vec || g.p[i].apro != APRO_NONE) return;
+  for (int c = 0; c < ncand; ++c) {
+    GemmProb& q = g.p[cand[c].prob];
+    const int64_t off = cand[c].off;
+    if (q.M % bm || q.N % bn || q.splitk > 1 || q.ldc != q.N || !q.store_c || !aligned16(q.C) || off % 4 ||
+        !aligned16(cand[c].stage) || fz->n >= MAX_ADAM_COPIES)
+      continue;
+    q.ad_p = p + off; q.ad_p_next = cand[c].stage; q.ad_m = m + off; q.ad_v = v + off; q.ad_tgt = tgt ? tgt + off : nullptr;
+    g.ad = fz->s;
+    fz->copy[fz->n++] = AdamCopy{(long)off, (long)(off + (int64_t)q.M * q.N), cand[c].stage};
+  }
 }
 
 constexpr int MAX_FWD_NETS = 5;
@@ -497,6 +540,10 @@
     }
   }
   w.pol_w = take(B);
+  for (int l = 1; l < L; ++l) {
+    for (int i = 0; i < 2; ++i) w.w1n_v[i][l] = take((int64_t)H * H);
+    w.w1n_p[l] = take((int64_t)H * H);
+  }
   w.total = o;
   *out = h;
   return PORL_OK;
@@ -528,6 +575,7 @@
     if (!aligned16(p)) PORL_FAIL(PORL_ERR_INVALID, "buffers must be 16-byte aligned");
   }
   h->buf = *b;
+  h->fz_v = FusedAdam{}; h->fz_p = FusedAdam{};
   h->bound = true;
   h->device = device_of(b->workspace);
   h->batch = 0;
@@ -564,7 +612,7 @@
   return PORL_OK;
 }
 
-static int value_backward_ln(porl_iql* h, const porl_iql_hyper* hp, hipStream_t s, ReduceArgs* defer) {
+static int value_backward_ln(porl_iql* h, const porl_iql_hyper* hp, hipStream_t s, ReduceArgs* defer, FusedAdam* fz) {
   (void)hp;
   const int B = h->batch, S = h->cfg.obs_dim, H = h->cfg.hidden_dim, L = h->cfg.n_hidden, Hp = h->Hp;
   float* W = h->buf.workspace;
@@ -599,12 +647,14 @@
     }
     ReduceArgs red{};
     GemmGroup g{};
+    FuseCand cand[2];
     for (int i = 0; i < 2; ++i) {
       const float* dz = W + ws.dz_v[i][1];
       const float* in = l == 0 ? W + ws.xs_slot[h->slot] : W + ws.act_v[i][l - 1];
       const int ldin = l == 0 ? h->Sp : Hp;
       GemmProb p = make_prob(GEMM_TN, dz, Hp, in, ldin, Gv + h->v[i].w[l], Kin, H, Kin, B);
       p.colsum = Gv + h->v[i].b[l];
+      cand[i] = FuseCand{g.nprob, h->v[i].w[l], W + ws.w1n_v[i][l]};
       g.p[g.nprob++] = p;
       if (l > 0)
         g.p[g.nprob++] = make_prob(GEMM_NN, dz, Hp, Pv + h->v[i].w[l], Kin, W + ws.dz_v[i][0], Hp, B, Kin, H);
@@ -625,6 +675,7 @@
         }
       }
     }
+    if (l > 0) fuse_adam(g, tile, fz, cand, 2, Pv, h->buf.adam_m_vf, h->buf.adam_v_vf, h->buf.params_tgt);
     PORL_TRY(iql_launch(h, g, tile, false, s));
     if (l == 0 && defer) *defer = red;
     else PORL_TRY(launch_reduce(red, s));
@@ -672,8 +723,10 @@
 
 int porl_iql_set_mode(porl_iql* h, int32_t mode) {
   if (!h) PORL_FAIL(PORL_ERR_INVALID, "null engine");
-  if (mode & ~(PORL_IQL_MODE_TWO_SLOTS | PORL_IQL_MODE_FOLD_COMBINE | PORL_IQL_MODE_SHORT_BLOCKS)) PORL_FAIL(PORL_ERR_INVALID, "unknown mode bits");
-  if (h->fin_v_pending || h->fin_p_pending) PORL_FAIL(PORL_ERR_INVALID, "a backward pass is waiting for its apply call");
+  if (mode & ~(PORL_IQL_MODE_TWO_SLOTS | PORL_IQL_MODE_FOLD_COMBINE | PORL_IQL_MODE_SHORT_BLOCKS | PORL_IQL_MODE_FUSED_ADAM))
+    PORL_FAIL(PORL_ERR_INVALID, "unknown mode bits");
+  if (h->fin_v_pending || h->fin_p_pending || h->fz_v.pending || h->fz_p.pending)
+    PORL_FAIL(PORL_ERR_INVALID, "a backward pass is waiting for its apply call");
   h->mode = mode;
   return PORL_OK;
 }
@@ -714,7 +767,7 @@
   return true;
 }
 
-static int value_backward_impl(porl_iql* h, const porl_iql_hyper* hp, hipStream_t s, ReduceArgs* defer) {
+static int value_backward_impl(porl_iql* h, const porl_iql_hyper* hp, hipStream_t s, ReduceArgs* defer, FusedAdam* fz = nullptr) {
   const int B = h->batch, S = h->cfg.obs_dim, H = h->cfg.hidden_dim, L = h->cfg.n_hidden, Hp = h->Hp;
   float* W = h->buf.workspace;
   const Workspace& ws = h->ws;
@@ -764,7 +817,7 @@
   }
 
   ReduceArgs red{};
-  if (LN) return value_backward_ln(h, hp, s, defer);
+  if (LN) return value_backward_ln(h, hp, s, defer, fz);
   {
     const int nhb = cdiv(B, HEAD_ROWS_PER_BLOCK);
     HeadBwdArgs a{};
@@ -801,12 +854,14 @@
       }
     }
     GemmGroup g{};
+    FuseCand cand[2];
     for (int i = 0; i < 2; ++i) {
       const float* dz = W + ws.dz_v[i][l & 1];
       const float* in = l == 0 ? W + ws.xs_slot[h->slot] : W + ws.act_v[i][l - 1];
       const int ldin = l == 0 ? h->Sp : Hp;
       GemmProb p = make_prob(GEMM_TN, dz, Hp, in, ldin, Gv + h->v[i].w[l], Kin, H, Kin, B);
       p.colsum = Gv + h->v[i].b[l];
+      cand[i] = FuseCand{g.nprob, h->v[i].w[l], W + ws.w1n_v[i][l]};
       g.p[g.nprob++] = p;
       if (l > 0) {
         GemmProb q = make_prob(GEMM_NN, dz, Hp, Pv + h->v[i].w[l], Kin, W + ws.dz_v[i][(l - 1) & 1], Hp, B, Kin, H);
@@ -831,6 +886,7 @@
         }
       }
     }
+    if (l > 0) fuse_adam(g, tile, fz, cand, 2, Pv, h->buf.adam_m_vf, h->buf.adam_v_vf, h->buf.params_tgt);
     g_phase = l == 0 ? "V6.dW0:" : "V5.bwd:";
     PORL_TRY(iql_launch(h, g, tile, false, s));
   }
@@ -841,29 +897,61 @@
   return PORL_OK;
 }
 
-int porl_iql_value_backward(porl_iql* h, const porl_iql_hyper* hp, void* stream) {
+static bool fused_adam_on(const porl_iql* h) {
+  return (short_blocks(h) ? h->tune.fused_adam_pipelined : h->tune.fused_adam) != 0;
+}
+static int check_not_applied(const porl_iql* h, bool value) {
+  if ((value ? h->fz_v : h->fz_p).pending)
+    PORL_FAIL(PORL_ERR_INVALID, "the %s group's fused backward pass is waiting for its apply call", value ? "value" : "policy");
+  return PORL_OK;
+}
+static FusedAdam* fused_begin(porl_iql* h, bool value, const porl_iql_hyper* hp) {
+  FusedAdam& fz = value ? h->fz_v : h->fz_p;
+  fz = FusedAdam{};
+  fz.s = value ? adam_scalars(hp->value_lr, hp->value_step, hp->adam_beta1, hp->adam_beta2, hp->adam_eps, hp->ema_beta)
+               : adam_scalars(hp->policy_lr, hp->policy_step, hp->adam_beta1, hp->adam_beta2, hp->adam_eps, 0.0);
+  return &fz;
+}
+
+static int value_backward_phase(porl_iql* h, const porl_iql_hyper* hp, void* stream, bool fuse) {
   PORL_TRY(check_ready(h, true)); DevGuard _dg(h->device);
   if (!hp) PORL_FAIL(PORL_ERR_INVALID, "null hyper-parameters");
+  PORL_TRY(check_not_applied(h, true));
+  if (fuse && hp->value_step < 1) PORL_FAIL(PORL_ERR_INVALID, "adam step must be >= 1");
   const bool fold = (h->mode & PORL_IQL_MODE_FOLD_COMBINE) != 0;
   h->fin_v = ReduceArgs{};
-  PORL_TRY(value_backward_impl(h, hp, (hipStream_t)stream, fold ? &h->fin_v : nullptr));
+  FusedAdam* fz = fuse && fused_adam_on(h) ? fused_begin(h, true, hp) : nullptr;
+  const int rc = value_backward_impl(h, hp, (hipStream_t)stream, fold ? &h->fin_v : nullptr, fz);
+  if (fz) fz->pending = fz->n > 0;
+  if (rc) return rc;
   h->fin_v_pending = fold;
   return PORL_OK;
 }
 
+int porl_iql_value_backward(porl_iql* h, const porl_iql_hyper* hp, void* stream) {
+  return value_backward_phase(h, hp, stream, h && (h->mode & PORL_IQL_MODE_FUSED_ADAM));
+}
+
 static int adam_launch(float* p, float* g, float* m, float* v, float* tgt, int64_t n, double lr, int step,
-                       double b1, double b2, double eps, double ema_beta, hipStream_t s, const ReduceArgs* fin = nullptr) {
+                       double b1, double b2, double eps, double ema_beta, hipStream_t s, const ReduceArgs* fin = nullptr,
+                       const FusedAdam* fz = nullptr) {
   if (n < 0 || n % 4) PORL_FAIL(PORL_ERR_INVALID, "adam range must be a non-negative multiple of 4 floats");
   if (step < 1) PORL_FAIL(PORL_ERR_INVALID, "adam step must be >= 1");
   if (n == 0 && !(fin && fin->njobs)) return PORL_OK;
   AdamArgs a{};
   a.p = p; a.g = g; a.m = m; a.v = v; a.tgt = tgt;
-  const double bc1 = 1.0 - std::pow(b1, (double)step);
-  const double bc2 = 1.0 - std::pow(b2, (double)step);
-  a.s.step_size = (float)(lr / bc1);
-  a.s.bc2_sqrt = (float)std::sqrt(bc2);
-  a.s.omb1 = (float)(1.0 - b1); a.s.beta2 = (float)b2; a.s.omb2 = (float)(1.0 - b2);
-  a.s.eps = (float)eps; a.s.ema_beta = (float)ema_beta; a.s.omeb = (float)(1.0 - ema_beta);
+  a.s = adam_scalars(lr, step, b1, b2, eps, ema_beta);
+  double copy_floats = 0.0;
+  if (fz && fz->n) {
+    if (memcmp(&a.s, &fz->s, sizeof(AdamScalars)))
+      PORL_FAIL(PORL_ERR_INVALID, "apply was given other Adam hyper-parameters (step, learning rate) than the fused backward pass");
+    for (int q = 0; q < fz->n; ++q) {
+      const AdamCopy& c = fz->copy[q];
+      if (c.lo < 0 || c.hi > n || c.lo % 4 || c.hi % 4) PORL_FAIL(PORL_ERR_INVALID, "fused Adam range outside the group");
+      a.copy[a.ncopy++] = c;
+      copy_floats += (double)(c.hi - c.lo);
+    }
+  }
   a.n4 = n / 4;
   const int sweep_blocks = (int)std::min<long>((a.n4 + 255) / 256, 1 << 20);
   a.span4 = sweep_blocks ? ((a.n4 + sweep_blocks - 1) / sweep_blocks + 255) / 256 * 256 : 256;
@@ -895,7 +983,7 @@
     }
     a.job_block0[a.r.njobs] = reduce_blocks;
   }
-  ProfScope ps("adam_ema_kernel", s, 0.0, (double)n * (tgt ? 36.0 : 28.0) + extra_bytes);
+  ProfScope ps("adam_ema_kernel", s, 0.0, ((double)n - copy_floats) * (tgt ? 36.0 : 28.0) + 8.0 * copy_floats + extra_bytes);
   a.reduce_blocks = reduce_blocks;
   hipLaunchKernelGGL(adam_ema_kernel, dim3(sweep_blocks + reduce_blocks), dim3(256), 0, s, a);
   PORL_HIP(hipGetLastError());
@@ -908,9 +996,12 @@
   g_phase = "V8.";
   const int rc = adam_launch(h->buf.params_vf, h->buf.grads_vf, h->buf.adam_m_vf, h->buf.adam_v_vf, h->buf.params_tgt,
                              h->n_vf, hp->value_lr, hp->value_step, hp->adam_beta1, hp->adam_beta2, hp->adam_eps,
-                             hp->ema_beta, (hipStream_t)stream, h->fin_v_pending ? &h->fin_v : nullptr);
+                             hp->ema_beta, (hipStream_t)stream, h->fin_v_pending ? &h->fin_v : nullptr,
+                             h->fz_v.pending ? &h->fz_v : nullptr);
   g_phase = "";
+  if (rc == PORL_ERR_INVALID && h->fz_v.pending) return rc;
   h->fin_v_pending = false;
+  h->fz_v.pending = false;
   return rc;
 }
 
@@ -920,9 +1011,11 @@
   g_phase = "P9.";
   const int rc = adam_launch(h->buf.params_pol, h->buf.grads_pol, h->buf.adam_m_pol, h->buf.adam_v_pol, nullptr, h->n_pol,
                              hp->policy_lr, hp->policy_step, hp->adam_beta1, hp->adam_beta2, hp->adam_eps, 0.0,
-                             (hipStream_t)stream, h->fin_p_pending ? &h->fin_p : nullptr);
+                             (hipStream_t)stream, h->fin_p_pending ? &h->fin_p : nullptr, h->fz_p.pending ? &h->fz_p : nullptr);
   g_phase = "";
+  if (rc == PORL_ERR_INVALID && h->fz_p.pending) return rc;
   h->fin_p_pending = false;
+  h->fz_p.pending = false;
   return rc;
 }
 
@@ -980,7 +1073,7 @@
 }
 
 static int policy_backward_impl(porl_iql* h, const porl_iql_hyper* hp, hipStream_t s, ReduceArgs* defer, int part = 3,
-                                bool only_policy = false) {
+                                bool only_policy = false, FusedAdam* fz = nullptr) {
   if (!h->have_pol_target) PORL_FAIL(PORL_ERR_INVALID, "policy step needs pol_target in porl_iql_load_batch");
   const int B = h->batch, S = h->cfg.obs_dim, H = h->cfg.hidden_dim, L = h->cfg.n_hidden, D = h->cfg.pol_out_dim;
   const int Hp = h->Hp, Dp = h->Dp;
@@ -1149,6 +1242,7 @@
     const float* in = l == 0 ? W + ws.xs_slot[h->slot] : W + ws.act_p[l - 1];
     const int ldin = l == 0 ? h->Sp : Hp;
     GemmGroup g{};
+    const FuseCand cand{g.nprob, h->pol.w[l], W + ws.w1n_p[l]};
     g.p[g.nprob] = make_prob(GEMM_TN, dz, Hp, in, ldin, Gp + h->pol.w[l], Kin, H, Kin, B);
     g.p[g.nprob++].colsum = Gp + h->pol.b[l];
     if (l > 0) {
@@ -1170,6 +1264,7 @@
         add_reduce(red, Gp + h->pol.b[0], slabC, H, H, sk);
       }
     }
+    if (l > 0) fuse_adam(g, tile, fz, &cand, 1, Pp, h->buf.adam_m_pol, h->buf.adam_v_pol, nullptr);
     g_phase = l == 0 ? "P7.dW0:" : "P6.bwd:";
     PORL_TRY(iql_launch(h, g, tile, true, s));
   }
@@ -1186,30 +1281,46 @@
   return policy_backward_impl(h, hp, (hipStream_t)stream, nullptr, 1);
 }
 
-int porl_iql_policy_backward(porl_iql* h, const porl_iql_hyper* hp, void* stream) {
+static int policy_backward_phase(porl_iql* h, const porl_iql_hyper* hp, void* stream, bool fuse) {
   PORL_TRY(check_ready(h, true)); DevGuard _dg(h->device);
   if (!hp) PORL_FAIL(PORL_ERR_INVALID, "null hyper-parameters");
+  PORL_TRY(check_not_applied(h, false));
+  if (fuse && hp->policy_step < 1) PORL_FAIL(PORL_ERR_INVALID, "adam step must be >= 1");
   const bool fold = (h->mode & PORL_IQL_MODE_FOLD_COMBINE) != 0;
   h->fin_p = ReduceArgs{};
-  PORL_TRY(policy_backward_impl(h, hp, (hipStream_t)stream, fold ? &h->fin_p : nullptr));
+  FusedAdam* fz = fuse && fused_adam_on(h) ? fused_begin(h, false, hp) : nullptr;
+  const int rc = policy_backward_impl(h, hp, (hipStream_t)stream, fold ? &h->fin_p : nullptr, 3, false, fz);
+  if (fz) fz->pending = fz->n > 0;
+  if (rc) return rc;
   h->fin_p_pending = fold;
   return PORL_OK;
+}
+
+int porl_iql_policy_backward(porl_iql* h, const porl_iql_hyper* hp, void* stream) {
+  return policy_backward_phase(h, hp, stream, h && (h->mode & PORL_IQL_MODE_FUSED_ADAM));
 }
 
 int porl_iql_step(porl_iql* h, const porl_iql_hyper* hp, void* stream) {
   PORL_TRY(check_ready(h, true)); DevGuard _dg(h->device);
   if (!hp) PORL_FAIL(PORL_ERR_INVALID, "null hyper-parameters");
   hipStream_t s = (hipStream_t)stream;
+  PORL_TRY(check_not_applied(h, true));
+  PORL_TRY(check_not_applied(h, false));
+  const bool fuse = fused_adam_on(h) && hp->value_step >= 1 && hp->policy_step >= 1 && h->have_pol_target;
   ReduceArgs fin{};
-  PORL_TRY(value_backward_impl(h, hp, s, h->tune.iql_fold ? &fin : nullptr));
+  FusedAdam fz{};
+  fz.s = adam_scalars(hp->value_lr, hp->value_step, hp->adam_beta1, hp->adam_beta2, hp->adam_eps, hp->ema_beta);
+  PORL_TRY(value_backward_impl(h, hp, s, h->tune.iql_fold ? &fin : nullptr, fuse ? &fz : nullptr));
   g_phase = "V8.";
   PORL_TRY(adam_launch(h->buf.params_vf, h->buf.grads_vf, h->buf.adam_m_vf, h->buf.adam_v_vf, h->buf.params_tgt, h->n_vf,
-                       hp->value_lr, hp->value_step, hp->adam_beta1, hp->adam_beta2, hp->adam_eps, hp->ema_beta, s, &fin));
+                       hp->value_lr, hp->value_step, hp->adam_beta1, hp->adam_beta2, hp->adam_eps, hp->ema_beta, s, &fin, &fz));
   fin = ReduceArgs{};
-  PORL_TRY(policy_backward_impl(h, hp, s, h->tune.iql_fold ? &fin : nullptr));
+  fz = FusedAdam{};
+  fz.s = adam_scalars(hp->policy_lr, hp->policy_step, hp->adam_beta1, hp->adam_beta2, hp->adam_eps, 0.0);
+  PORL_TRY(policy_backward_impl(h, hp, s, h->tune.iql_fold ? &fin : nullptr, 3, false, fuse ? &fz : nullptr));
   g_phase = "P9.";
   PORL_TRY(adam_launch(h->buf.params_pol, h->buf.grads_pol, h->buf.adam_m_pol, h->buf.adam_v_pol, nullptr, h->n_pol,
-                       hp->policy_lr, hp->policy_step, hp->adam_beta1, hp->adam_beta2, hp->adam_eps, 0.0, s, &fin));
+                       hp->policy_lr, hp->policy_step, hp->adam_beta1, hp->adam_beta2, hp->adam_eps, 0.0, s, &fin, &fz));
   g_phase = "";
   return PORL_OK;
 }
@@ -1225,6 +1336,7 @@
   PORL_TRY(check_ready(h, true)); DevGuard _dg(h->device);
   if (!hp) PORL_FAIL(PORL_ERR_INVALID, "null hyper-parameters");
   if (!h->have_pol_target) PORL_FAIL(PORL_ERR_INVALID, "policy step needs pol_target in porl_iql_load_batch");
+  PORL_TRY(check_not_applied(h, false));
   hipStream_t s = (hipStream_t)stream;
   h->pol_fwd_done = false;
   ReduceArgs fin{};
@@ -1672,14 +1784,14 @@
     PORL_FAIL(PORL_ERR_INVALID, "policy target width mismatch");
   if (wait_policy_seq) PORL_TRY(porl_signal_wait_ge(sig_policy, wait_policy_seq, main_stream));
   PORL_TRY(porl_iql_load_batch_sampled(h, batch, rows, row_stride, n_rows, act_dim, target_is_action, seed, step, nullptr, main_stream));
-  PORL_TRY(porl_iql_value_backward(h, hp, main_stream));
+  PORL_TRY(value_backward_phase(h, hp, main_stream, true));
   if (wait_fwd_seq) PORL_TRY(porl_signal_wait_ge(sig_fwd, wait_fwd_seq, main_stream));
   PORL_TRY(porl_iql_value_apply(h, hp, main_stream));
   PORL_TRY(porl_signal_write(sig_value, seq, main_stream));
   PORL_TRY(porl_signal_wait_ge(sig_value, seq, side_stream));
   PORL_TRY(porl_iql_policy_forward(h, hp, side_stream));
   PORL_TRY(porl_signal_write(sig_fwd, seq, side_stream));
-  PORL_TRY(porl_iql_policy_backward(h, hp, side_stream));
+  PORL_TRY(policy_backward_phase(h, hp, side_stream, true));
   PORL_TRY(porl_iql_policy_apply(h, hp, side_stream));
   if (write_policy) PORL_TRY(porl_signal_write(sig_policy, seq, side_stream));
   return PORL_OK;
diff --git a/porl_amd/engine.py b/porl_amd/engine.py
--- a/porl_amd/engine.py
+++ b/porl_amd/engine.py
@@ -18,7 +18,7 @@
 
 class IqlEngine:
     GROUP_VF, GROUP_POL = 0, 1
-    MODE_TWO_SLOTS, MODE_FOLD_COMBINE, MODE_SHORT_BLOCKS = 1, 2, 4
+    MODE_TWO_SLOTS, MODE_FOLD_COMBINE, MODE_SHORT_BLOCKS, MODE_FUSED_ADAM = 1, 2, 4, 8
     SLOTS = 3
 
     def __init__(self, obs_dim, pol_out_dim, hidden_dim, n_hidden, layer_norm=False, pol_tanh=False,
```

After: 2980 gradient-steps/sec. 3.0% lower.
